# NVlabs/CenterPose

Hardware: AMD Instinct MI355X
Metric: images/sec at 512x512 DLA-34 (backbone + heat-map decode + post-process + PnP) (higher is better)
Workload: dtype f32 via split-f16 (f16x3) MFMA, f32 accumulate

## Files before the change

### centerpose_amd/csrc/cp_common.h

```cpp
#pragma once
#include <hip/hip_runtime.h>
#include <stdint.h>

#include "../../include/centerpose_hip_testing.h"

#if defined(__HIP_DEVICE_COMPILE__) && !defined(__gfx950__)
#error "centerpose_amd device code is written for gfx950 only (raw-buffer range-check semantics, MFMA shapes, LDS-DMA)"
#endif

#define CP_OK 0
#define CP_ERR_INVALID (-1)
#define CP_ERR_LAUNCH (-2)
#define CP_ERR_ALLOC (-3)
#define CP_ERR_STATE (-4)

enum CpAct : int {
    CP_ACT_NONE = 0,
    CP_ACT_RELU = 1,
    CP_ACT_SIGMOID = 2,
    CP_ACT_SIGMOID_FROM = 3,
};

enum CpStore : int {
    CP_STORE_NHWC = 0,
// ... 28 lines not shown
        const int nw = (int)(blockDim.x + 63) >> 6;
        float m = cp_amax_red[0];
        for (int i = 1; i < nw; ++i) m = fmaxf(m, cp_amax_red[i]);
        unsigned* sub = slot + (blockIdx.x & (CP_AMAX_SUB - 1)) * CP_AMAX_STRIDE;
        const unsigned b = __float_as_uint(m);
        if (b > __hip_atomic_load(sub, __ATOMIC_RELAXED, __HIP_MEMORY_SCOPE_AGENT)) atomicMax(sub, b);
    }
}

__device__ __forceinline__ float cp_fast_sigmoid(float x) {
    return __builtin_amdgcn_rcpf(1.f + __builtin_amdgcn_exp2f(-1.4426950408889634f * x));
}
__device__ __forceinline__ float cp_fast_tanh(float x) {
    return 2.f * __builtin_amdgcn_rcpf(1.f + __builtin_amdgcn_exp2f(-2.8853900817779268f * x)) - 1.f;
}
#endif

struct ConvParams {
    const float* src[CP_MAX_SRC];
    int src_c[CP_MAX_SRC];
    int nsrc;
    int Cin;
    int B, H, W, Ho, Wo;
    int KH, KW, stride, pad;
    int K;
    int Kpad;
    const float* wp;
    int Cout, CoutPad;
    const float* scale;
    const float* shift;
    const float* res;
    int res_ld;
    int act;
    int act_from;
    float* out;
    int store;
    int ldo;
    int coff;
    const void* w16_hi;
    const void* w16_lo;
    const void* w16f_hi;
    const void* w16f_lo;
    int Kpad16;
    double* gn_stats;
    int gn_groups, gn_cpg;
    const float* gn_in_mr;
    const float* gn_in_gamma;
    const float* gn_in_beta;
    const float* gn_in_a;
    const float* gn_in_d;
    const float* gru_x3;
    const float* gru_hprev;
    int splitk;
    float* partial;
    int tile_m, tile_n;
    const void* fuse_w2_hi;
    const void* fuse_w2_lo;
    float* fuse_out;
    int fuse_c2;
    int fuse_ngroups, fuse_gtiles;
    int fuse_gc2[CP_MAX_HEAD_GROUP];
    int fuse_gbase[CP_MAX_HEAD_GROUP];
    int fuse_final;
    int fuse_gsig[CP_MAX_HEAD_GROUP];
    const float* fuse_gbias[CP_MAX_HEAD_GROUP];
    float* fuse_gout[CP_MAX_HEAD_GROUP];
    const unsigned* in_amax[CP_MAX_SRC];
    unsigned* out_amax;
    const float* fuse_w2_inv;
    int dbg;
    const float* offmask;
    const int* row_index;
    int rows_per_image, row_index_stride;
    const float* up_t;
    const float* up_wt;
    int up_ld, up_f;
    const float* pj_src;
    int pj_c;
    const unsigned* pj_amax;
    const void* pj_w_hi;
    const void* pj_w_lo;
    const float* pj_scale;
    const float* pj_shift;
};

int cp_launch_conv(const ConvParams& p, hipStream_t stream);
int cp_conv_tile_n(int cout);
int cp_conv_variant(const ConvParams& p);
int cp_launch_splitk_epilogue(const ConvParams& p, hipStream_t stream);
void cp_conv_geometry(const ConvParams& p, bool f16x3, int* tiles, int* nk);
const char* cp_conv_variant_name(int v);
#define CP_NUM_CONV_VARIANTS 46
#define CP_VARIANT_HEAD_ROWS 45
#define CP_VARIANT_DECONV_F32 43
#define CP_VARIANT_DECONV16 44
#define CP_VARIANT_STRM16 41
#define CP_VARIANT_LOWC1S 42
#define CP_VARIANT_GRU 26
bool cp_conv16_supported(const ConvParams& p);
int cp_launch_conv16(const ConvParams& p, hipStream_t stream);
int cp_conv16_variant(const ConvParams& p);
bool cp_conv16_project_supported(const ConvParams& p);
bool cp_halo16_supported(const ConvParams& p);
bool cp_halo16_fused_head_supported(const ConvParams& p);
int cp_launch_halo16_fused_head(const ConvParams& p, hipStream_t stream);
bool cp_halo16_gru_supported(const ConvParams& p);
int cp_launch_halo16_gru(const ConvParams& p, hipStream_t stream);
int cp_launch_halo16(const ConvParams& p, int bn, hipStream_t stream);
bool cp_halo16_project_supported(const ConvParams& p, int bn);
bool cp_strm16_supported(const ConvParams& p);
int cp_strm16_jobs(const ConvParams& p);
int cp_launch_strm16(const ConvParams& p, hipStream_t stream);
int cp_launch_dcn16(const ConvParams& p, int bn, hipStream_t stream);
bool cp_pw16_supported(const ConvParams& p);
int cp_launch_pw16(const ConvParams& p, hipStream_t stream);
bool cp_dcn16p_supported(const ConvParams& p);
int cp_dcn16p_blocks(const ConvParams& p);
int cp_launch_dcn16p(const ConvParams& p, hipStream_t stream);
bool cp_dcn16p_wide(const ConvParams& p);
#define CP_VARIANT_DCN16S 36
#define CP_VARIANT_M64N64 37
#define CP_VARIANT_DCN16PW 38
bool cp_dcn16s_supported(const ConvParams& p);
int cp_dcn16s_items(const ConvParams& p);
int cp_launch_dcn16s(const ConvParams& p, hipStream_t stream);
int cp_launch_frag16_repack(const void* w16, void* w16f, int CoutPad, int Kpad16, hipStream_t s);
#define CP_VARIANT_DCN16T 39
bool cp_dcn16t_supported(const ConvParams& p);
bool cp_dcn16t_upadd_supported(const ConvParams& p);
int cp_launch_dcn16t(const ConvParams& p, hipStream_t stream);
#define CP_VARIANT_DCN16P 30
#define CP_VARIANT_GN_FINAL 31
#define CP_VARIANT_HALO_HEAD 32
#define CP_VARIANT_HALO_GRU 33
#define CP_VARIANT_PW16 34
int cp_launch_pack_weight16(const float* w, void* hi, void* lo, int Cout, int Cin, int taps, int Kpad16, int coff,
                            const float* fwd, hipStream_t s);
int cp_launch_weight_scale(const float* w, int Cout, int per, float* fwd, float* inv, hipStream_t s);
int cp_launch_scale16(const float* scale, const float* inv, float* out, int n, hipStream_t s);
int cp_launch_absmax(const float* x, size_t n, unsigned* slot, hipStream_t s);
bool cp_head_fuse_supported(const ConvParams& p, int c2);
int cp_launch_conv16_fused_head(const ConvParams& p, hipStream_t stream);
int cp_launch_conv16_fused_head_rows(const ConvParams& p, hipStream_t stream);
int cp_launch_pack_head_w2(const float* w1, void* hi, void* lo, float* w2_inv, int C2, int Chid, hipStream_t s);
int cp_launch_head_reduce(const float* slabs, const float* bias, float* out_nchw, int slices, int C2, int B, int HW,
                          int sigmoid, hipStream_t s);
struct HeadReduceGroup {
    int n, slices;
    int c2[CP_MAX_HEAD_GROUP], base[CP_MAX_HEAD_GROUP], sigmoid[CP_MAX_HEAD_GROUP];
    const float* bias[CP_MAX_HEAD_GROUP];
    float* out[CP_MAX_HEAD_GROUP];
};
int cp_launch_head_reduce_grouped(const float* slabs, const HeadReduceGroup& g, int B, int HW, hipStream_t s);
int cp_launch_conv16_gru(const ConvParams& p, hipStream_t stream);
#define CP_VARIANT_FUSED_HEAD 22
size_t cp_lowc_weight_halfs(int kind);
int cp_launch_pack_lowc(int kind, const float* w, void* hi, void* lo, const float* fwd, int cin, hipStream_t s);
int cp_launch_lowc(int kind, const float* in, float* out, const void* w_hi, const void* w_lo, const float* scale,
                   const float* shift, const unsigned* in_amax, unsigned* out_amax, int B, int H, int W, int planes,
                   hipStream_t s);
#define CP_VARIANT_LOWC0 23
#define CP_VARIANT_LOWC01 40
int cp_launch_lowc_fused(const float* in, float* out, const void* w0_hi, const void* w0_lo, const float* scale0, const float* shift0,
                         const void* w1_hi, const void* w1_lo, const float* scale1, const float* shift1, float bound_l, float bound_s,
                         const unsigned* in_amax, unsigned* out_amax, int B, int H, int W, int planes, hipStream_t s);
struct DeconvLaunch {
    const float* x;
    const float* wf;
    const void* w_hi;
    const void* w_lo;
    const float* scale;
    const float* shift;
    float* out;
    const unsigned* in_amax;
    unsigned* out_amax;
    int B, H, W, Cin, Cout, relu, f16x3;
};
int cp_deconv_cout_pad(int Cout);
int cp_launch_pack_deconv(const float* w, float* wf, void* hi, void* lo, float* inv, int Cin, int Cout, hipStream_t s);
int cp_launch_deconv(const DeconvLaunch& l, hipStream_t s);
#define CP_PREC_F32 0
#define CP_PREC_F16X3 1

int cp_launch_nchw_to_nhwc(const float* in, float* out, int B, int C, int H, int W, int Cpad, hipStream_t s);
int cp_launch_nhwc_to_nchw(const float* in, float* out, int B, int C, int H, int W, int ldi, hipStream_t s);
int cp_launch_maxpool2(const float* in, float* out, int B, int H, int W, int C, hipStream_t s);
int cp_launch_maxpool3s2(const float* in, float* out, int B, int H, int W, int C, unsigned* out_amax, hipStream_t s);
int cp_launch_upsample_add(const float* in, const float* w, const float* add, float* out, int B, int H, int W,
                           int C, int f, unsigned* out_amax, hipStream_t s);
int cp_launch_add_relu_sum(const float* a, const float* b, const float* c, const float* d, float* out, size_t n,
                           unsigned* out_amax, hipStream_t s);
int cp_launch_upsample2_nearest_add(const float* up1, const float* low, float* out, int B, int H, int W, int C,
                                    unsigned* out_amax, hipStream_t s);
int cp_launch_gru_gate(const float* x3, const float* h3, const float* hprev, float* hout, size_t M, unsigned* out_amax,
                       hipStream_t s);
int cp_launch_groupnorm_relu(float* x, const float* gamma, const float* beta, double* stats_ws, int B, int HW, int C,
                             int groups, float eps, unsigned* out_amax, hipStream_t s);
int cp_launch_gn_final(const float* x, const float* ga, const float* gd, const float* wp, const float* bias, float* out,
                       int B, int HW, int C, int N, int wld, int sigmoid, hipStream_t s);
int cp_launch_gn_affine(const double* stats, const float* gamma, const float* beta, float* a, float* d, int B, int C,
                        int groups, double count, float eps, const unsigned* x_amax, unsigned* y_amax, hipStream_t s);
int cp_launch_gn_finalize(const double* stats, float* mr, int n, double count, float eps, hipStream_t s);
int cp_launch_pack_weight(const float* w, float* wp, int Cout, int Cin, int taps, int CinP, int CoutPad, int coff,
                          hipStream_t s);

#define CP_DET_BBOX 0
#define CP_DET_SCORE 4
#define CP_DET_KPS 5
#define CP_DET_CLS 21
#define CP_DET_SCALE 22
#define CP_DET_SCALE_UNC 25
#define CP_DET_TRACKING 28
#define CP_DET_TRACKING_HP 30
#define CP_DET_KPS_DISP_MEAN 46
#define CP_DET_KPS_DISP_STD 62
#define CP_DET_KPS_HM_MEAN 78
#define CP_DET_KPS_HM_STD 94
#define CP_DET_KPS_HM_HEIGHT 110
#define CP_DET_STRIDE 118
size_t cp_decode_ws_bytes(int B, int J, int K);
int cp_launch_decode(hipStream_t s, int B, int J, int H, int W, float* hm, const float* hps, const float* wh,
                     const float* hps_unc, const float* scale, const float* scale_unc, const float* reg, float* hm_hp,
                     const float* hp_offset, const float* tracking, const float* tracking_hp, int K, int rep_mode,
                     int fit_gaussian, float balance, int legacy_bool_mask, int apply_sigmoid, float* det, void* ws);
int cp_launch_decode_peaks(hipStream_t s, int B, int J, int H, int W, float* hm, float* hm_hp, int K, int apply_sigmoid,
                           float* pk_score, int* pk_ind, void* cand);
int cp_launch_decode_assoc(hipStream_t s, int B, int J, int H, int W, const float* hps, const float* wh, const float* hps_unc,
                           const float* scale, const float* scale_unc, const float* reg, const float* hm_hp,
                           const float* hp_offset, const float* tracking, const float* tracking_hp, const float* pk_score,
                           const int* pk_ind, int K, int rep_mode, int fit_gaussian, float balance, int legacy_bool_mask,
                           int compact, float* det);
size_t cp_decode_cand_bytes(int B, int J, int H, int W, int K);
size_t cp_decode_tiled_ws_bytes(int B, int J, int H, int W, int K);
int cp_launch_decode_tiled(hipStream_t s, int B, int J, int H, int W, float* hm, const float* hps, const float* wh,
                           const float* hps_unc, const float* scale, const float* scale_unc, const float* reg, float* hm_hp,
                           const float* hp_offset, const float* tracking, const float* tracking_hp, int K, int rep_mode,
                           int fit_gaussian, float balance, int legacy_bool_mask, int apply_sigmoid, float* det, void* ws);

int cp_launch_dcn_generic(hipStream_t s, const float* x, const float* w, const float* bias, const float* offset,
                          const float* mask, float* out, int B, int C, int H, int W, int Co, int Ho, int Wo, int kh, int kw,
                          int sh, int sw, int ph, int pw, int dh, int dw, int dg);

struct DcnBwdArgs {
// ... 152 lines not shown
```

### centerpose_amd/csrc/engine.hip

```cpp
#include "engine_model.h"
#include "track_common.h"

namespace {
thread_local std::string g_err;
}

namespace cp_engine {
int fail(int code, const std::string& msg) {
    g_err = msg;
    return code;
}
int g_default_precision = CP_PREC_F32;
int g_dbg = 0;
}

using namespace cp_engine;

static void drop_kept_in(cp_model* m, const void* ws, size_t bytes) {
    const char* k = (const char*)m->kept.ptr;
    if (k && k >= (const char*)ws && k < (const char*)ws + bytes) m->kept = cp_model::KeptFeat();
}

template <class F>
static int replay_or_capture(cp_model* m, hipStream_t s, const std::vector<uint64_t>& key, F&& enqueue) {
// ... 29 lines not shown
extern "C" {

const char* cp_version(void) { return "centerpose_hip 0.3.0 (gfx950; f32 and split-f16 MFMA)"; }
int cp_abi_version(void) { return CP_ABI_VERSION; }
static_assert(CP_NUM_KERNEL_VARIANTS == CP_NUM_CONV_VARIANTS, "public and internal kernel-variant counts");
int cp_num_kernel_variants(void) { return CP_NUM_KERNEL_VARIANTS; }
int cp_num_roles(void) { return CP_NUM_ROLES; }
const char* cp_last_error(void) { return g_err.c_str(); }

int cp_set_debug(int flags) {
    if (flags & ~CP_SEL_ALL)
        return fail(CP_ERR_INVALID, "cp_set_debug: unknown switch bits " + std::to_string(flags & ~CP_SEL_ALL));
    g_dbg = flags;
    return CP_OK;
}

int cp_set_default_precision(int precision) {
    if (precision != CP_PREC_F32 && precision != CP_PREC_F16X3) return fail(CP_ERR_INVALID, "precision must be 0 or 1");
    g_default_precision = precision;
    return CP_OK;
}

int cp_model_set_precision(cp_model* m, int precision) {
    if (!m || (precision != CP_PREC_F32 && precision != CP_PREC_F16X3)) return fail(CP_ERR_INVALID, "bad argument");
    m->precision = precision;
    m->ws_cached = 0;
    return CP_OK;
}

int cp_model_profile(cp_model* m, int enable) {
    if (!m) return fail(CP_ERR_INVALID, "null model");
    m->profile = enable != 0;
    return CP_OK;
}

int cp_model_profile_read(cp_model* m, double* out, int num_variants) {
    if (!m || !out || num_variants < CP_NUM_CONV_VARIANTS) return fail(CP_ERR_INVALID, "bad argument");
    for (int i = 0; i < num_variants * 4; ++i) out[i] = 0.0;
    for (int i = 0; i < CP_NUM_ROLES * 4; ++i) m->roles[i] = 0.0;
    const char* dump = getenv("CP_PROFILE_DUMP");
    FILE* df = dump ? fopen(dump, "a") : nullptr;
    for (auto& r : m->prof) {
        float ms = 0.f;
        if (hipEventSynchronize(r.e1) != hipSuccess || hipEventElapsedTime(&ms, r.e0, r.e1) != hipSuccess)
            return fail(CP_ERR_LAUNCH, "event timing failed");
        if (df)
            fprintf(df, "%s,%d,%d,%d,%d,%d,%.4f,%.2f,%s\n", r.variant >= 0 ? cp_conv_variant_name(r.variant) : "decode", r.M,
                    r.N, r.K, r.kh, r.stride, ms, r.flops / (ms * 1e-3) / 1e12, cp_role_name(r.role));
        if (r.variant >= 0) {
            out[r.variant * 4 + 0] += 1.0;
            out[r.variant * 4 + 1] += ms;
            out[r.variant * 4 + 2] += r.flops;
            out[r.variant * 4 + 3] += r.bytes;
        }
        if (r.role >= 0 && r.role < CP_NUM_ROLES) {
            m->roles[r.role * 4 + 0] += 1.0;
            m->roles[r.role * 4 + 1] += ms;
            m->roles[r.role * 4 + 2] += r.flops;
            m->roles[r.role * 4 + 3] += r.bytes;
        }
        m->event_pool.push_back(r.e0);
        m->event_pool.push_back(r.e1);
    }
    m->prof.clear();
    if (df) fclose(df);
    return CP_OK;
}

const char* cp_kernel_variant_name(int v) { return cp_conv_variant_name(v); }

const char* cp_role_name(int role) {
    static const char* names[CP_NUM_ROLES] = {"conv", "conv1x1", "dcn", "dcn_offset", "head", "head_final", "gru", "lowc",
                                              "decode", "deconv"};
    return (role >= 0 && role < CP_NUM_ROLES) ? names[role] : "?";
}

int cp_model_profile_roles(cp_model* m, double* out, int num_roles) {
    if (!m || !out || num_roles < CP_NUM_ROLES) return fail(CP_ERR_INVALID, "bad argument");
    for (int i = 0; i < CP_NUM_ROLES * 4; ++i) out[i] = m->roles[i];
    return CP_OK;
}

size_t cp_model_workspace_used(const cp_model* m) { return m ? m->arena.peak : 0; }

size_t cp_model_workspace_bytes(cp_model* m, int B, int H, int W) {
    if (!m) {
        fail(CP_ERR_STATE, "cp_model_workspace_bytes: null model");
        return 0;
    }
    if (m->ws_cached && m->ws_key[0] == B && m->ws_key[1] == H && m->ws_key[2] == W && m->ws_key[3] == g_dbg && m->finalized)
        return m->ws_cached;
    size_t peak = 0;
    const char* const tap_before = m->tap_name;
    const int nu = m->ups_t.empty() ? 1 : 3;
    const int np = m->convs.count("base.level2.project") ? 2 : 1;
    for (int v = 0; v < 4 * nu * np; ++v) {
        const int up = (v >> 2) % nu;
        m->dry_variant = v & 1;
        m->tap_name = (v & 2) ? "" : nullptr;
        m->dry_no_upadd = up != 0;
        m->dry_boundary_upadd = up == 2;
        m->dry_no_project = v >= 4 * nu;
        const int rc = forward_impl(m, nullptr, B, H, W, nullptr, (const float*)1, (const float*)1, (const float*)1, nullptr, 0,
                                    nullptr, 0, true);
        m->dry_variant = 0;
        m->dry_no_upadd = false;
        m->dry_boundary_upadd = false;
        m->dry_no_project = false;
        m->tap_name = tap_before;
        if (rc != CP_OK) return 0;
        if (m->arena.peak > peak) peak = m->arena.peak;
    }
    m->ws_key[0] = B; m->ws_key[1] = H; m->ws_key[2] = W; m->ws_key[3] = g_dbg;
    m->ws_cached = peak;
    return peak;
}

int cp_model_forward(cp_model* m, cp_stream_t stream, int B, int H, int W, const float* images, const float* pre_img,
                     const float* pre_hm, const float* pre_hm_hp, float* const* head_out, int sigmoid_hm,
                     void* workspace, size_t workspace_bytes) {
    if (!images || !head_out || !workspace) return fail(CP_ERR_INVALID, "null argument");
    m->tap_name = nullptr;
    drop_kept_in(m, workspace, workspace_bytes);
    return forward_impl(m, (hipStream_t)stream, B, H, W, images, pre_img, pre_hm, pre_hm_hp, head_out, sigmoid_hm,
                        workspace, workspace_bytes, false);
}

int cp_model_features(cp_model* m, cp_stream_t stream, int B, int H, int W, const float* images, const float* pre_img,
                      const float* pre_hm, const float* pre_hm_hp, float* feat_out, void* workspace, size_t workspace_bytes) {
    if (!m || !images || !feat_out || !workspace) return fail(CP_ERR_INVALID, "null argument");
    if (m->gru) return fail(CP_ERR_STATE, "cp_model_features: dlav1 heads read the ConvGRU steps through GroupNorm, not one feature map");
    if (m->hourglass) return fail(CP_ERR_STATE, "cp_model_features: hourglass has two stacks of heads, not one feature map");
    m->tap_name = nullptr;
    drop_kept_in(m, workspace, workspace_bytes);
    m->feat_out = feat_out;
    const int rc = forward_impl(m, (hipStream_t)stream, B, H, W, images, pre_img, pre_hm, pre_hm_hp, nullptr, 0, workspace,
                                workspace_bytes, false);
    m->feat_out = nullptr;
    return rc;
}

static size_t detect_decode_ws_bytes(int B, int H, int W, int K) {
    const int ho = H / 4, wo = W / 4;
    return ho * wo <= 32768 ? cp_decode_ws_bytes(B, 8, K) : cp_decode_tiled_ws_bytes(B, 8, ho, wo, K);
}

size_t cp_model_detect_workspace_bytes(cp_model* m, int B, int H, int W, int K) {
    const size_t a = cp_model_workspace_bytes(m, B, H, W);
    const size_t d = detect_decode_ws_bytes(B, H, W, K);
    return a && d ? align_up(a, 256) + d : 0;
}

int cp_model_detect(cp_model* m, cp_stream_t stream, int B, int H, int W, const float* images, const float* pre_img,
                    const float* pre_hm, const float* pre_hm_hp, float* const* head_out, int K, int rep_mode,
                    int fit_gaussian, float balance, int legacy_bool_mask, float* det, void* workspace,
                    size_t workspace_bytes, int use_graph) {
    if (!m || !images || !head_out || !det || !workspace) return fail(CP_ERR_INVALID, "null argument");
    if (!m->finalized) return fail(CP_ERR_STATE, "model not finalized");
    const size_t model_ws = align_up(cp_model_workspace_bytes(m, B, H, W), 256);
    if (model_ws == 0) return CP_ERR_INVALID;
    const bool tiled = (H / 4) * (W / 4) > 32768;
    const size_t dec_ws = detect_decode_ws_bytes(B, H, W, K);
    if (dec_ws == 0) return fail(CP_ERR_INVALID, "detect: unsupported decode shape (need K <= 128, K <= H*W/16 <= 2^20, W/4 <= 4096)");
    if (workspace_bytes < model_ws + dec_ws) return fail(CP_ERR_INVALID, "workspace too small");
    float* hp[11] = {nullptr, nullptr, nullptr, nullptr, nullptr, nullptr, nullptr, nullptr, nullptr, nullptr, nullptr};
    const char* names[11] = {"hm", "hps", "wh", "hps_uncertainty", "scale", "scale_uncertainty", "reg", "hm_hp",
                             "hp_offset", "tracking", "tracking_hp"};
    for (size_t i = 0; i < m->headw.size(); ++i)
        for (int j = 0; j < 11; ++j)
            if (m->headw[i].name == names[j]) hp[j] = head_out[i];
    if (!hp[0] || !hp[1] || !hp[2] || !hp[7]) return fail(CP_ERR_INVALID, "detect needs the hm, hps, wh and hm_hp heads");
    hipStream_t s = (hipStream_t)stream;
    auto enqueue = [&]() -> int {
        m->tap_name = nullptr;
        int rc = forward_impl(m, s, B, H, W, images, pre_img, pre_hm, pre_hm_hp, head_out, 1, workspace, model_ws, false);
        if (rc != CP_OK) return rc;
        rc = timed(m, s, [&](cp_model::ProfRec& r) {
            const double hw = (double)(H / 4) * (W / 4);
            r.variant = -1;
            r.role = CP_ROLE_DECODE;
            r.flops = 0.0;
            r.bytes = (double)B * (9.0 * hw * 4 + K * 60.0 * 4 + 8.0 * K * 2 * 4 + (double)K * CP_DET_STRIDE * 4);
            r.M = B; r.N = K; r.K = (int)hw; r.kh = 0; r.stride = 0;
        }, [&]() {
            return (tiled ? cp_launch_decode_tiled : cp_launch_decode)(
                s, B, 8, H / 4, W / 4, hp[0], hp[1], hp[2], hp[3], hp[4], hp[5], hp[6], hp[7], hp[8], hp[9], hp[10], K, rep_mode,
                fit_gaussian, balance, legacy_bool_mask, 0, det, (char*)workspace + model_ws);
        });
        if (rc != CP_OK) return fail(rc, "detect: decode failed (need K <= 128, K <= H*W/16 <= 2^20, W/4 <= 4096)");
        return rc;
    };
// ... 423 lines not shown
```

### centerpose_amd/csrc/engine_forward.hip

```cpp
#include "engine_model.h"

using namespace cp_engine;

namespace {

constexpr int kSplitTiles = 128, kSplitTarget = 384;
constexpr long kLeanMinPixels = 32768;

struct Fwd {
    cp_model* m;
    int B;
    hipStream_t s;
    double* gn_stats_out = nullptr;
    const float* gn_in_mr = nullptr;
    const float* gn_in_a = nullptr;
    const float* gn_in_d = nullptr;
    const float* gn_in_gamma = nullptr;
    const float* gn_in_beta = nullptr;
    int role = -1;
    const unsigned* gn_in_amax = nullptr;
    static constexpr int kMaxSlots = CP_AMAX_STRIDE;
    static constexpr size_t kSlotBytes = (size_t)CP_AMAX_SUB * CP_AMAX_STRIDE * sizeof(unsigned);
    Tensor slots_t;
    unsigned* slots = nullptr;
// ... 269 lines not shown
        timed([&](cp_model::ProfRec& r) { decode_rec(r, (double)B * (K * 60.0 * 4 + 8.0 * K * 2 * 4 + (double)K * CP_DET_STRIDE * 4)); },
              [&]() {
                  return cp_launch_decode_assoc(s, B, J, x.H, x.W, tb[1], tb[2], tb[3], tb[4], tb[5], tb[6], hm_hp, tb[8], tb[9], tb[10],
                                                lc.pk_score, lc.pk_ind, K, lc.rep_mode, lc.fit_gaussian, lc.balance,
                                                lc.legacy_bool_mask, 1, lc.det);
              });
        return true;
    }

    struct UpFuse {
        const Tensor* t;
        const float* wt;
        int f;
    };
    int plan_split(ConvParams& p, bool use16, const ConvW& w) {
        int tiles = 0, nk = 0;
        cp_conv_geometry(p, use16, &tiles, &nk);
        if (use16 && tiles > 0 && (tiles <= 32 || (tiles <= 64 && nk <= 36)) && nk >= 8 && !p.gn_stats && !p.gn_in_a &&
            p.CoutPad % 64 == 0 && w.Cout >= 64 && !(g_dbg & CP_SEL_TILE128_SMALL)) {
            p.tile_m = p.tile_n = 64;
            cp_conv_geometry(p, use16, &tiles, &nk);
        }
        const bool force_strm = use16 && (g_dbg & CP_SEL_STRM16_ALWAYS) && cp_strm16_supported(p);
        if (tiles > 0 && tiles < (p.tile_m == 64 ? 256 : kSplitTiles) && nk >= 8 && !p.gn_stats && !force_strm) {
            int want = (kSplitTarget + tiles - 1) / tiles;
            if (want > nk / 2) want = nk / 2;
            if (want > 32) want = 32;
            if (want > 1) {
                const int per = (nk + want - 1) / want;
                const int sk = (nk + per - 1) / per;
                if (sk > 1) return sk;
            }
        }
        return 1;
    }
    bool upadd_fusable(const DeformW& d, int C, int H, int W, int t_c, int f, bool boundary = false) {
        if (m->precision != CP_PREC_F16X3 || (m->dry_no_upadd && !(boundary && m->dry_boundary_upadd))) return false;
        const float* const some = (const float*)0x1000;
        ConvParams p = conv_params(B, H, W, &some, &C, 1, d.main, 1, 1, CP_ACT_RELU);
        if (p.Cin != d.main.CinP) return false;
        p.offmask = some;
        const unsigned* no_amax = nullptr;
        if (!conv_params_f16(p, d.main, &no_amax, true)) return false;
        p.store = CP_STORE_NHWC;
        p.ldo = d.main.Cout;
        p.up_t = p.up_wt = some;
        p.up_ld = t_c;
        p.up_f = f;
        p.splitk = plan_split(p, true, d.main);
        return p.splitk == 1 && cp_conv16_variant(p) == CP_VARIANT_DCN16T && cp_dcn16t_upadd_supported(p);
    }

    struct ProjFuse {
        const Tensor* bottom;
        const ConvW* w;
    };
    bool project_fusable(const std::string& p, const ConvW& wp, const ConvW& w2, int cb, int C, int H, int W) {
        if (m->precision != CP_PREC_F16X3 || m->dry_no_project) return false;
        if (m->tap_name && std::strstr(m->tap_name, ".project") != nullptr) return false;
        if (g_dbg & (CP_SEL_PW16_FRAG_A | CP_SEL_PW16_NEVER)) return false;
        if (wp.CoutPad != w2.CoutPad || wp.Cout != w2.Cout || wp.Kpad16 != cb || !wp.w16f_hi || !wp.w16f_lo) return false;
        const float* const some = (const float*)0x1000;
        const unsigned* no_amax = nullptr;
        ConvParams q = conv_params(B, H, W, &some, &cb, 1, wp, 1, 0, CP_ACT_NONE);
        if (q.Cin != wp.CinP || !conv_params_f16(q, wp, &no_amax, true)) return false;
        q.store = CP_STORE_NHWC;
        q.ldo = wp.Cout;
        q.splitk = plan_split(q, true, wp);
        const int qv = cp_conv16_variant(q);
        if (q.splitk != 1 || (qv != CP_VARIANT_PW16 && qv != CP_VARIANT_PW16 + 1)) return false;
        ConvParams c = conv_params(B, H, W, &some, &C, 1, w2, 1, 1, CP_ACT_RELU);
        if (c.Cin != w2.CinP || !conv_params_f16(c, w2, &no_amax, true)) return false;
        c.store = CP_STORE_NHWC;
        c.ldo = w2.Cout;
        c.pj_src = some;
        c.pj_c = cb;
        c.pj_w_hi = c.pj_w_lo = some;
        c.splitk = plan_split(c, true, w2);
        return c.splitk == 1 && cp_conv16_project_supported(c);
    }

    Tensor conv(const ConvW& w, const std::vector<const Tensor*>& srcs, int stride, int pad, int act,
                const Tensor* res = nullptr, const Tensor* offmask = nullptr, int act_from = 0,
                float* out_nchw = nullptr, int out_ld = 0, const UpFuse* up = nullptr, const ProjFuse* pj = nullptr) {
        const Tensor& x0 = *srcs[0];
        const int nsrc = (int)srcs.size();
        const float* src[CP_MAX_SRC];
        int src_c[CP_MAX_SRC];
        const unsigned* src_amax[CP_MAX_SRC];
        for (int i = 0; i < nsrc; ++i) {
            src[i] = srcs[i]->ptr();
            src_c[i] = srcs[i]->C;
            src_amax[i] = srcs[i]->amax;
        }
        ConvParams p = conv_params(B, x0.H, x0.W, src, src_c, nsrc, w, stride, pad, act);
        if (p.Cin != w.CinP) {
            chk(fail(CP_ERR_INVALID, "conv: channel mismatch"));
            return Tensor();
        }
        p.res = res ? res->ptr() : nullptr;
        p.res_ld = res ? res->C : 0;
        p.act_from = act_from;
        p.offmask = offmask ? offmask->ptr() : nullptr;
        p.gn_stats = gn_stats_out;
        p.gn_groups = 32;
        p.gn_cpg = w.Cout / 32 > 0 ? w.Cout / 32 : 1;
        if (gn_in_a) {
            p.gn_in_a = gn_in_a;
            p.gn_in_d = gn_in_d;
        }
        if (gn_in_mr) {
            p.gn_in_mr = gn_in_mr;
            p.gn_in_gamma = gn_in_gamma;
            p.gn_in_beta = gn_in_beta;
            p.gn_cpg = w.Cin / 32;
        }
        const bool use16 = conv_params_f16(p, w, src_amax, m->precision == CP_PREC_F16X3);
        if (use16 && p.gn_in_a) p.in_amax[0] = gn_in_amax;
        if (p.gn_in_a && !use16) {
            chk(fail(CP_ERR_INVALID, "conv: GroupNorm affine input without an f16x3 kernel"));
            return Tensor();
        }
        Tensor out;
        if (out_nchw) {
            p.out = out_nchw;
            p.store = CP_STORE_NCHW;
            p.ldo = out_ld;
            p.coff = 0;
        } else {
            const int cstore = (act == CP_ACT_SIGMOID_FROM) ? w.CoutPad : w.Cout;
            out = make(cstore, p.Ho, p.Wo);
            p.out = out.ptr();
            p.out_amax = act == CP_ACT_SIGMOID_FROM ? nullptr : out.amax;
            p.store = CP_STORE_NHWC;
            p.ldo = cstore;
            p.coff = 0;
        }
        Tensor partial;
        p.splitk = plan_split(p, use16, w);
        if (p.splitk > 1) {
            partial = make(p.splitk * p.CoutPad, p.Ho, p.Wo);
            p.partial = partial.ptr();
        }
        if (up) {
            p.up_t = up->t->ptr();
            p.up_wt = up->wt;
            p.up_ld = up->t->C;
            p.up_f = up->f;
        }
        if (pj) {
            p.pj_src = pj->bottom->ptr();
            p.pj_c = pj->bottom->C;
            p.pj_amax = pj->bottom->amax;
            p.pj_w_hi = pj->w->w16f_hi;
            p.pj_w_lo = pj->w->w16f_lo;
            p.pj_scale = pj->w->scale16;
            p.pj_shift = pj->w->shift;
        }
        auto launch = [&]() -> int {
            int rc = use16 ? cp_launch_conv16(p, s) : cp_launch_conv(p, s);
            if (rc == CP_OK && p.splitk > 1) rc = cp_launch_splitk_epilogue(p, s);
            return rc;
        };
        if (!m->dry)
            timed([&](cp_model::ProfRec& r) {
                r.variant = use16 ? cp_conv16_variant(p) : cp_conv_variant(p);
                r.role = role >= 0 ? role : offmask ? CP_ROLE_DCN : act == CP_ACT_SIGMOID_FROM ? CP_ROLE_DCN_OFFSET
                         : (w.KH == 1 && w.KW == 1) ? CP_ROLE_CONV1X1 : CP_ROLE_CONV;
                const double M = (double)B * p.Ho * p.Wo;
                const int cin_real = w.Cin;
                r.flops = 2.0 * M * w.Cout * (double)(w.KH * w.KW * cin_real + (pj ? pj->w->Cin : 0));
                r.bytes = 4.0 * ((double)B * x0.H * x0.W * cin_real + M * w.Cout +
                                 (double)w.KH * w.KW * cin_real * w.Cout + (offmask ? M * 27 : 0.0) +
                                 (res ? M * w.Cout : 0.0) + (up ? (double)B * up->t->H * up->t->W * w.Cout : 0.0) +
                                 (pj ? (M + w.Cout) * (double)pj->w->Cin : 0.0));
                r.M = (int)M; r.N = w.Cout; r.K = w.KH * w.KW * cin_real; r.kh = w.KH; r.stride = stride;
            }, launch);
        gn_stats_out = nullptr;
        gn_in_mr = nullptr;
        gn_in_a = nullptr;
        gn_in_d = nullptr;
        gn_in_amax = nullptr;
        role = -1;
        return out;
    }
    const ConvW& cw(const std::string& k) { return m->convs.at(k); }

    Tensor maxpool(const Tensor& x) {
        Tensor o = make(x.C, x.H / 2, x.W / 2);
        o.amax = x.amax;
        if (!m->dry) chk(cp_launch_maxpool2(x.ptr(), o.ptr(), B, x.H, x.W, x.C, s));
        return o;
    }

    Tensor basic_block(const std::string& p, const Tensor& x, int stride, const Tensor* residual, const ProjFuse* pj = nullptr) {
        Tensor t = conv(cw(p + ".conv1"), {&x}, stride, 1, CP_ACT_RELU);
        tap(p + ".conv1", t);
        Tensor o = conv(cw(p + ".conv2"), {&t}, 1, 1, CP_ACT_RELU, residual, nullptr, 0, nullptr, 0, nullptr, pj);
        tap(p, o);
        return o;
    }

    Tensor tree1(const std::string& p, const Tensor& x, int cin, int cout, int stride, bool level_root,
                 std::vector<const Tensor*> children, const Tensor* bottom_in = nullptr) {
        Tensor bottom_own;
        const Tensor* bottom = &x;
        if (stride > 1) {
            if (bottom_in) bottom = bottom_in;
            else {
                bottom_own = maxpool(x);
                bottom = &bottom_own;
            }
        }
        Tensor proj;
        const Tensor* residual = bottom;
        ProjFuse pj = {bottom, nullptr};
        if (cin != cout) {
            const ConvW& wp = cw(p + ".project");
            const ConvW& w2 = cw(p + ".tree1.conv2");
            if (project_fusable(p, wp, w2, bottom->C, w2.CinP, bottom->H, bottom->W)) {
                pj.w = &wp;
                residual = nullptr;
            } else {
                proj = conv(wp, {bottom}, 1, 0, CP_ACT_NONE);
                tap(p + ".project", proj);
                residual = &proj;
            }
        }
        if (level_root) children.insert(children.begin(), bottom);
        Tensor x1 = basic_block(p + ".tree1", x, stride, residual, pj.w ? &pj : nullptr);
        proj = Tensor();
        Tensor x2 = basic_block(p + ".tree2", x1, 1, &x1);
        std::vector<const Tensor*> srcs = {&x2, &x1};
        for (auto* c : children) srcs.push_back(c);
        Tensor o = conv(cw(p + ".root"), srcs, 1, 0, CP_ACT_RELU);
        tap(p + ".root", o);
        return o;
    }
    Tensor tree2(const std::string& p, const Tensor& x, int cin, int cout) {
        Tensor bottom = maxpool(x);
        Tensor x1 = tree1(p + ".tree1", x, cin, cout, 2, false, {}, &bottom);
        return tree1(p + ".tree2", x1, cout, cout, 1, false, {&bottom, &x1});
    }

    Tensor deform(const std::string& p, const Tensor& x, const UpFuse* up = nullptr) {
        const DeformW& d = m->deforms.at(p);
        Tensor om = conv(d.offset, {&x}, 1, 1, CP_ACT_SIGMOID_FROM, nullptr, nullptr, 18);
        tap(p + ".offmask", om, 27);
        Tensor o = conv(d.main, {&x}, 1, 1, CP_ACT_RELU, nullptr, &om, 0, nullptr, 0, up);
        if (!up) tap(p, o);
        return o;
    }
    Tensor upsample_add(const std::string& p, const Tensor& x, int f, const Tensor& add) {
        Tensor o = make(x.C, x.H * f, x.W * f);
        if (!m->dry)
            chk(cp_launch_upsample_add(x.ptr(), m->ups.at(p), add.ptr(), o.ptr(), B, x.H, x.W, x.C, f, o.amax, s));
        return o;
    }
    struct IdaNext {
        std::string p;
        const Tensor* layer;
        int f;
    };
    Tensor ida(const std::string& p, std::vector<Tensor>& layers, int startp, int endp, const std::vector<int>& up_f,
               bool node_dead = false, const IdaNext* next = nullptr, Tensor u_first = Tensor()) {
        const bool tap_on_node = m->tap_name && std::strstr(m->tap_name, ".node_") != nullptr;
        Tensor u_next = u_first;
        u_first = Tensor();
        for (int i = startp + 1; i < endp; ++i) {
            const std::string k = std::to_string(i - startp);
            Tensor u = u_next;
            u_next = Tensor();
            if (!u.valid()) {
                Tensor t = deform(p + ".proj_" + k, layers[i]);
                u = upsample_add(p + ".up_" + k, t, up_f[i - startp], layers[i - 1]);
            }
            tap(p + ".up_" + k, u);
            const std::string kn = std::to_string(i + 1 - startp);
            const int fn = i + 1 < endp ? up_f[i + 1 - startp] : 0;
            const DeformW& node = m->deforms.at(p + ".node_" + k);
            if (node_dead && !tap_on_node && i + 1 < endp && m->ups_t.count(p + ".up_" + kn) &&
                upadd_fusable(node, u.C, u.H, u.W, m->deforms.at(p + ".proj_" + kn).main.Cout, fn)) {
                Tensor t = deform(p + ".proj_" + kn, layers[i + 1]);
                const UpFuse up = {&t, m->ups_t.at(p + ".up_" + kn), fn};
                u_next = deform(p + ".node_" + k, u, &up);
                layers[i] = Tensor();
            } else if (next && i + 1 == endp && m->ups_t.count(next->p + ".up_1") &&
                       !(m->tap_name && std::strncmp(m->tap_name, (p + ".node_" + k).c_str(), (p + ".node_" + k).size()) == 0) &&
                       upadd_fusable(node, u.C, u.H, u.W, m->deforms.at(next->p + ".proj_1").main.Cout, next->f, true)) {
                Tensor t = deform(next->p + ".proj_1", *next->layer);
                const UpFuse up = {&t, m->ups_t.at(next->p + ".up_1"), next->f};
                u_next = deform(p + ".node_" + k, u, &up);
                layers[i] = Tensor();
            } else {
                layers[i] = deform(p + ".node_" + k, u);
            }
        }
        return u_next;
    }

    Tensor lowc(const std::string& name, int kind, const float* in, int H, int W, int planes, const unsigned* in_amax) {
        if (m->precision != CP_PREC_F16X3 || (g_dbg & CP_SEL_NO_LOWC)) return Tensor();
        const int Ho = kind == 2 ? (H - 1) / 2 + 1 : H, Wo = kind == 2 ? (W - 1) / 2 + 1 : W;
        if (kind == 2 && m->lowc.count(name + ".rows") && !(g_dbg & CP_SEL_LEVEL1_ROWS_NEVER) &&
            ((g_dbg & CP_SEL_LEVEL1_ROWS_ALWAYS) || (long)B * ((Wo + 31) / 32) * ((Ho + 7) / 8) >= 2048))
            kind = 5;
        auto it = m->lowc.find(kind == 5 ? name + ".rows" : name);
        if (it == m->lowc.end()) return Tensor();
        const ConvW& w = cw(name);
        const bool stem = kind == 0 || kind == 3;
        const bool l1 = kind == 2 || kind == 5;
        const int cout = l1 ? 32 : 16, cin = stem ? planes : 16, k = stem ? 7 : 3;
        Tensor out = make(cout, Ho, Wo);
        if (m->dry) return out;
        auto launch = [&]() {
            return cp_launch_lowc(kind, in, out.ptr(), it->second.hi, it->second.lo, it->second.scale16, w.shift, in_amax,
                                  out.amax, B, H, W, planes, s);
        };
        timed([&](cp_model::ProfRec& r) {
            r.variant = kind == 5 ? CP_VARIANT_LOWC1S : CP_VARIANT_LOWC0 + (kind == 3 ? 0 : kind);
            r.role = CP_ROLE_LOWC;
            const double M = (double)B * Ho * Wo;
            r.flops = 2.0 * M * cout * (double)(k * k * cin);
            r.bytes = 4.0 * ((double)B * H * W * cin + M * cout + (double)k * k * cin * cout);
            r.M = (int)M; r.N = cout; r.K = k * k * cin; r.kh = k; r.stride = l1 ? 2 : 1;
        }, launch);
        return out;
    }

    Tensor to_nhwc(const float* nchw, int C, int Cpad, int H, int W) {
        Tensor t = make(Cpad, H, W);
        t.amax = nullptr;
        if (!m->dry) chk(cp_launch_nchw_to_nhwc(nchw, t.ptr(), B, C, H, W, Cpad, s));
        return t;
    }
    Tensor stem(const char* name, int kind, const float* nchw, int H, int W, int C, int Cpad, bool use_lowc) {
        Tensor t = lowc(name, kind, nchw, H, W, C, use_lowc && !m->dry ? input_slot(nchw, (size_t)B * C * H * W) : nullptr);
        if (!t.valid()) {
            Tensor in = to_nhwc(nchw, C, Cpad, H, W);
            t = conv(cw(name), {&in}, 1, 3, CP_ACT_RELU);
        }
        return t;
    }

    Tensor hg_residual(const std::string& p, const Tensor& x, int stride) {
        Tensor t = conv(cw(p + ".conv1"), {&x}, stride, 1, CP_ACT_RELU);
        if (m->convs.count(p + ".skip")) {
            Tensor sk = conv(cw(p + ".skip"), {&x}, stride, 0, CP_ACT_NONE);
            return conv(cw(p + ".conv2"), {&t}, 1, 1, CP_ACT_RELU, &sk);
        }
        return conv(cw(p + ".conv2"), {&t}, 1, 1, CP_ACT_RELU, &x);
    }
    Tensor hg_seq(const std::string& p, Tensor x, int n, int first_stride) {
        for (int i = 0; i < n; ++i) x = hg_residual(p + "." + std::to_string(i), x, i == 0 ? first_stride : 1);
        return x;
    }
    Tensor hg_kp(const std::string& p, const Tensor& x, int n, const int* mods) {
        const int cm = mods[0], nm = mods[1];
        Tensor up1 = hg_seq(p + ".up1", x, cm, 1);
        Tensor low = hg_seq(p + ".low1", x, cm, 2);
        low = n > 1 ? hg_kp(p + ".low2", low, n - 1, mods + 1) : hg_seq(p + ".low2", low, nm, 1);
        low = hg_seq(p + ".low3", low, cm, 1);
        Tensor out = make(up1.C, up1.H, up1.W);
        if (!m->dry)
            chk(cp_launch_upsample2_nearest_add(up1.ptr(), low.ptr(), out.ptr(), B, low.H, low.W, low.C, out.amax, s));
        tap(p, out);
        return out;
    }
    void run_hourglass(int H, int W, const float* images, float* const* head_out, int sigmoid_hm) {
        static const int mods[6] = {2, 2, 2, 2, 2, 4};
        init_slots();
        Tensor inter;
        {
            Tensor in = to_nhwc(images, 3, 4, H, W);
            Tensor p0 = conv(cw("pre.0"), {&in}, 2, 3, CP_ACT_RELU);
            inter = hg_residual("pre.1", p0, 2);
        }
        tap("pre", inter);
        Tensor cnv;
        for (int k = 0; k < 2; ++k) {
            const std::string ks = std::to_string(k);
            Tensor kp = hg_kp("kps." + ks, inter, 5, mods);
            cnv = conv(cw("cnvs." + ks), {&kp}, 1, 1, CP_ACT_RELU);
            tap("cnvs." + ks, cnv);
            if (k == 0) {
                Tensor a = conv(cw("inters_.0"), {&inter}, 1, 0, CP_ACT_NONE);
                Tensor b = conv(cw("cnvs_.0"), {&cnv}, 1, 0, CP_ACT_RELU, &a);
                inter = hg_residual("inters.0", b, 1);
            }
        }
        if (fused_heads_grouped(cnv, head_out, sigmoid_hm)) return;
        for (size_t i = 0; i < m->headw.size(); ++i) {
            const HeadW& hw = m->headw[i];
            const bool sg = sigmoid_hm && (hw.name == "hm" || hw.name == "hm_hp");
            if (hw.w2_hi && m->precision == CP_PREC_F16X3 && !m->tap_name && !(g_dbg & CP_SEL_NO_HEAD_FUSION) &&
                fused_head(hw, cnv, sg, m->dry ? (float*)0x1000 : head_out[i]))
                continue;
            role = CP_ROLE_HEAD;
            Tensor hid = conv(hw.c0, {&cnv}, 1, 1, CP_ACT_RELU);
            role = CP_ROLE_HEAD_FINAL;
            conv(hw.c1, {&hid}, 1, 0, sg ? CP_ACT_SIGMOID : CP_ACT_NONE, nullptr, nullptr, 0,
                 m->dry ? (float*)0x1000 : head_out[i], hw.classes);
        }
    }

    Tensor deconv(const std::string& p, const Tensor& x) {
        const DeconvW& d = m->deconvs.at(p);
// ... 53 lines not shown
            for (int b = 0; b < blocks[l]; ++b) x = res_block(ln + "." + std::to_string(b), x, b == 0 && l ? 2 : 1, bott);
            tap(ln, x);
        }
        for (int i = 0; i < 3; ++i) {
            const std::string fc = "deconv_layers." + std::to_string(6 * i);
            x = deform(fc, x);
            tap("deconv_layers." + std::to_string(6 * i + 2), x);
            x = deconv("deconv_layers." + std::to_string(6 * i + 3), x);
            tap("deconv_layers." + std::to_string(6 * i + 5), x);
        }
        if (features_only(x)) return;
        for (size_t i = 0; i < m->headw.size(); ++i) {
            const HeadW& hw = m->headw[i];
            const bool sg = sigmoid_hm && (hw.name == "hm" || hw.name == "hm_hp");
            role = CP_ROLE_HEAD;
            Tensor hid = conv(hw.c0, {&x}, 1, 1, CP_ACT_RELU);
            role = CP_ROLE_HEAD_FINAL;
            conv(hw.c1, {&hid}, 1, 0, sg ? CP_ACT_SIGMOID : CP_ACT_NONE, nullptr, nullptr, 0,
                 m->dry ? (float*)0x1000 : head_out[i], hw.classes);
        }
    }

    void run(int H, int W, const float* images, const float* pre_img, const float* pre_hm, const float* pre_hm_hp,
             float* const* head_out, int sigmoid_hm) {
        init_slots();
        const bool use_lowc = m->precision == CP_PREC_F16X3 && !(g_dbg & CP_SEL_NO_LOWC) && m->lowc.count("base.base_layer");
        const bool no_pre = m->dry ? m->dry_variant == 1 : (!pre_img && !pre_hm && !pre_hm_hp);
        const bool fuse01 = use_lowc && no_pre && m->lowc.count("base.level0.rows") && m->stem_bound_l > 0.f &&
                            !(g_dbg & CP_SEL_STEM_LEVEL0_UNFUSED) && !(m->tap_name && std::strcmp(m->tap_name, "base.base_layer") == 0) &&
                            !m->convs.count("base.pre_img_layer") && !m->convs.count("base.pre_hm_layer") && !m->convs.count("base.pre_hm_hp_layer");
        Tensor l0f;
        if (fuse01) {
            const unsigned* in_slot = !m->dry ? input_slot(images, (size_t)B * 3 * H * W) : nullptr;
            l0f = make(16, H, W);
            if (!m->dry) {
                const LowcW& a = m->lowc["base.base_layer"];
                const LowcW& c = m->lowc["base.level0.rows"];
                auto launch = [&]() {
                    return cp_launch_lowc_fused(images, l0f.ptr(), a.hi, a.lo, a.scale16, cw("base.base_layer").shift, c.hi, c.lo, c.scale16,
                                                cw("base.level0").shift, m->stem_bound_l, m->stem_bound_s, in_slot, l0f.amax, B, H, W, 3, s);
                };
                timed([&](cp_model::ProfRec& r) {
                    r.variant = CP_VARIANT_LOWC01;
                    r.role = CP_ROLE_LOWC;
                    const double M = (double)B * H * W;
                    r.flops = 2.0 * M * 16 * (147.0 + 144.0);
                    r.bytes = 4.0 * (M * 3 + M * 16);
                    r.M = (int)M; r.N = 16; r.K = 147 + 144; r.kh = 7; r.stride = 1;
                }, launch);
            }
        }
        Tensor x0 = fuse01 ? Tensor() : stem("base.base_layer", 0, images, H, W, 3, 4, use_lowc);
        if (m->dry) {
            if (!m->convs.count("base.pre_img_layer")) pre_img = nullptr;
            if (!m->convs.count("base.pre_hm_layer")) pre_hm = nullptr;
            if (!m->convs.count("base.pre_hm_hp_layer")) pre_hm_hp = nullptr;
        }
        if ((pre_img && !m->convs.count("base.pre_img_layer")) || (pre_hm && !m->convs.count("base.pre_hm_layer")) ||
            (pre_hm_hp && !m->convs.count("base.pre_hm_hp_layer"))) {
            chk(fail(CP_ERR_INVALID, "a previous-frame input was given to a model built without that pre_* layer"));
            return;
        }
        if (pre_img || pre_hm || pre_hm_hp) {
            Tensor a, b, c;
            if (pre_img) a = stem("base.pre_img_layer", 0, pre_img, H, W, 3, 4, use_lowc);
            if (pre_hm) b = stem("base.pre_hm_layer", 0, pre_hm, H, W, 1, 4, use_lowc);
            if (pre_hm_hp) c = stem("base.pre_hm_hp_layer", 3, pre_hm_hp, H, W, 8, 8, use_lowc);
            std::vector<const Tensor*> adds;
            for (Tensor* t : {&a, &b, &c})
                if (t->valid()) adds.push_back(t);
            Tensor sum = make(16, H, W);
            if (!m->dry)
                chk(cp_launch_add_relu_sum(x0.ptr(), adds[0]->ptr(), adds.size() > 1 ? adds[1]->ptr() : nullptr,
                                           adds.size() > 2 ? adds[2]->ptr() : nullptr, sum.ptr(),
                                           (size_t)B * H * W * 16, sum.amax, s));
            x0 = sum;
        }
        if (!fuse01) tap("base.base_layer", x0);
        Tensor l0 = fuse01 ? l0f : lowc("base.level0", 1, x0.ptr(), H, W, 16, x0.amax);
        l0f = Tensor();
        if (!l0.valid()) l0 = conv(cw("base.level0"), {&x0}, 1, 1, CP_ACT_RELU);
        tap("base.level0", l0);
        x0 = Tensor();
        Tensor l1 = lowc("base.level1", 2, l0.ptr(), H, W, 16, l0.amax);
        if (!l1.valid()) l1 = conv(cw("base.level1"), {&l0}, 2, 1, CP_ACT_RELU);
        tap("base.level1", l1);
        l0 = Tensor();
        std::vector<Tensor> L(6);
        L[2] = tree1("base.level2", l1, 32, 64, 2, false, {});
        l1 = Tensor();
        L[3] = tree2("base.level3", L[2], 64, 128);
        L[4] = tree2("base.level4", L[3], 128, 256);
        L[5] = tree1("base.level5", L[4], 256, 512, 2, true, {});
        tap("base.level2", L[2]);
        tap("base.level3", L[3]);
        tap("base.level4", L[4]);
        tap("base.level5", L[5]);

        ida("dla_up.ida_0", L, 4, 6, {1, 2});
        Tensor o2 = L[5];
        ida("dla_up.ida_1", L, 3, 6, {1, 2, 2});
        Tensor o1 = L[5];
        const IdaNext to_ida_up = {"ida_up", &o1, 2};
        Tensor u1 = ida("dla_up.ida_2", L, 2, 6, {1, 2, 2, 2}, true, &to_ida_up);
        Tensor o0 = L[5];
        for (auto& t : L) t = Tensor();
        std::vector<Tensor> y = {o0, o1, o2};
        o0 = o1 = o2 = Tensor();
        ida("ida_up", y, 0, 3, {1, 2, 4}, true, nullptr, u1);
        u1 = Tensor();
        Tensor feat = y[2];
        y.clear();
        tap("feat", feat);
        if (features_only(feat)) return;

        std::vector<Tensor> gru_out;
        if (m->gru) {
            const int steps = m->tracking ? 4 : 3;
            role = CP_ROLE_GRU;
            Tensor x3 = conv(m->gru_x, {&feat}, 1, 1, CP_ACT_NONE);
            Tensor h;
            for (int st = 0; st < steps; ++st) {
                Tensor hn = make(64, feat.H, feat.W);
                const size_t M = (size_t)B * feat.H * feat.W;
                if (st == 0) {
                    if (!m->dry) chk(cp_launch_gru_gate(x3.ptr(), nullptr, nullptr, hn.ptr(), M, hn.amax, s));
                } else if (m->precision == CP_PREC_F16X3 && m->gru_h16_hi && !(g_dbg & CP_SEL_GRU_UNFUSED) &&
                           (size_t)M * 192 * 4 < (size_t)0xf0000000u) {
                    if (!m->dry) {
                        ConvW w;
                        w.KH = w.KW = 3;
                        w.K = w.Kpad = w.Kpad16 = 576;
                        w.Cout = w.CoutPad = 192;
                        w.w16_hi = m->gru_h16_hi;
                        w.w16_lo = m->gru_h16_lo;
                        w.w16f_hi = m->gru_h16f_hi;
                        w.w16f_lo = m->gru_h16f_lo;
                        w.scale16 = m->gru_h16_inv;
                        const float* src = h.ptr();
                        ConvParams p = conv_params(B, feat.H, feat.W, &src, &h.C, 1, w, 1, 1, CP_ACT_NONE);
                        conv_params_f16(p, w, &h.amax, true, true);
                        p.out_amax = hn.amax;
                        p.out = hn.ptr();
                        p.gru_x3 = x3.ptr();
                        p.gru_hprev = h.ptr();
                        p.splitk = 1;
                        timed([&](cp_model::ProfRec& r) {
                            r.variant = cp_halo16_gru_supported(p) ? CP_VARIANT_HALO_GRU : CP_VARIANT_GRU;
                            r.role = CP_ROLE_GRU;
                            r.flops = 2.0 * (double)M * 192 * 576;
                            r.bytes = 4.0 * ((double)M * (64 + 192 + 64 + 64) + 576.0 * 192);
                            r.M = (int)M; r.N = 192; r.K = 576; r.kh = 3; r.stride = 1;
                        }, [&]() { return cp_launch_conv16_gru(p, s); });
                    }
                } else {
                    role = CP_ROLE_GRU;
                    Tensor h3 = conv(m->gru_h, {&h}, 1, 1, CP_ACT_NONE);
                    if (!m->dry) chk(cp_launch_gru_gate(x3.ptr(), h3.ptr(), h.ptr(), hn.ptr(), M, hn.amax, s));
                }
                h = hn;
                gru_out.push_back(h);
                tap(("convGRU.step" + std::to_string(st)).c_str(), h);
            }
        }

        if (!m->gru && fused_heads_grouped(feat, head_out, sigmoid_hm)) return;
        Tensor stats_all;
        if (m->gru) {
            stats_all = make(128 * (int)m->headw.size(), 1, 1);
            if (!m->dry && hipMemsetAsync(stats_all.ptr(), 0, sizeof(double) * 64 * B * m->headw.size(), s) != hipSuccess)
                chk(CP_ERR_LAUNCH);
        }
        for (size_t i = 0; i < m->headw.size(); ++i) {
            const HeadW& hw = m->headw[i];
            const Tensor* src = &feat;
            if (m->gru) {
// ... 14 lines not shown
                    continue;
                }
                src = &gru_out[r];
            }
            Tensor mr, ad;
            double* stats = m->gru && !m->dry ? (double*)stats_all.ptr() + (size_t)i * 64 * B : nullptr;
            const bool fuse_gn = m->gru && ((src->H * src->W) % 32 == 0) && hw.c0.Cout % 32 == 0 && (hw.c0.Cout / 32) % 4 == 0;
            if (m->gru) {
                mr = make(64, 1, 1);
                if (fuse_gn && !m->dry) gn_stats_out = stats;
            }
            const bool sg = sigmoid_hm && (hw.name == "hm" || hw.name == "hm_hp");
            if (!m->gru && hw.w2_hi && m->precision == CP_PREC_F16X3 && !m->tap_name && !(g_dbg & CP_SEL_NO_HEAD_FUSION) &&
                fused_head(hw, *src, sg, m->dry ? (float*)0x1000 : head_out[i]))
                continue;
            role = CP_ROLE_HEAD;
            Tensor hid = conv(hw.c0, {src}, 1, 1, m->gru ? CP_ACT_NONE : CP_ACT_RELU);
            if (m->gru) {
                if (fuse_gn) {
                    const bool affine16 = m->precision == CP_PREC_F16X3 && hw.c1.w16_hi && (hid.H * hid.W) % 128 == 0 &&
                                          !(g_dbg & CP_SEL_GN_HEAD_F32);
                    if (affine16) {
                        ad = make(2 * hid.C, 1, 1);
                        if (!m->dry) {
                            float* ap = ad.ptr();
                            float* dp = ap + (size_t)B * hid.C;
                            unsigned* bound = new_slot();
                            chk(cp_launch_gn_affine((const double*)stats, hw.gn_gamma, hw.gn_beta, ap, dp, B, hid.C, 32,
                                                    (double)hid.H * hid.W * (hid.C / 32), 1e-5f, hid.amax, bound, s));
                            gn_in_a = ap;
                            gn_in_d = dp;
                            gn_in_amax = bound;
                        }
                    } else if (!m->dry) {
                        chk(cp_launch_gn_finalize((const double*)stats, mr.ptr(), B * 32,
                                                  (double)hid.H * hid.W * (hid.C / 32), 1e-5f, s));
                        gn_in_mr = mr.ptr();
                        gn_in_gamma = hw.gn_gamma;
                        gn_in_beta = hw.gn_beta;
                    }
                } else if (!m->dry) {
                    chk(cp_launch_groupnorm_relu(hid.ptr(), hw.gn_gamma, hw.gn_beta, stats, B,
                                                 hid.H * hid.W, hid.C, 32, 1e-5f, hid.amax, s));
                }
            }
            role = CP_ROLE_HEAD_FINAL;
            if (gn_in_a && !(g_dbg & CP_SEL_GN_HEAD_MFMA) && hid.C % 64 == 0 && hid.C <= 256 && (hid.H * hid.W) % 64 == 0 &&
                ((size_t)B * hid.H * hid.W) % 256 == 0 && hw.classes <= 16 && !m->tap_name) {
                auto launch = [&]() -> int {
                    return cp_launch_gn_final(hid.ptr(), gn_in_a, gn_in_d, hw.c1.wp, hw.c1.shift, head_out[i], B, hid.H * hid.W,
                                              hid.C, hw.classes, hw.c1.CoutPad, sg ? 1 : 0, s);
                };
                timed([&](cp_model::ProfRec& r) {
                    r.variant = CP_VARIANT_GN_FINAL;
                    r.role = CP_ROLE_HEAD_FINAL;
                    const double M = (double)B * hid.H * hid.W;
                    r.flops = 2.0 * M * hw.classes * (double)hid.C;
                    r.bytes = 4.0 * (M * hid.C + M * hw.classes + (double)hid.C * hw.classes);
                    r.M = (int)M; r.N = hw.classes; r.K = hid.C; r.kh = 1; r.stride = 1;
                }, launch);
                gn_in_a = gn_in_d = nullptr;
                gn_in_amax = nullptr;
                role = -1;
                continue;
            }
            conv(hw.c1, {&hid}, 1, 0, sg ? CP_ACT_SIGMOID : CP_ACT_NONE, nullptr, nullptr, 0,
                 m->dry ? (float*)0x1000 : head_out[i], hw.classes);
        }
    }
};

}

int cp_engine::forward_impl(cp_model* m, hipStream_t stream, int B, int H, int W, const float* images, const float* pre_img,
                 const float* pre_hm, const float* pre_hm_hp, float* const* head_out, int sigmoid_hm, void* ws,
                 size_t ws_bytes, bool dry) {
    if (!m || !m->finalized) return fail(CP_ERR_STATE, "model not finalized");
    if (B < 1 || H % 32 || W % 32 || H < 32 || W < 32) return fail(CP_ERR_INVALID, "H and W must be multiples of 32");
    if (m->hourglass && (H % 128 || W % 128))
        return fail(CP_ERR_INVALID, "hourglass: H and W must be multiples of 128 (stride 4, then five stride-2 levels)");
    m->arena.reset(dry ? nullptr : ws, ws_bytes);
    m->dry = dry;
    m->status = CP_OK;
    Fwd f{m, B, stream};
    if (m->hourglass) f.run_hourglass(H, W, images, head_out, sigmoid_hm);
    else if (m->resnet) f.run_resnet(H, W, images, head_out, sigmoid_hm);
    else f.run(H, W, images, pre_img, pre_hm, pre_hm_hp, head_out, sigmoid_hm);
    if (!dry && m->arena.overflow)
        return fail(CP_ERR_INVALID, "workspace too small: " + std::to_string(ws_bytes) + " bytes given, this launch sequence peaks at " +
                                        std::to_string(m->arena.peak));
    return m->status;
}

int cp_engine::kept_dense_heads(cp_model* m, hipStream_t stream, float* const* head_out) {
    const auto& k = m->kept;
    m->dry = false;
    m->status = CP_OK;
    Fwd f{m, k.B, stream};
    if (!lean_finished_maps(m) && !k.slabs)
        return fail(CP_ERR_STATE, "dense heads: the lean detect's workspace was sized without room for the slabs this switch setting needs");
    if (!f.grouped_launch(m->reg_group, k.ptr, k.amax, k.C, k.H, k.W, head_out, 0, k.slabs))
        return fail(CP_ERR_STATE, "dense heads: the grouped head launch does not apply under the current switches");
    return m->status;
}

int cp_engine::kept_heads_at(cp_model* m, hipStream_t stream, const int* index, int n, float* const* table_out, float* slabs) {
    const auto& k = m->kept;
    m->dry = false;
    m->status = CP_OK;
    Fwd f{m, k.B, stream};
    f.heads_at_rows(0, (int)m->reg_group.idx.size(), k.ptr, k.amax, k.C, k.H, k.W, index, n, n, k.B, n, table_out, slabs);
    return m->status;
}
```

### centerpose_amd/csrc/engine_model.h

```cpp
#pragma once
#include "../../include/centerpose_hip.h"
#include "../../include/centerpose_hip_testing.h"
#undef CP_OK
#undef CP_ERR_INVALID
#undef CP_ERR_LAUNCH
#undef CP_ERR_ALLOC
#undef CP_ERR_STATE
#undef CP_DET_STRIDE
#undef CP_PNP_STRIDE
#undef CP_TRACK_STRIDE
#include "cp_common.h"

#include <cmath>
#include <cstdio>
#include <cstdlib>
#include <cstring>
#include <map>
#include <memory>
#include <string>
#include <vector>

namespace cp_engine {

int fail(int code, const std::string& msg);
// ... 101 lines not shown
};

struct HeadW {
    std::string name;
    int classes = 0;
    ConvW c0, c1;
    void* w2_hi = nullptr;
    void* w2_lo = nullptr;
    float* w2_inv = nullptr;
    float* gn_gamma = nullptr;
    float* gn_beta = nullptr;
};

inline bool resnet_spec(int depth, bool* bottleneck, int* blocks) {
    static const int spec[5][5] = {{18, 2, 2, 2, 2}, {34, 3, 4, 6, 3}, {50, 3, 4, 6, 3}, {101, 3, 4, 23, 3}, {152, 3, 8, 36, 3}};
    for (const auto& r : spec)
        if (r[0] == depth) {
            *bottleneck = depth >= 50;
            for (int i = 0; i < 4; ++i) blocks[i] = r[i + 1];
            return true;
        }
    return false;
}

}

struct cp_model {
    std::string arch;
    bool gru = false, tracking = false, finalized = false, hourglass = false;
    int resnet = 0;
    int precision = cp_engine::g_default_precision;
    int head_conv = 256;
    std::vector<std::pair<std::string, int>> heads;
    std::map<std::string, std::vector<float>> params;
    std::map<std::string, cp_engine::ConvW> convs;
    std::map<std::string, cp_engine::DeformW> deforms;
    std::map<std::string, float*> ups;
    std::map<std::string, float*> ups_t;
    std::map<std::string, cp_engine::DeconvW> deconvs;
    std::vector<cp_engine::HeadW> headw;
    struct HeadGroup {
        bool ok = false;
        void* w16f_hi = nullptr;
        void* w16f_lo = nullptr;
        void* w2_hi = nullptr;
        void* w2_lo = nullptr;
        float* scale16 = nullptr;
        float* shift = nullptr;
        float* w2_inv = nullptr;
        int Cin = 0, hid = 0, Kpad16 = 0;
        void* w16_hi = nullptr;
        void* w16_lo = nullptr;
        std::vector<int> idx;
    } head_group;
    HeadGroup hm_group, reg_group;
    int lean_ncentre = 0;
    struct LeanCall {
        float* const* table_out;
        float* pk_score;
        int* pk_ind;
        void* scratch;
        float* dense_slabs;
        int K, rep_mode, fit_gaussian, legacy_bool_mask;
        float balance;
        float* det;
    };
    const LeanCall* lean = nullptr;
    bool lean_taken = false;
    int lean_key[5] = {0, 0, 0, -1, -1};
    bool lean_ok = false;
    struct KeptFeat {
        const float* ptr = nullptr;
        unsigned* amax = nullptr;
        int B = 0, H = 0, W = 0, C = 0;
        float* slabs = nullptr;
    } kept;
    std::map<std::vector<uint64_t>, KeptFeat> graph_kept;
    std::map<std::string, cp_engine::LowcW> lowc;
    int ws_key[4] = {0, 0, 0, -1};
    size_t ws_cached = 0;
    bool dry_no_upadd = false;
    bool dry_boundary_upadd = false;
    bool dry_no_project = false;
    int dry_variant = 0;
    float stem_bound_l = 0.f, stem_bound_s = 0.f;
    cp_engine::ConvW gru_x, gru_h;
    void* gru_h16_hi = nullptr;
    void* gru_h16_lo = nullptr;
    void* gru_h16f_hi = nullptr;
    void* gru_h16f_lo = nullptr;
    float* gru_h16_fwd = nullptr;
    float* gru_h16_inv = nullptr;
    std::vector<void*> device_allocs;
    cp_engine::Arena arena;
    hipStream_t stream = nullptr;
    int B = 0;
    bool dry = false;
    int status = CP_OK;
    const char* tap_name = nullptr;
    float* tap_out = nullptr;
    int* tap_dims = nullptr;
    float* feat_out = nullptr;
    struct ProfRec {
        int variant;
        int role = 0;
        double flops, bytes;
        int M, N, K, kh, stride;
        hipEvent_t e0, e1;
    };
    std::map<std::vector<uint64_t>, hipGraphExec_t> graphs;
    bool profile = false;
    std::vector<ProfRec> prof;
    double roles[CP_NUM_ROLES * 4] = {0};
    std::vector<hipEvent_t> event_pool;
    hipEvent_t get_event() {
        if (!event_pool.empty()) {
            hipEvent_t e = event_pool.back();
            event_pool.pop_back();
            return e;
        }
        hipEvent_t e = nullptr;
        (void)hipEventCreate(&e);
        return e;
    }
};

namespace cp_engine {

int forward_impl(cp_model* m, hipStream_t stream, int B, int H, int W, const float* images, const float* pre_img,
                 const float* pre_hm, const float* pre_hm_hp, float* const* head_out, int sigmoid_hm, void* ws,
                 size_t ws_bytes, bool dry);

int kept_dense_heads(cp_model* m, hipStream_t stream, float* const* head_out);
int kept_heads_at(cp_model* m, hipStream_t stream, const int* index, int n, float* const* table_out, float* slabs);

inline size_t lean_slab_bytes(const cp_model* m, size_t rows) {
    size_t planes = 0;
    for (int i : m->reg_group.idx) planes += (size_t)(m->reg_group.hid / 128) * m->headw[i].classes;
    return align_up(planes * rows * sizeof(float), 256);
}

inline bool lean_finished_maps(const cp_model* m) {
    return m->head_group.Cin == 64 && m->head_group.hid == 256 && !(g_dbg & CP_SEL_HEADS_SLABS);
}

template <class D, class F>
inline int timed(cp_model* m, hipStream_t s, D&& describe, F&& launch) {
    if (!m->profile) return launch();
    cp_model::ProfRec r;
    describe(r);
    r.e0 = m->get_event();
    r.e1 = m->get_event();
    (void)hipEventRecord(r.e0, s);
    const int rc = launch();
    (void)hipEventRecord(r.e1, s);
    m->prof.push_back(r);
    return rc;
}

inline ConvW conv_w_f32(float* wp, const float* scale, const float* shift, int Cin, int Cout, int KH, int KW) {
    ConvW w;
    w.wp = wp;
    w.scale = scale;
    w.shift = shift;
    w.Cin = w.CinP = Cin;
    w.Cout = Cout;
    w.CoutPad = (int)align_up((size_t)Cout, cp_conv_tile_n(Cout));
    w.KH = KH;
    w.KW = KW;
    w.K = KH * KW * Cin;
    w.Kpad = (int)align_up((size_t)w.K, 16);
    return w;
}

inline ConvParams conv_params(int B, int H, int W, const float* const* src, const int* src_c, int nsrc, const ConvW& w,
                              int stride, int pad, int act) {
    ConvParams p;
    std::memset(&p, 0, sizeof(p));
    p.nsrc = nsrc;
    for (int i = 0; i < nsrc; ++i) {
        p.src[i] = src[i];
// ... 60 lines not shown
```

### centerpose_amd/csrc/igemm16.hip

```cpp
#include "igemm16_common.h"

namespace {

template <int MT, int NT, int WM, int WN, bool MULTISRC, bool FUSE = false, bool GNIN = false, bool GRU = false, bool ROWS = false>
__global__ __launch_bounds__(WM * WN * 64, 2) void igemm16p_kernel(const ConvParams p, const int tiles_m, const int tiles_n) {
    static_assert(!FUSE || (MT == 2 && NT == 2 && WM == 2 && WN == 2 && !MULTISRC), "fused head: 128x128 tiles");
    static_assert(!GRU || (MT == 1 && NT == 3 && WM == 4 && WN == 1 && !MULTISRC && !FUSE), "GRU: 128x96 tiles");
    static_assert(!ROWS || FUSE, "pixel lists: fused heads only");
    typedef Frag<32> F;
    typedef F::acc_t acc_t;
    constexpr int BM = 32 * MT * WM, BN = 32 * NT * WN;
    constexpr int NTH = WM * WN * 64;
    constexpr int RPP = NTH / 8;
    constexpr int A_SLOTS = BM * BK16 / 4 / NTH;
    constexpr int B_CHUNKS = BN * BK16 * 2 / 16;
    constexpr int B_SLOTS = (B_CHUNKS + NTH - 1) / NTH;
    constexpr bool B_PART = B_CHUNKS % NTH != 0;
    constexpr int A_SZ = BM * LDH, B_SZ = BN * LDH;
    constexpr int BUF = 2 * A_SZ + 2 * B_SZ;
    constexpr int NM = 3 * MT * NT;
    constexpr int NR = 2 * MT + 2 * NT;
    __shared__ __attribute__((aligned(16))) _Float16 lds[2 * BUF];

    const int tid = threadIdx.x;
// ... 507 lines not shown
    hipLaunchKernelGGL(weight_scale_kernel, dim3(Cout), dim3(64), 0, s, w, per, fwd, inv);
    return hipGetLastError() == hipSuccess ? CP_OK : CP_ERR_LAUNCH;
}

int cp_launch_scale16(const float* scale, const float* inv, float* out, int n, hipStream_t s) {
    hipLaunchKernelGGL(scale16_kernel, dim3((n + 255) / 256), dim3(256), 0, s, scale, inv, out, n);
    return hipGetLastError() == hipSuccess ? CP_OK : CP_ERR_LAUNCH;
}

int cp_launch_absmax(const float* x, size_t n, unsigned* slot, hipStream_t s) {
    if (n % 4 || ((uintptr_t)x & 15)) return CP_ERR_INVALID;
    size_t g = (n / 4 + 255) / 256;
    if (g > 2048) g = 2048;
    if (g < 1) g = 1;
    hipLaunchKernelGGL(absmax_kernel, dim3((unsigned)g), dim3(256), 0, s, (const float4*)x, n / 4, slot);
    return hipGetLastError() == hipSuccess ? CP_OK : CP_ERR_LAUNCH;
}

static int conv16_tile_n(const ConvParams& p) {
    const int bn = cp_conv_tile_n(p.Cout);
    if (p.tile_n && p.tile_n < bn && p.CoutPad % p.tile_n == 0 && (!p.offmask || p.tile_n == 64)) return p.tile_n;
    return (bn < 32 && p.CoutPad >= 32 && p.CoutPad % 32 == 0) ? 32 : bn;
}

static bool dcn16p_wanted(const ConvParams& p) {
    if ((p.dbg & CP_SEL_DCN16P_NEVER) || !cp_dcn16p_supported(p)) return false;
    return (p.dbg & CP_SEL_DCN16P_ALWAYS) || cp_dcn16p_blocks(p) >= 64;
}

static bool dcn16s_wanted(const ConvParams& p) {
    if ((p.dbg & CP_SEL_DCN16S_NEVER) || !dcn16p_wanted(p) || !cp_dcn16s_supported(p)) return false;
    if (cp_dcn16p_wide(p) && !(p.dbg & CP_SEL_DCN16S_ALWAYS)) return false;
    return (p.dbg & CP_SEL_DCN16S_ALWAYS) || cp_dcn16s_items(p) >= 4096;
}

static bool dcn16t_wanted(const ConvParams& p) {
    if ((p.dbg & CP_SEL_DCN16T_NEVER) || !dcn16p_wanted(p) || !cp_dcn16t_supported(p)) return false;
    if (p.dbg & CP_SEL_DCN16T_ALWAYS) return true;
    if (p.dbg & CP_SEL_DCN16S_ALWAYS) return false;
    return !cp_dcn16p_wide(p) && cp_dcn16p_blocks(p) >= 1024;
}

static bool strm16_wanted(const ConvParams& p) {
    if ((p.dbg & CP_SEL_STRM16_NEVER) || (p.dbg & CP_SEL_HALO_NEVER) || !cp_strm16_supported(p)) return false;
    return (p.dbg & CP_SEL_STRM16_ALWAYS) || cp_strm16_jobs(p) >= 1024;
}

static bool halo16_wanted(const ConvParams& p, int bn) {
    if ((p.dbg & CP_SEL_HALO_NEVER) || p.gn_in_a || !cp_halo16_supported(p)) return false;
    return bn == 32 || (p.w16f_hi && p.w16f_lo && !(p.dbg & CP_SEL_HALO_LDS_WEIGHTS)) || (p.dbg & CP_SEL_HALO_ALWAYS);
}

static bool pw16_wanted(const ConvParams& p) { return !(p.dbg & CP_SEL_PW16_NEVER) && cp_pw16_supported(p); }

bool cp_conv16_supported(const ConvParams& p) {
    if (!p.w16_hi || !p.w16_lo || p.Cin % BK16 != 0 || p.KH * p.KW > 32) return false;
    for (int s = 0; s < p.nsrc; ++s)
        if (p.src_c[s] % BK16 != 0) return false;
    const int bn = conv16_tile_n(p);
    if (bn < 32) return false;
    if (p.gn_in_mr) return false;
    if (p.gn_in_a || p.gn_in_d) {
        if (!p.gn_in_a || !p.gn_in_d || bn != 32 || p.KH != 1 || p.KW != 1 || p.pad != 0 || p.stride != 1 || p.nsrc != 1 ||
            p.offmask || (p.Ho * p.Wo) % 128 != 0)
            return false;
    }
    if (p.offmask && bn < 64) return false;
    for (int s = 0; s < p.nsrc; ++s)
        if ((size_t)p.B * p.H * p.W * p.src_c[s] * 4 >= (size_t)0xf0000000u) return false;
    if ((size_t)p.CoutPad * p.Kpad16 * 2 >= ((size_t)1 << 32)) return false;
    return true;
}

bool cp_conv16_project_supported(const ConvParams& p) {
    if (!cp_conv16_supported(p) || p.offmask || p.gn_in_a || p.up_t) return false;
    const int bn = conv16_tile_n(p);
    return !(bn == 64 && p.tile_m == 64) && halo16_wanted(p, bn) && cp_halo16_project_supported(p, bn);
}

int cp_launch_conv16(const ConvParams& p, hipStream_t stream) {
    if (!cp_conv16_supported(p)) return CP_ERR_INVALID;
    if (p.up_t && !(p.offmask && dcn16t_wanted(p) && cp_dcn16t_upadd_supported(p))) return CP_ERR_INVALID;
    const int bn = conv16_tile_n(p);
    if (p.pj_src) return cp_conv16_project_supported(p) ? cp_launch_halo16(p, bn, stream) : CP_ERR_INVALID;
    const bool cat = p.nsrc > 1;
    if (p.gn_in_a) {
        const int M = p.B * p.Ho * p.Wo;
        const int tiles_m = (M + 127) / 128, tiles_n = p.CoutPad / 32;
        hipLaunchKernelGGL((igemm16p_kernel<1, 1, 4, 1, false, false, true>),
                           dim3(tiles_m * tiles_n, p.splitk > 1 ? p.splitk : 1), dim3(NT16), 0, stream, p, tiles_m, tiles_n);
        return hipGetLastError() == hipSuccess ? CP_OK : CP_ERR_LAUNCH;
    }
    if (p.offmask) {
        if (p.KH != 3 || p.KW != 3 || p.stride != 1 || p.pad != 1 || p.nsrc != 1 || p.H != p.Ho || p.W != p.Wo)
            return CP_ERR_INVALID;
        if (dcn16t_wanted(p)) return cp_launch_dcn16t(p, stream);
        if (dcn16s_wanted(p)) return cp_launch_dcn16s(p, stream);
        if (dcn16p_wanted(p)) return cp_launch_dcn16p(p, stream);
        return cp_launch_dcn16(p, bn, stream);
    }
    if (bn == 64 && p.tile_m == 64) return cat ? launch16<1, 1, 2, 2, true>(p, stream) : launch16<1, 1, 2, 2, false>(p, stream);
    if (bn == 32 && strm16_wanted(p)) return cp_launch_strm16(p, stream);
    if (halo16_wanted(p, bn)) return cp_launch_halo16(p, bn, stream);
    if (pw16_wanted(p)) return cp_launch_pw16(p, stream);
    if (bn == 128) return cat ? launch16<2, 2, 2, 2, true>(p, stream) : launch16<2, 2, 2, 2, false>(p, stream);
    if (bn == 64) return cat ? launch16<2, 1, 2, 2, true>(p, stream) : launch16<2, 1, 2, 2, false>(p, stream);
    return cat ? launch16<1, 1, 4, 1, true>(p, stream) : launch16<1, 1, 4, 1, false>(p, stream);
}

int cp_conv16_variant(const ConvParams& p) {
    const int bn = conv16_tile_n(p);
    if (p.offmask) return dcn16t_wanted(p) ? CP_VARIANT_DCN16T : dcn16s_wanted(p) ? CP_VARIANT_DCN16S : dcn16p_wanted(p) ? (cp_dcn16p_wide(p) ? CP_VARIANT_DCN16PW : CP_VARIANT_DCN16P) : bn == 128 ? 18 : 17;
    const int t = bn == 32 ? 0 : bn == 64 ? 1 : 2;
    if (bn == 64 && p.tile_m == 64) return CP_VARIANT_M64N64;
    if (bn == 32 && strm16_wanted(p)) return CP_VARIANT_STRM16;
    if (halo16_wanted(p, bn)) return 27 + t;
    if (pw16_wanted(p)) return CP_VARIANT_PW16 + (p.CoutPad % 128 == 0 ? 1 : 0);
    return (p.nsrc > 1 ? 19 : 14) + t;
}

int cp_launch_pack_weight16(const float* w, void* hi, void* lo, int Cout, int Cin, int taps, int Kpad16, int coff,
                            const float* fwd, hipStream_t s) {
    const size_t n = (size_t)Cout * Cin * taps;
    int g = (int)((n + 255) / 256);
    if (g > 4096) g = 4096;
    hipLaunchKernelGGL(pack_weight16_kernel, dim3(g), dim3(256), 0, s, w, (_Float16*)hi, (_Float16*)lo, Cout, Cin, taps,
                       Kpad16, coff, fwd);
    return hipGetLastError() == hipSuccess ? CP_OK : CP_ERR_LAUNCH;
}

bool cp_head_fuse_supported(const ConvParams& p, int c2) {
    return cp_conv16_supported(p) && !p.offmask && p.nsrc == 1 && p.CoutPad % 128 == 0 && p.Cout == p.CoutPad &&
           c2 >= 1 && c2 <= 32 && !p.res && !p.gn_stats && !p.gn_in_mr &&
           (p.act == CP_ACT_RELU || p.act == CP_ACT_NONE);
}

int cp_launch_conv16_fused_head(const ConvParams& p, hipStream_t stream) {
    if (!cp_head_fuse_supported(p, p.fuse_c2) || !p.fuse_w2_hi || !p.fuse_w2_lo || !p.fuse_out || p.splitk > 1)
        return CP_ERR_INVALID;
    if (cp_halo16_fused_head_supported(p)) return cp_launch_halo16_fused_head(p, stream);
    const int M = p.B * p.Ho * p.Wo;
    const int tiles_m = (M + 127) / 128, tiles_n = p.CoutPad / 128;
    hipLaunchKernelGGL((igemm16p_kernel<2, 2, 2, 2, false, true>), dim3(tiles_m * tiles_n), dim3(NT16), 0, stream, p,
                       tiles_m, tiles_n);
    return hipGetLastError() == hipSuccess ? CP_OK : CP_ERR_LAUNCH;
}

int cp_launch_conv16_fused_head_rows(const ConvParams& p, hipStream_t stream) {
    const int c2 = p.fuse_ngroups > 0 ? 1 : p.fuse_c2;
    if (!cp_head_fuse_supported(p, c2) || !p.fuse_w2_hi || !p.fuse_w2_lo || !p.fuse_out || p.splitk > 1 || !p.row_index ||
        p.rows_per_image < 1 || p.row_index_stride < p.rows_per_image || p.KH != 3 || p.KW != 3 || p.stride != 1 || p.pad != 1 ||
        p.fuse_ngroups < 0 || p.fuse_ngroups > CP_MAX_HEAD_GROUP)
        return CP_ERR_INVALID;
    if (p.fuse_ngroups > 0) {
        if (p.fuse_gtiles < 1 || p.fuse_ngroups * p.fuse_gtiles * 128 != p.CoutPad) return CP_ERR_INVALID;
        for (int g = 0; g < p.fuse_ngroups; ++g)
            if (p.fuse_gc2[g] < 1 || p.fuse_gc2[g] > 32 || p.fuse_gbase[g] < 0) return CP_ERR_INVALID;
    }
    const long long M = (long long)p.B * p.rows_per_image;
    if (M >= (1ll << 24)) return CP_ERR_INVALID;
    const int tiles_m = (int)((M + 127) / 128), tiles_n = p.CoutPad / 128;
    hipLaunchKernelGGL((igemm16p_kernel<2, 2, 2, 2, false, true, false, false, true>), dim3(tiles_m * tiles_n), dim3(NT16), 0,
                       stream, p, tiles_m, tiles_n);
    return hipGetLastError() == hipSuccess ? CP_OK : CP_ERR_LAUNCH;
}

// ... 44 lines not shown
```

### centerpose_amd/csrc/lowc.hip

```cpp
#include "cp_common.h"

typedef _Float16 h8 __attribute__((ext_vector_type(8)));
typedef __fp16 fp16x2 __attribute__((ext_vector_type(2)));
typedef float f32x4 __attribute__((ext_vector_type(4)));
typedef float f32x16 __attribute__((ext_vector_type(16)));
typedef uint32_t u32x4 __attribute__((ext_vector_type(4)));
typedef uint32_t u32x2 __attribute__((ext_vector_type(2)));

#ifdef CP_LOWC_STAMP
__device__ unsigned long long g_lowc_clk[4][16];
#define LOWC_STAMP(i) do { if (blockIdx.x == gridDim.x / 2 + 1 && threadIdx.x == 0) { asm volatile("s_waitcnt vmcnt(0) lgkmcnt(0)"); \
                                g_lowc_clk[(CIN == 4 ? 0 : S) + (NG - 1) * 3][i] = clock64(); } } while (0)
extern "C" int cp_debug_read_lowc_clk(unsigned long long* out) {
    return hipMemcpyFromSymbol(out, HIP_SYMBOL(g_lowc_clk), sizeof(unsigned long long) * 64) == hipSuccess ? 0 : -1;
}
#else
#define LOWC_STAMP(i) do { } while (0)
#endif

namespace {

struct LowcParams {
    const float* in;
    float* out;
// ... 362 lines not shown
            for (int g = 0; g < 2; ++g) {
                h8 wh[3], wl[3];
#pragma unroll
                for (int k = 0; k < 3; ++k) {
                    const u32x4 a = w1_s[0][2 * (2 - k) + g][lane], c = w1_s[1][2 * (2 - k) + g][lane];
                    wh[k] = *reinterpret_cast<const h8*>(&a);
                    wl[k] = *reinterpret_cast<const h8*>(&c);
                }
#pragma unroll
                for (int k = 0; k < 3; ++k) lacc[k] = __builtin_amdgcn_mfma_f32_16x16x32_f16(wh[k], bl[g], lacc[k], 0, 0, 0);
#pragma unroll
                for (int k = 0; k < 3; ++k) lacc[k] = __builtin_amdgcn_mfma_f32_16x16x32_f16(wl[k], bh[g], lacc[k], 0, 0, 0);
#pragma unroll
                for (int k = 0; k < 3; ++k) lacc[k] = __builtin_amdgcn_mfma_f32_16x16x32_f16(wh[k], bh[g], lacc[k], 0, 0, 0);
            }
            const int o = i - 1;
            const f32x4 ldone = lacc[0];
            lacc[0] = lacc[1];
            lacc[1] = lacc[2];
            lacc[2] = f32x4{0.f, 0.f, 0.f, 0.f};
            {
                const bool st_ok = o >= y0 && o < y_end && ocol_ok;
                float4 y;
                y.x = fmaxf(ldone[0] * sc1.x + sh1.x, 0.f);
                y.y = fmaxf(ldone[1] * sc1.y + sh1.y, 0.f);
                y.z = fmaxf(ldone[2] * sc1.z + sh1.z, 0.f);
                y.w = fmaxf(ldone[3] * sc1.w + sh1.w, 0.f);
                const float m4 = fmaxf(fmaxf(y.x, y.y), fmaxf(y.z, y.w));
                amax = fmaxf(amax, st_ok ? m4 : 0.f);
                const u32x4 pk = {__float_as_uint(y.x), __float_as_uint(y.y), __float_as_uint(y.z), __float_as_uint(y.w)};
                __builtin_amdgcn_raw_buffer_store_b128(pk, r_out, (int)(st_ok ? (unsigned)((o * p.W + x0 + pl) * 64 + 16 * q) : 0x80000000u), 0, 0);
            }
        }
    }
    if (p.out_amax) cp_amax_commit(p.out_amax, amax);
}

template <int CIN, int KS>
__global__ void pack_lowc_weights(const float* __restrict__ w, uint16_t* __restrict__ hi, uint16_t* __restrict__ lo,
                                  const float* __restrict__ fwd, int cout, int cin, int ci0) {
    constexpr int KSTEPS = CIN == 4 ? KS : (KS * KS * CIN + 31) / 32;
    const int nf = cout / 16, total = KSTEPS * nf * 64 * 8;
    for (int idx = blockIdx.x * blockDim.x + threadIdx.x; idx < total; idx += gridDim.x * blockDim.x) {
        const int j = idx & 7, lane = (idx >> 3) & 63, sf = idx >> 9;
        const int f = sf % nf, s = sf / nf;
        const int co = f * 16 + (lane & 15), q = lane >> 4;
        float v = 0.f;
        if (CIN == 4) {
            const int kh = s, kw = 2 * q + (j >> 2), ci = ci0 + (j & 3);
            if (kw < KS && ci < cin) v = w[(((size_t)co * cin + ci) * KS + kh) * KS + kw];
        } else {
            const int tap = 2 * s + (q >> 1), ci = (q & 1) * 8 + j;
            if (tap < KS * KS && ci < cin) v = w[(((size_t)co * cin + ci) * KS + tap / KS) * KS + tap % KS];
        }
        uint32_t h, l;
        split2(fwd ? v * fwd[co] : v, 0.f, &h, &l);
        hi[idx] = (uint16_t)(h & 0xffffu);
        lo[idx] = (uint16_t)(l & 0xffffu);
    }
}

constexpr int L1_W = 32;
constexpr int L1_PIECES = (2 * L1_W + 1) * 4;
constexpr int L1_NLD = (L1_PIECES + 63) / 64;
constexpr int L1_PITCH = 48;
constexpr int L1_PLANE = 40 * L1_PITCH;
constexpr int L1_ROWB = 4 * L1_PLANE;
constexpr int L1_WAVES = 8;
constexpr int L1_WB = 9 * 2 * 1024;
constexpr int L1_TPITCH = 144;
constexpr int L1_TRB = 32 * L1_TPITCH;
constexpr int L1_LDS = L1_WB + L1_WAVES * (L1_ROWB + L1_TRB);
constexpr int L1_PF = 4;
static_assert(L1_LDS > 80 * 1024 && L1_LDS <= 160 * 1024, "one workgroup per CU");

struct Lowc1Params {
    const float* in;
    float* out;
    const void *w_hi, *w_lo;
    const float *scale, *shift;
    const unsigned* in_amax;
    unsigned* out_amax;
    int B, H, W, Ho, Wo, rows, strips, bands, njobs;
};

__global__ __launch_bounds__(64 * L1_WAVES, 1) void lowc1s_kernel(const Lowc1Params p) {
    extern __shared__ __attribute__((aligned(16))) unsigned char l1_smem[];
    const int tid = threadIdx.x, lane = tid & 63;
    const int wid = __builtin_amdgcn_readfirstlane(tid >> 6);
    {
        const u32x4* gh = reinterpret_cast<const u32x4*>(p.w_hi);
        const u32x4* gl = reinterpret_cast<const u32x4*>(p.w_lo);
        u32x4* ws = reinterpret_cast<u32x4*>(l1_smem);
        for (int i = tid; i < 9 * 64; i += 64 * L1_WAVES) {
            const int t = i >> 6, l = i & 63;
            ws[(2 * t) * 64 + l] = gh[i];
            ws[(2 * t + 1) * 64 + l] = gl[i];
        }
    }
    __syncthreads();
    float afwd = 1.f, ainv = 1.f;
    if (p.in_amax) cp_amax_to_scale(cp_amax_read(p.in_amax), &afwd, &ainv);
    afwd = __uint_as_float(__builtin_amdgcn_readfirstlane(__float_as_uint(afwd)));
    ainv = __uint_as_float(__builtin_amdgcn_readfirstlane(__float_as_uint(ainv)));
    unsigned char* row_b = l1_smem + L1_WB + wid * (L1_ROWB + L1_TRB);
    unsigned char* tr_b = row_b + L1_ROWB;
    const unsigned char* w_b = l1_smem + lane * 16;
    const int px = lane & 31, kg = lane >> 5;
    float4 sc[4], sh[4];
#pragma unroll
    for (int g4 = 0; g4 < 4; ++g4) {
        const int n0 = 8 * g4 + 4 * kg;
        sc[g4] = p.scale ? *reinterpret_cast<const float4*>(p.scale + n0) : make_float4(1.f, 1.f, 1.f, 1.f);
        sh[g4] = p.shift ? *reinterpret_cast<const float4*>(p.shift + n0) : make_float4(0.f, 0.f, 0.f, 0.f);
        sc[g4].x *= ainv; sc[g4].y *= ainv; sc[g4].z *= ainv; sc[g4].w *= ainv;
    }
    float amax = 0.f;
    int wo[L1_NLD];
#pragma unroll
    for (int k = 0; k < L1_NLD; ++k) {
        const int i = lane + 64 * k, pp = i >> 2;
        wo[k] = (pp & 1) * L1_PLANE + (pp >> 1) * L1_PITCH + (i & 3) * 8;
    }

    for (int job = (int)blockIdx.x * L1_WAVES + wid; job < p.njobs; job += (int)gridDim.x * L1_WAVES) {
        int t = job;
        const int sx = t % p.strips;
        t /= p.strips;
        const int band = t % p.bands, b = t / p.bands;
        const int x0 = sx * L1_W;
        const int y0 = band * p.rows, y1 = min(y0 + p.rows, p.Ho);
        const int jlast = 2 * y1 - 1;
        const __amdgpu_buffer_rsrc_t r_in = __builtin_amdgcn_make_buffer_rsrc(const_cast<float*>(p.in + (size_t)b * p.H * p.W * 16), 0,
                                                                            (int)((unsigned)p.H * (unsigned)p.W * 64u), 0x00020000);
        const __amdgpu_buffer_rsrc_t r_out = __builtin_amdgcn_make_buffer_rsrc(p.out + (size_t)b * p.Ho * p.Wo * 32, 0,
                                                                             (int)((unsigned)p.Ho * (unsigned)p.Wo * 128u), 0x00020000);
        unsigned cvo[L1_NLD];
#pragma unroll
        for (int k = 0; k < L1_NLD; ++k) {
            const int i = lane + 64 * k, c = 2 * x0 - 1 + (i >> 2);
            cvo[k] = (i < L1_PIECES && (unsigned)c < (unsigned)p.W) ? (unsigned)(c * 64 + (i & 3) * 16) : 0xffffffffu;
        }
        const float col_okf = x0 + px < p.Wo ? 1.f : 0.f;
        float4 pf[L1_PF][L1_NLD];
        auto request = [&](int j, float4 (&v)[L1_NLD]) {
            const bool row_ok = (unsigned)j < (unsigned)p.H && j <= jlast;
            const int so = row_ok ? j * p.W * 64 : 0;
#pragma unroll
            for (int k = 0; k < L1_NLD; ++k) {
                const u32x4 x = __builtin_amdgcn_raw_buffer_load_b128(r_in, (int)(row_ok ? cvo[k] : 0xffffffffu), so, 0);
                v[k] = make_float4(__uint_as_float(x.x), __uint_as_float(x.y), __uint_as_float(x.z), __uint_as_float(x.w));
            }
        };
#pragma unroll
        for (int d = 0; d < L1_PF; ++d) {
            request(2 * y0 - 1 + d, pf[d]);
            __builtin_amdgcn_sched_barrier(0);
        }
        f32x16 acc;
#pragma unroll
        for (int r = 0; r < 16; ++r) acc[r] = 0.f;

        auto stage = [&](const int j, float4 (&buf)[L1_NLD]) {
#pragma unroll
            for (int k = 0; k < L1_NLD; ++k) {
                const float4 v = buf[k];
                uint32_t h0, l0, h1, l1;
                split2(v.x * afwd, v.y * afwd, &h0, &l0);
                split2(v.z * afwd, v.w * afwd, &h1, &l1);
                *reinterpret_cast<u32x2*>(row_b + wo[k]) = u32x2{h0, h1};
                *reinterpret_cast<u32x2*>(row_b + 2 * L1_PLANE + wo[k]) = u32x2{l0, l1};
            }
            request(j + L1_PF, buf);
            __builtin_amdgcn_wave_barrier();
        };
        auto mac = [&](const int kh, f32x16& a) {
#pragma unroll
            for (int kw = 0; kw < 3; ++kw) {
                const int ao = (kw == 1 ? L1_PLANE : 0) + (px + (kw == 2 ? 1 : 0)) * L1_PITCH + kg * 16;
                const h8 xh = *reinterpret_cast<const h8*>(row_b + ao), xl = *reinterpret_cast<const h8*>(row_b + 2 * L1_PLANE + ao);
                const int tp = kh * 3 + kw;
                const h8 wh = *reinterpret_cast<const h8*>(w_b + (2 * tp) * 1024), wl = *reinterpret_cast<const h8*>(w_b + (2 * tp + 1) * 1024);
                a = __builtin_amdgcn_mfma_f32_32x32x16_f16(wh, xl, a, 0, 0, 0);
                a = __builtin_amdgcn_mfma_f32_32x32x16_f16(wl, xh, a, 0, 0, 0);
                a = __builtin_amdgcn_mfma_f32_32x32x16_f16(wh, xh, a, 0, 0, 0);
            }
        };
        auto odd_row = [&](const int j, float4 (&buf)[L1_NLD]) {
            stage(j, buf);
            mac(2, acc);
            f32x16 nxt;
#pragma unroll
            for (int r = 0; r < 16; ++r) nxt[r] = 0.f;
            mac(0, nxt);
            __builtin_amdgcn_wave_barrier();
            const int o = (j - 1) >> 1;
            const unsigned okm = ~(unsigned)((o - y0) >> 31) & (unsigned)((o - y1) >> 31);
            const float okf = __uint_as_float(okm & __float_as_uint(col_okf));
#pragma unroll
            for (int g4 = 0; g4 < 4; ++g4) {
                float4 y;
                y.x = fmaxf(acc[4 * g4] * sc[g4].x + sh[g4].x, 0.f);
                y.y = fmaxf(acc[4 * g4 + 1] * sc[g4].y + sh[g4].y, 0.f);
                y.z = fmaxf(acc[4 * g4 + 2] * sc[g4].z + sh[g4].z, 0.f);
                y.w = fmaxf(acc[4 * g4 + 3] * sc[g4].w + sh[g4].w, 0.f);
                amax = fmaxf(amax, fmaxf(fmaxf(y.x, y.y), fmaxf(y.z, y.w)) * okf);
                *reinterpret_cast<float4*>(tr_b + px * L1_TPITCH + (2 * g4 + kg) * 16) = y;
            }
            __builtin_amdgcn_wave_barrier();
            const unsigned row_out = (unsigned)(o * p.Wo) * 128u, row_no = ~okm & 0x80000000u;
#pragma unroll
            for (int i = 0; i < 4; ++i) {
                const int pxo = (lane >> 3) + 8 * i;
                const u32x4 pk = *reinterpret_cast<const u32x4*>(tr_b + pxo * L1_TPITCH + (lane & 7) * 16);
                const unsigned col_no = x0 + pxo < p.Wo ? 0u : 0x80000000u;
                __builtin_amdgcn_raw_buffer_store_b128(pk, r_out, (int)((row_out + (unsigned)((x0 + pxo) * 128 + (lane & 7) * 16)) | row_no | col_no), 0, 0);
            }
            __builtin_amdgcn_wave_barrier();
            acc = nxt;
        };
        auto even_row = [&](const int j, float4 (&buf)[L1_NLD]) {
            stage(j, buf);
            mac(1, acc);
            __builtin_amdgcn_wave_barrier();
        };
        for (int j = 2 * y0 - 1; j <= jlast; j += 4) {
            odd_row(j, pf[0]);
            even_row(j + 1, pf[1]);
            odd_row(j + 2, pf[2]);
            even_row(j + 3, pf[3]);
        }
    }
    if (p.out_amax) cp_amax_commit(p.out_amax, amax);
}

__global__ void pack_lowc1s_weights(const float* __restrict__ w, uint16_t* __restrict__ hi, uint16_t* __restrict__ lo,
                                    const float* __restrict__ fwd, int cin) {
    const int total = 9 * 64 * 8;
    for (int idx = blockIdx.x * blockDim.x + threadIdx.x; idx < total; idx += gridDim.x * blockDim.x) {
        const int j = idx & 7, lane = (idx >> 3) & 63, tp = idx >> 9;
        const int co = lane & 31, ci = (lane >> 5) * 8 + j;
        float v = 0.f;
        if (ci < cin) v = w[(((size_t)co * cin + ci) * 3 + tp / 3) * 3 + tp % 3];
        uint32_t h, l;
        split2(fwd ? v * fwd[co] : v, 0.f, &h, &l);
        hi[idx] = (uint16_t)(h & 0xffffu);
        lo[idx] = (uint16_t)(l & 0xffffu);
    }
}

template <int CIN, int KS, int S, int COUT, int TW, int TH, bool NCHW_IN, int NG = 1>
int launch_lowc(const LowcParams& p, hipStream_t s) {
    const int tiles = ((p.Wo + TW - 1) / TW) * ((p.Ho + TH - 1) / TH) * p.B;
    hipLaunchKernelGGL((lowc_kernel<CIN, KS, S, COUT, TW, TH, NCHW_IN, NG>), dim3(tiles), dim3(256), 0, s, p);
    return hipGetLastError() == hipSuccess ? CP_OK : CP_ERR_LAUNCH;
}

}

size_t cp_lowc_weight_halfs(int kind) {
    return kind == 0 ? (size_t)7 * 1 * 512 : kind == 1 ? (size_t)5 * 1 * 512 : kind == 2 ? (size_t)5 * 2 * 512 : kind == 4 ? (size_t)6 * 512 : kind == 5 ? (size_t)9 * 512 : (size_t)14 * 512;
}

int cp_launch_pack_lowc(int kind, const float* w, void* hi, void* lo, const float* fwd, int cin, hipStream_t s) {
    if (kind == 0) hipLaunchKernelGGL((pack_lowc_weights<4, 7>), dim3(16), dim3(256), 0, s, w, (uint16_t*)hi, (uint16_t*)lo, fwd, 16, cin, 0);
    else if (kind == 1) hipLaunchKernelGGL((pack_lowc_weights<16, 3>), dim3(16), dim3(256), 0, s, w, (uint16_t*)hi, (uint16_t*)lo, fwd, 16, cin, 0);
    else if (kind == 2) hipLaunchKernelGGL((pack_lowc_weights<16, 3>), dim3(16), dim3(256), 0, s, w, (uint16_t*)hi, (uint16_t*)lo, fwd, 32, cin, 0);
    else if (kind == 3) {
        hipLaunchKernelGGL((pack_lowc_weights<4, 7>), dim3(16), dim3(256), 0, s, w, (uint16_t*)hi, (uint16_t*)lo, fwd, 16, cin, 0);
        hipLaunchKernelGGL((pack_lowc_weights<4, 7>), dim3(16), dim3(256), 0, s, w, (uint16_t*)hi + 7 * 512, (uint16_t*)lo + 7 * 512,
                           fwd, 16, cin, 4);
    } else if (kind == 4) {
        hipLaunchKernelGGL(pack_lowc_rows_weights, dim3(16), dim3(256), 0, s, w, (uint16_t*)hi, (uint16_t*)lo, fwd, 16, cin);
    } else if (kind == 5) {
        hipLaunchKernelGGL(pack_lowc1s_weights, dim3(16), dim3(256), 0, s, w, (uint16_t*)hi, (uint16_t*)lo, fwd, cin);
    } else return CP_ERR_INVALID;
    return hipGetLastError() == hipSuccess ? CP_OK : CP_ERR_LAUNCH;
}

int cp_launch_lowc_fused(const float* in, float* out, const void* w0_hi, const void* w0_lo, const float* scale0, const float* shift0,
                         const void* w1_hi, const void* w1_lo, const float* scale1, const float* shift1, float bound_l, float bound_s,
                         const unsigned* in_amax, unsigned* out_amax, int B, int H, int W, int planes, hipStream_t s) {
    if (planes < 1 || planes > 3 || B < 1 || H < 1 || W < 1) return CP_ERR_INVALID;
    Lowc2Params p;
    p.in = in; p.out = out;
    p.w0_hi = w0_hi; p.w0_lo = w0_lo; p.w1_hi = w1_hi; p.w1_lo = w1_lo;
    p.scale0 = scale0; p.shift0 = shift0; p.scale1 = scale1; p.shift1 = shift1;
    p.in_amax = in_amax; p.out_amax = out_amax;
    p.bound_l = bound_l; p.bound_s = bound_s;
    p.B = B; p.H = H; p.W = W; p.planes = planes;
    p.strips = (W + L2_SW - 1) / L2_SW;
    int bands = 8192 / (B * p.strips);
    if (bands < 1) bands = 1;
    int rows = (H + bands - 1) / bands;
    if (rows < 8) rows = 8;
    p.rows = rows;
    p.bands = (H + rows - 1) / rows;
    const int groups = (p.strips + 3) / 4;
    hipLaunchKernelGGL(lowc2_kernel, dim3(groups * p.bands * B), dim3(256), 0, s, p);
    return hipGetLastError() == hipSuccess ? CP_OK : CP_ERR_LAUNCH;
}

int cp_launch_lowc(int kind, const float* in, float* out, const void* w_hi, const void* w_lo, const float* scale,
                   const float* shift, const unsigned* in_amax, unsigned* out_amax, int B, int H, int W, int planes,
                   hipStream_t s) {
    LowcParams p;
    p.in_amax = in_amax;
    p.out_amax = out_amax;
    p.in = in;
    p.out = out;
    p.w_hi = w_hi;
    p.w_lo = w_lo;
    p.scale = scale;
    p.shift = shift;
    p.B = B;
    p.H = H;
    p.W = W;
    p.planes = planes;
    if (kind == 0) {
        if (planes < 1 || planes > 4) return CP_ERR_INVALID;
        p.Ho = H; p.Wo = W; p.pad = 3;
        return launch_lowc<4, 7, 1, 16, 64, 8, true>(p, s);
    }
    if (kind == 1) {
        p.Ho = H; p.Wo = W; p.pad = 1;
        return launch_lowc<16, 3, 1, 16, 32, 8, false>(p, s);
    }
    if (kind == 2) {
        p.Ho = (H + 2 - 3) / 2 + 1; p.Wo = (W + 2 - 3) / 2 + 1; p.pad = 1;
        return launch_lowc<16, 3, 2, 32, 32, 8, false>(p, s);
    }
    if (kind == 3) {
        if (planes < 5 || planes > 8) return CP_ERR_INVALID;
        p.Ho = H; p.Wo = W; p.pad = 3;
        return launch_lowc<4, 7, 1, 16, 64, 8, true, 2>(p, s);
    }
    if (kind == 5) {
        Lowc1Params q;
        q.in = in; q.out = out; q.w_hi = w_hi; q.w_lo = w_lo; q.scale = scale; q.shift = shift; q.in_amax = in_amax; q.out_amax = out_amax;
        q.B = B; q.H = H; q.W = W;
        q.Ho = (H + 2 - 3) / 2 + 1; q.Wo = (W + 2 - 3) / 2 + 1;
        if ((size_t)H * W * 64 >= (size_t)0x70000000u || (size_t)q.Ho * q.Wo * 128 >= (size_t)0x70000000u) return CP_ERR_INVALID;
        static int cus_of[16] = {0};
        int dev = 0;
        if (hipGetDevice(&dev) != hipSuccess || dev < 0 || dev >= 16) return CP_ERR_LAUNCH;
        if (!cus_of[dev]) {
            hipDeviceProp_t prop;
            if (hipFuncSetAttribute(reinterpret_cast<const void*>(&lowc1s_kernel), hipFuncAttributeMaxDynamicSharedMemorySize, L1_LDS) != hipSuccess)
                return CP_ERR_LAUNCH;
            cus_of[dev] = (hipGetDeviceProperties(&prop, dev) == hipSuccess && prop.multiProcessorCount > 0) ? prop.multiProcessorCount : 256;
        }
        const int cus = cus_of[dev];
        q.strips = (q.Wo + L1_W - 1) / L1_W;
        int rows = 64;
        while (rows > 8 && B * q.strips * ((q.Ho + rows - 1) / rows) < cus * L1_WAVES) rows >>= 1;
        int use_cus = cus;
        if (B * q.strips * ((q.Ho + 31) / 32) >= 2 * cus * L1_WAVES) {
            rows = 32;
            use_cus = cus * 3 / 4;
        }
        q.rows = rows;
        q.bands = (q.Ho + rows - 1) / rows;
        q.njobs = B * q.strips * q.bands;
        const int blocks = (q.njobs + L1_WAVES - 1) / L1_WAVES < use_cus ? (q.njobs + L1_WAVES - 1) / L1_WAVES : use_cus;
        hipLaunchKernelGGL(lowc1s_kernel, dim3(blocks), dim3(64 * L1_WAVES), L1_LDS, s, q);
        return hipGetLastError() == hipSuccess ? CP_OK : CP_ERR_LAUNCH;
    }
    return CP_ERR_INVALID;
}
```

### centerpose_amd/csrc/pw16.hip

```cpp
#include "igemm16_common.h"

namespace {

constexpr int DA = 6;
constexpr int DB = 3;

template <int NT>
__global__ __launch_bounds__(256, 2) void pw16_kernel(const ConvParams p, const int tiles_m, const int tiles_n) {
    typedef Frag<32> F;
    typedef F::acc_t acc_t;
    const int lane = threadIdx.x & 63;
    const int wid = __builtin_amdgcn_readfirstlane(threadIdx.x >> 6);
    const int tile = tile_of_block(tiles_m, tiles_n);
    const int tn = tile % tiles_n, tm = tile / tiles_n;
    const int M = p.B * p.Ho * p.Wo;
    float afwd, ainv;
    conv_in_scale(p, &afwd, &ainv);

    const int row = tm * 128 + wid * 32 + (lane & 31), half = lane >> 5;
    const int n0 = p.src_c[0] >> 4, n1 = p.nsrc > 1 ? p.src_c[1] >> 4 : 0, n2 = p.nsrc > 2 ? p.src_c[2] >> 4 : 0;
    const __amdgpu_buffer_rsrc_t r0 = make_rsrc(p.src[0], (unsigned)M * (unsigned)p.src_c[0] * 4u);
    const __amdgpu_buffer_rsrc_t r1 = make_rsrc(p.nsrc > 1 ? p.src[1] : p.src[0], p.nsrc > 1 ? (unsigned)M * (unsigned)p.src_c[1] * 4u : 0u);
    const __amdgpu_buffer_rsrc_t r2 = make_rsrc(p.nsrc > 2 ? p.src[2] : p.src[0], p.nsrc > 2 ? (unsigned)M * (unsigned)p.src_c[2] * 4u : 0u);
    const __amdgpu_buffer_rsrc_t r3 = make_rsrc(p.nsrc > 3 ? p.src[3] : p.src[0], p.nsrc > 3 ? (unsigned)M * (unsigned)p.src_c[3] * 4u : 0u);
// ... 15 lines not shown
    auto issue_a = [&](int set, int g) {
        if (g >= G) return;
        int kk = g;
        if (kk < n0) {
            ra[set][0] = __builtin_amdgcn_raw_buffer_load_b128(r0, (int)v0, kk * 64, 0);
            ra[set][1] = __builtin_amdgcn_raw_buffer_load_b128(r0, (int)v0, kk * 64 + 16, 0);
            return;
        }
        kk -= n0;
        if (kk < n1) {
            ra[set][0] = __builtin_amdgcn_raw_buffer_load_b128(r1, (int)v1, kk * 64, 0);
            ra[set][1] = __builtin_amdgcn_raw_buffer_load_b128(r1, (int)v1, kk * 64 + 16, 0);
            return;
        }
        kk -= n1;
        if (kk < n2) {
            ra[set][0] = __builtin_amdgcn_raw_buffer_load_b128(r2, (int)v2, kk * 64, 0);
            ra[set][1] = __builtin_amdgcn_raw_buffer_load_b128(r2, (int)v2, kk * 64 + 16, 0);
            return;
        }
        kk -= n2;
        ra[set][0] = __builtin_amdgcn_raw_buffer_load_b128(r3, (int)v3, kk * 64, 0);
        ra[set][1] = __builtin_amdgcn_raw_buffer_load_b128(r3, (int)v3, kk * 64 + 16, 0);
    };
    auto issue_b = [&](int set, int g) {
        if (g >= G) return;
#pragma unroll
        for (int j = 0; j < NT; ++j) {
            rbh[set][j] = __builtin_amdgcn_raw_buffer_load_b128(r_wh, (int)bd_off[j], g * 1024, 0);
            rbl[set][j] = __builtin_amdgcn_raw_buffer_load_b128(r_wl, (int)bd_off[j], g * 1024, 0);
        }
    };

    acc_t acc[1][NT];
#pragma unroll
    for (int j = 0; j < NT; ++j)
#pragma unroll
        for (int r = 0; r < F::NACC; ++r) acc[0][j][r] = 0.f;

#pragma unroll
    for (int u = 0; u < DB; ++u) issue_b(u, u);
#pragma unroll
    for (int u = 0; u < DA; ++u) issue_a(u, u);

    for (int g0 = 0; g0 < G; g0 += DA) {
#pragma unroll
        for (int u = 0; u < DA; ++u) {
            const int g = g0 + u;
            if (g < G) {
                const u32x4 x0 = ra[u][0], x1 = ra[u][1];
                const Split2 s0 = split2(__uint_as_float(x0.x) * afwd, __uint_as_float(x0.y) * afwd);
                const Split2 s1 = split2(__uint_as_float(x0.z) * afwd, __uint_as_float(x0.w) * afwd);
                const Split2 s2 = split2(__uint_as_float(x1.x) * afwd, __uint_as_float(x1.y) * afwd);
                const Split2 s3 = split2(__uint_as_float(x1.z) * afwd, __uint_as_float(x1.w) * afwd);
                const u32x4 hv = {s0.hi, s1.hi, s2.hi, s3.hi}, lv = {s0.lo, s1.lo, s2.lo, s3.lo};
                const h8 ah = *reinterpret_cast<const h8*>(&hv), al = *reinterpret_cast<const h8*>(&lv);
                issue_a(u, g + DA);
                __builtin_amdgcn_sched_barrier(0);
                constexpr int DBm = DB;
                const int sb = u % DBm;
#pragma unroll
                for (int j = 0; j < NT; ++j)
                    acc[0][j] = __builtin_amdgcn_mfma_f32_32x32x16_f16(al, *reinterpret_cast<const h8*>(&rbh[sb][j]), acc[0][j], 0, 0, 0);
#pragma unroll
                for (int j = 0; j < NT; ++j)
                    acc[0][j] = __builtin_amdgcn_mfma_f32_32x32x16_f16(ah, *reinterpret_cast<const h8*>(&rbl[sb][j]), acc[0][j], 0, 0, 0);
#pragma unroll
                for (int j = 0; j < NT; ++j)
                    acc[0][j] = __builtin_amdgcn_mfma_f32_32x32x16_f16(ah, *reinterpret_cast<const h8*>(&rbh[sb][j]), acc[0][j], 0, 0, 0);
                __builtin_amdgcn_sched_barrier(0);
                issue_b(sb, g + DB);
                __builtin_amdgcn_sched_barrier(0);
            }
        }
    }
    igemm_epilogue<32, 1, NT, 4, 1>(p, acc, tm, tn, wid, 0, lane, ainv);
}

constexpr int PA = 3;
constexpr int PW_PITCH = 80;
constexpr int PW_PLANE = 32 * PW_PITCH;

template <int NT>
__global__ __launch_bounds__(256, NT == 2 ? 3 : 2) void pw16s_kernel(const ConvParams p, const int tiles_m, const int tiles_n) {
    typedef Frag<32> F;
    typedef F::acc_t acc_t;
    __shared__ __attribute__((aligned(16))) unsigned char stage_s[4][2 * PW_PLANE];
    const int lane = threadIdx.x & 63;
    const int wid = __builtin_amdgcn_readfirstlane(threadIdx.x >> 6);
    const int tile = tile_of_block(tiles_m, tiles_n);
    const int tn = tile % tiles_n, tm = tile / tiles_n;
    const int M = p.B * p.Ho * p.Wo;
    float afwd, ainv;
    conv_in_scale(p, &afwd, &ainv);
    unsigned char* st_hi = stage_s[wid];
    unsigned char* st_lo = st_hi + PW_PLANE;

    const int c4 = lane & 7, row0 = tm * 128 + wid * 32 + (lane >> 3);
    const int n0 = p.src_c[0] >> 5, n1 = p.nsrc > 1 ? p.src_c[1] >> 5 : 0, n2 = p.nsrc > 2 ? p.src_c[2] >> 5 : 0;
    const __amdgpu_buffer_rsrc_t r0 = make_rsrc(p.src[0], (unsigned)M * (unsigned)p.src_c[0] * 4u);
    const __amdgpu_buffer_rsrc_t r1 = make_rsrc(p.nsrc > 1 ? p.src[1] : p.src[0], p.nsrc > 1 ? (unsigned)M * (unsigned)p.src_c[1] * 4u : 0u);
    const __amdgpu_buffer_rsrc_t r2 = make_rsrc(p.nsrc > 2 ? p.src[2] : p.src[0], p.nsrc > 2 ? (unsigned)M * (unsigned)p.src_c[2] * 4u : 0u);
    const __amdgpu_buffer_rsrc_t r3 = make_rsrc(p.nsrc > 3 ? p.src[3] : p.src[0], p.nsrc > 3 ? (unsigned)M * (unsigned)p.src_c[3] * 4u : 0u);
    const int GC = p.Kpad16 >> 5;

    const unsigned w_bytes = (unsigned)((size_t)p.CoutPad * p.Kpad16 * 2);
    const __amdgpu_buffer_rsrc_t r_wh = make_rsrc(p.w16f_hi, w_bytes), r_wl = make_rsrc(p.w16f_lo, w_bytes);
    const int G = p.Kpad16 >> 4;
    unsigned bd_off[NT];
#pragma unroll
    for (int j = 0; j < NT; ++j) bd_off[j] = (unsigned)((((tn * NT + j) * G) * 64 + lane) * 16);

    u32x4 ra[PA][4];
    u32x4 rbh[DB][NT], rbl[DB][NT];
    auto load4 = [&](u32x4 (&dst)[4], const __amdgpu_buffer_rsrc_t r, const int cs, const int kk) {
        const unsigned v = (unsigned)row0 * (unsigned)(cs * 4) + (unsigned)(c4 * 16);
#pragma unroll
        for (int i = 0; i < 4; ++i) dst[i] = __builtin_amdgcn_raw_buffer_load_b128(r, (int)v, kk * 128 + i * 8 * cs * 4, 0);
    };
    auto issue_a = [&](int set, int c) {
        if (c >= GC) return;
        int kk = c;
        if (kk < n0) { load4(ra[set], r0, p.src_c[0], kk); return; }
        kk -= n0;
        if (kk < n1) { load4(ra[set], r1, p.src_c[1], kk); return; }
        kk -= n1;
        if (kk < n2) { load4(ra[set], r2, p.src_c[2], kk); return; }
        kk -= n2;
        load4(ra[set], r3, p.src_c[3], kk);
    };
    auto issue_b = [&](int set, int g) {
        if (g >= G) return;
#pragma unroll
        for (int j = 0; j < NT; ++j) {
            rbh[set][j] = __builtin_amdgcn_raw_buffer_load_b128(r_wh, (int)bd_off[j], g * 1024, 0);
            rbl[set][j] = __builtin_amdgcn_raw_buffer_load_b128(r_wl, (int)bd_off[j], g * 1024, 0);
        }
    };

    acc_t acc[1][NT];
#pragma unroll
    for (int j = 0; j < NT; ++j)
#pragma unroll
        for (int r = 0; r < F::NACC; ++r) acc[0][j][r] = 0.f;

#pragma unroll
    for (int u = 0; u < DB; ++u) issue_b(u, u);
#pragma unroll
    for (int u = 0; u < PA; ++u) issue_a(u, u);

    const int wr_off = (lane >> 3) * PW_PITCH + c4 * 8;
    const int rd_off = (lane & 31) * PW_PITCH + (lane >> 5) * 16;
    static_assert((2 * PA) % DB == 0, "the B register set of a K step must be a compile-time index");
    for (int c0 = 0; c0 < GC; c0 += PA) {
#pragma unroll
        for (int u = 0; u < PA; ++u) {
            const int c = c0 + u;
            if (c < GC) {
#pragma unroll
                for (int i = 0; i < 4; ++i) {
                    const u32x4 x = ra[u][i];
                    const Split2 s0 = split2(__uint_as_float(x.x) * afwd, __uint_as_float(x.y) * afwd);
                    const Split2 s1 = split2(__uint_as_float(x.z) * afwd, __uint_as_float(x.w) * afwd);
                    *reinterpret_cast<u32x2*>(st_hi + wr_off + 8 * i * PW_PITCH) = u32x2{s0.hi, s1.hi};
                    *reinterpret_cast<u32x2*>(st_lo + wr_off + 8 * i * PW_PITCH) = u32x2{s0.lo, s1.lo};
                }
                issue_a(u, c + PA);
                __builtin_amdgcn_wave_barrier();
                h8 ah[2], al[2];
#pragma unroll
                for (int h = 0; h < 2; ++h) {
                    ah[h] = *reinterpret_cast<const h8*>(st_hi + rd_off + 32 * h);
                    al[h] = *reinterpret_cast<const h8*>(st_lo + rd_off + 32 * h);
                }
                __builtin_amdgcn_wave_barrier();
#pragma unroll
                for (int h = 0; h < 2; ++h) {
                    const int g = 2 * c + h;
                    const int sb = (2 * u + h) % DB;
                    __builtin_amdgcn_sched_barrier(0);
#pragma unroll
                    for (int j = 0; j < NT; ++j)
                        acc[0][j] = __builtin_amdgcn_mfma_f32_32x32x16_f16(al[h], *reinterpret_cast<const h8*>(&rbh[sb][j]), acc[0][j], 0, 0, 0);
#pragma unroll
                    for (int j = 0; j < NT; ++j)
                        acc[0][j] = __builtin_amdgcn_mfma_f32_32x32x16_f16(ah[h], *reinterpret_cast<const h8*>(&rbl[sb][j]), acc[0][j], 0, 0, 0);
#pragma unroll
                    for (int j = 0; j < NT; ++j)
                        acc[0][j] = __builtin_amdgcn_mfma_f32_32x32x16_f16(ah[h], *reinterpret_cast<const h8*>(&rbh[sb][j]), acc[0][j], 0, 0, 0);
                    __builtin_amdgcn_sched_barrier(0);
                    issue_b(sb, g + DB);
                    __builtin_amdgcn_sched_barrier(0);
                }
            }
        }
    }
    igemm_epilogue<32, 1, NT, 4, 1>(p, acc, tm, tn, wid, 0, lane, ainv);
}

template <int NT>
int launch_pw16s(const ConvParams& p, hipStream_t stream) {
    const int M = p.B * p.Ho * p.Wo;
    const int tiles_m = (M + 127) / 128, tiles_n = p.CoutPad / (32 * NT);
    hipLaunchKernelGGL((pw16s_kernel<NT>), dim3(tiles_m * tiles_n), dim3(256), 0, stream, p, tiles_m, tiles_n);
    return hipGetLastError() == hipSuccess ? CP_OK : CP_ERR_LAUNCH;
}

template <int NT>
int launch_pw16(const ConvParams& p, hipStream_t stream) {
    const int M = p.B * p.Ho * p.Wo;
    const int tiles_m = (M + 127) / 128, tiles_n = p.CoutPad / (32 * NT);
    hipLaunchKernelGGL((pw16_kernel<NT>), dim3(tiles_m * tiles_n), dim3(256), 0, stream, p, tiles_m, tiles_n);
    return hipGetLastError() == hipSuccess ? CP_OK : CP_ERR_LAUNCH;
}

}

static_assert(DA % DB == 0, "the B register set of a K step must be a compile-time index");

bool cp_pw16_supported(const ConvParams& p) {
    if (!p.w16f_hi || !p.w16f_lo || p.KH != 1 || p.KW != 1 || p.stride != 1 || p.pad != 0 || p.H != p.Ho || p.W != p.Wo)
        return false;
    if (p.offmask || p.gn_in_a || p.gn_in_d || p.gn_in_mr || p.gn_stats || p.splitk > 1 || p.nsrc < 1 || p.nsrc > 4)
        return false;
    if (p.CoutPad % 64 != 0 || p.Kpad16 != p.Cin || p.Cin % 32 != 0) return false;
    int c = 0;
    const size_t M = (size_t)p.B * p.Ho * p.Wo;
    for (int s = 0; s < p.nsrc; ++s) {
        if (p.src_c[s] % 32 != 0 || M * p.src_c[s] * 4 >= (size_t)0xf0000000u) return false;
        c += p.src_c[s];
    }
    return c == p.Cin && (size_t)p.CoutPad * p.Kpad16 * 2 < (size_t)0x7fffffff && M * p.ldo * 4 < (size_t)0xf0000000u;
}

int cp_launch_pw16(const ConvParams& p, hipStream_t stream) {
    if (!cp_pw16_supported(p)) return CP_ERR_INVALID;
    if (!(p.dbg & CP_SEL_PW16_FRAG_A)) return p.CoutPad % 128 == 0 ? launch_pw16s<4>(p, stream) : launch_pw16s<2>(p, stream);
    return p.CoutPad % 128 == 0 ? launch_pw16<4>(p, stream) : launch_pw16<2>(p, stream);
}
```

### centerpose_amd/hip.py

```python
import contextlib
import ctypes
import enum
import os
from collections import OrderedDict
from collections.abc import Mapping

import torch

_HERE = os.path.dirname(os.path.abspath(__file__))
LIB_PATH = os.environ.get("CENTERPOSE_HIP_LIB") or os.path.join(_HERE, "libcenterpose_hip.so")

_lib = None
ABI_VERSION = 7

c_void_p = ctypes.c_void_p
c_int = ctypes.c_int
c_size_t = ctypes.c_size_t
c_char_p = ctypes.c_char_p


class TrackParams(ctypes.Structure):
    _fields_ = [(n, ctypes.c_double) for n in ("new_thresh", "pre_thresh", "R", "conf_lo", "conf_hi")] + \
               [(n, ctypes.c_int) for n in ("max_age", "kalman", "scale_pool", "use_pnp", "hps_uncertainty", "show_axes",
                                            "cat_rule", "render_hm_mode", "render_hmhp_mode", "pre_hm", "pre_hm_hp", "K",
# ... 19 lines not shown
                ("clamped", (c_void_p * 2) * POSE_LOSS_MAX_STACKS)]


CP_ERR_INVALID = -1
PT_MAX_OBJS = 64
PT_IMG_STRIDE, PT_OBJ_STRIDE = 32, 64
PT_IMG = dict(trans=0, width=6, height=7, flipped=8, rot=9, num_objs=10, proj=11)
PT_OBJ = dict(nsym=0, cuboid=1, quat=19, loc=23, kps3d=26, scale=53)
PT_FLAGS = ("center_3D", "use_absolute_scale", "obj_scale", "hps_uncertainty", "reg_hp_offset", "hm_hp")
PT_OUTPUTS = ("hm", "hm_hp", "reg_mask", "ind", "hps", "hps_mask", "hps_uncertainty", "wh", "reg", "scale",
              "scale_uncertainty", "hp_offset", "hp_ind", "hp_mask")


class PoseTargetsDesc(ctypes.Structure):
    _fields_ = [(n, c_int) for n in ("B", "S", "R", "max_objs", "num_joints") + PT_FLAGS] + \
               [("images", c_void_p), ("objects", c_void_p)] + [("out_" + n, c_void_p) for n in PT_OUTPUTS]


PTK_IMG_STRIDE, PTK_PRE_STRIDE, PTK_CUR_STRIDE = 32, 128, 2
PTK_IMG = dict(trans=0, num_pre=6, proj=7)
PTK_PRE = dict(skip=56, idsym=57, id=58, draws=64)
PTK_DRAW = dict(ct_noise=0, ct_lost=2, ct_heat=3, ct_fp=4, ct_fp_noise=5, ct_fp_peak=7, joints=8, joint_stride=7,
                j_noise=0, j_lost=2, j_fp=3, j_fp_noise=4, j_fp_peak=6)
PTK_NUM_DRAWS = 64
PTK_CUR = dict(id=0, skip=1)
PTK_GEOMETRY = ("input_w", "input_h", "down_ratio", "max_pre_objs")
PTK_FLAGS = ("hm_heat_random", "hm_hp_heat_random", "tracking_label_mode", "pre_hm", "pre_hm_hp", "tracking", "tracking_hp")
PTK_DISTURB = ("hm_disturb", "lost_disturb", "fp_disturb", "hm_hp_disturb", "hp_lost_disturb", "hp_fp_disturb")
PTK_OUTPUTS = ("pre_hm", "pre_hm_hp", "tracking", "tracking_mask", "tracking_hp", "tracking_hp_mask")


class PoseTargetsTrackDesc(ctypes.Structure):
    _fields_ = [("cur", PoseTargetsDesc)] + [(n, c_int) for n in PTK_GEOMETRY + PTK_FLAGS + ("reserved",)] + \
               [(n, ctypes.c_double) for n in PTK_DISTURB] + \
               [(n, c_void_p) for n in ("track_images", "pre_objects", "cur_objects")] + \
               [("out_" + n, c_void_p) for n in PTK_OUTPUTS]


def _sig(fn, restype, *argtypes):
    fn.restype = restype
    fn.argtypes = list(argtypes)


def lib():
    global _lib
    if _lib is not None:
        return _lib
    if not os.path.exists(LIB_PATH):
        raise RuntimeError(
            "centerpose_amd: %s not found — build it with `python -c 'import __graft_entry__ as g; g.build()'` "
            "(or `make -C centerpose_amd/csrc`).  There is no CPU fallback." % LIB_PATH)
    L = ctypes.CDLL(LIB_PATH)
    if not hasattr(L, "cp_abi_version"):
        raise RuntimeError("centerpose_amd: %s predates the ABI guard (no cp_abi_version): rebuild the library" % LIB_PATH)
    _sig(L.cp_abi_version, c_int)
    if L.cp_abi_version() != ABI_VERSION:
        raise RuntimeError("centerpose_amd: %s has ABI version %d, this binding was written for %d (rebuild the library)"
                           % (LIB_PATH, L.cp_abi_version(), ABI_VERSION))
    _sig(L.cp_version, c_char_p)
    _sig(L.cp_last_error, c_char_p)
    _sig(L.cp_num_kernel_variants, c_int)
    _sig(L.cp_num_roles, c_int)
    _sig(L.cp_dcnv2_workspace_bytes, c_size_t, c_int, c_int, c_int, c_int, c_int)
    _sig(L.cp_dcnv2_forward, c_int, c_void_p, c_void_p, c_void_p, c_void_p, c_void_p, c_void_p, c_void_p,
         *([c_int] * 14), c_void_p, c_size_t)
    _sig(L.cp_dcnv2_backward_workspace_bytes, c_size_t, *([c_int] * 14))
    _sig(L.cp_dcnv2_backward, c_int, *([c_void_p] * 11), *([c_int] * 14), c_void_p, c_size_t)
    _sig(L.cp_pose_heads_chunk_images, c_int, c_int, c_int, c_int, c_int)
    _sig(L.cp_pose_heads_forward_workspace_bytes, c_size_t, *([c_int] * 6), ctypes.POINTER(c_int))
    _sig(L.cp_pose_heads_backward_workspace_bytes, c_size_t, *([c_int] * 6), ctypes.POINTER(c_int))
    _sig(L.cp_pose_heads_forward, c_int, c_void_p, c_void_p, c_int, *([ctypes.POINTER(c_void_p)] * 4), ctypes.POINTER(c_int),
         ctypes.POINTER(c_void_p), *([c_int] * 5), c_void_p, c_size_t)
    _sig(L.cp_pose_heads_backward, c_int, c_void_p, c_void_p, c_int, *([ctypes.POINTER(c_void_p)] * 4), ctypes.POINTER(c_int),
         *([ctypes.POINTER(c_void_p)] * 5), c_void_p, *([c_int] * 5), c_void_p, c_size_t)
    _sig(L.cp_model_features, c_int, c_void_p, c_void_p, c_int, c_int, c_int, c_void_p, c_void_p, c_void_p, c_void_p,
         c_void_p, c_void_p, c_size_t)
    _sig(L.cp_model_create, c_int, c_char_p, c_int, c_int, ctypes.POINTER(c_char_p), ctypes.POINTER(c_int), c_int,
         ctypes.POINTER(c_void_p))
    _sig(L.cp_model_set_param, c_int, c_void_p, c_char_p, c_void_p, ctypes.c_int64)
    _sig(L.cp_model_finalize, c_int, c_void_p)
    _sig(L.cp_model_destroy, None, c_void_p)
    _sig(L.cp_model_workspace_bytes, c_size_t, c_void_p, c_int, c_int, c_int)
    _sig(L.cp_model_workspace_used, c_size_t, c_void_p)
    _sig(L.cp_model_forward, c_int, c_void_p, c_void_p, c_int, c_int, c_int, c_void_p, c_void_p, c_void_p, c_void_p,
         ctypes.POINTER(c_void_p), c_int, c_void_p, c_size_t)
    _sig(L.cp_model_forward_tap, c_int, c_void_p, c_void_p, c_int, c_int, c_int, c_void_p, c_void_p, c_void_p,
         c_void_p, ctypes.POINTER(c_void_p), c_int, c_void_p, c_size_t, c_char_p, c_void_p, ctypes.POINTER(c_int))
    _sig(L.cp_conv2d_workspace_bytes, c_size_t, c_int, c_int, c_int, c_int)
    _sig(L.cp_conv_transpose2d_workspace_bytes, c_size_t, c_int, c_int)
    _sig(L.cp_conv_transpose2d_nhwc, c_int, c_void_p, c_void_p, c_void_p, c_void_p, c_void_p, c_void_p,
         c_int, c_int, c_int, c_int, c_int, c_int, c_void_p, c_size_t)
    _sig(L.cp_conv2d_nhwc, c_int, c_void_p, c_void_p, c_void_p, c_void_p, c_void_p, c_void_p, c_void_p,
         *([c_int] * 10), c_void_p, c_size_t)
    _sig(L.cp_conv2d_backward_workspace_bytes, c_size_t, *([c_int] * 10))
    _sig(L.cp_conv2d_backward_nhwc, c_int, *([c_void_p] * 8), *([c_int] * 9), c_void_p, c_size_t)
    _sig(L.cp_conv_transpose2d_dw_nhwc, c_int, *([c_void_p] * 5), *([c_int] * 5))
    _sig(L.cp_conv_transpose2d_backward_workspace_bytes, c_size_t, *([c_int] * 10))
    _sig(L.cp_conv_transpose2d_backward_nhwc, c_int, *([c_void_p] * 6), *([c_int] * 9), c_void_p, c_size_t)
    _sig(L.cp_batchnorm_workspace_bytes, c_size_t, *([c_int] * 4))
    _sig(L.cp_batchnorm_forward_nhwc, c_int, *([c_void_p] * 10), *([c_int] * 5), ctypes.c_float, ctypes.c_float, c_int, c_void_p,
         c_size_t)
    _sig(L.cp_batchnorm_backward_nhwc, c_int, *([c_void_p] * 11), *([c_int] * 5), c_void_p, c_size_t)
    _sig(L.cp_groupnorm_workspace_bytes, c_size_t, *([c_int] * 5))
    _sig(L.cp_groupnorm_forward_nhwc, c_int, *([c_void_p] * 7), *([c_int] * 5), ctypes.c_float, c_int, c_void_p, c_size_t)
    _sig(L.cp_groupnorm_backward_nhwc, c_int, *([c_void_p] * 10), *([c_int] * 5), c_void_p, c_size_t)
    _sig(L.cp_gru_gate_forward, c_int, *([c_void_p] * 5), c_int, c_int)
    _sig(L.cp_gru_gate_backward, c_int, *([c_void_p] * 8), c_int, c_int)
    _sig(L.cp_maxpool2d_forward_nhwc, c_int, c_void_p, c_void_p, c_void_p, *([c_int] * 7))
    _sig(L.cp_maxpool2d_backward_nhwc, c_int, c_void_p, c_void_p, c_void_p, c_void_p, *([c_int] * 7))
    _sig(L.cp_conv2d_stem_backward_workspace_bytes, c_size_t, *([c_int] * 6))
    _sig(L.cp_conv2d_stem_backward, c_int, *([c_void_p] * 7), c_size_t, *([c_int] * 6))
    _sig(L.cp_decode_workspace_bytes, c_size_t, c_int, c_int)
    _sig(L.cp_decode, c_int, c_void_p, c_int, c_int, c_int, *([c_void_p] * 11), c_int, c_int, c_int, ctypes.c_float,
         c_int, c_int, c_void_p, c_void_p, c_size_t)
    _sig(L.cp_decode_tiled_workspace_bytes, c_size_t, c_int, c_int, c_int, c_int)
    _sig(L.cp_decode_tiled, c_int, c_void_p, c_int, c_int, c_int, *([c_void_p] * 11), c_int, c_int, c_int, ctypes.c_float,
         c_int, c_int, c_void_p, c_void_p, c_size_t)
    _sig(L.cp_model_detect_workspace_bytes, c_size_t, c_void_p, c_int, c_int, c_int, c_int)
    _sig(L.cp_model_detect, c_int, c_void_p, c_void_p, c_int, c_int, c_int, c_void_p, c_void_p, c_void_p, c_void_p,
         ctypes.POINTER(c_void_p), c_int, c_int, c_int, ctypes.c_float, c_int, c_void_p, c_void_p, c_size_t, c_int)
    _sig(L.cp_model_lean_supported, c_int, c_void_p, c_int, c_int, c_int)
    _sig(L.cp_model_detect_lean_workspace_bytes, c_size_t, c_void_p, c_int, c_int, c_int, c_int)
    _sig(L.cp_model_detect_lean, c_int, c_void_p, c_void_p, c_int, c_int, c_int, c_void_p, c_void_p, c_void_p, c_void_p,
         ctypes.POINTER(c_void_p), ctypes.POINTER(c_void_p), c_void_p, c_void_p, c_int, c_int, c_int, ctypes.c_float, c_int,
         c_void_p, c_void_p, c_size_t, c_int)
    _sig(L.cp_model_dense_heads, c_int, c_void_p, c_void_p, ctypes.POINTER(c_void_p))
    _sig(L.cp_model_heads_at_workspace_bytes, c_size_t, c_void_p, c_int, c_int)
    _sig(L.cp_model_heads_at, c_int, c_void_p, c_void_p, c_void_p, c_int, ctypes.POINTER(c_void_p), c_void_p, c_size_t)
    _sig(L.cp_decode_peaks_workspace_bytes, c_size_t, c_int, c_int, c_int, c_int)
    _sig(L.cp_decode_peaks, c_int, c_void_p, c_int, c_int, c_int, c_void_p, c_void_p, c_int, c_int, c_void_p, c_void_p,
         c_void_p, c_size_t)
    _sig(L.cp_decode_gathered, c_int, c_void_p, c_int, c_int, c_int, *([c_void_p] * 12), c_int, c_int, c_int, ctypes.c_float,
         c_int, c_void_p)
    _sig(L.cp_set_default_precision, c_int, c_int)
    _sig(L.cp_set_debug, c_int, c_int)
    _sig(L.cp_render_gaussians, c_int, c_void_p, c_void_p, c_int, c_void_p, c_int, c_int, c_int, c_int)
    _sig(L.cp_postprocess_workspace_bytes, c_size_t, c_int, c_int)
    _sig(L.cp_postprocess, c_int, c_void_p, c_void_p, c_int, c_int, c_void_p, ctypes.c_double, c_int, ctypes.c_float,
         c_void_p, c_void_p, c_void_p, c_size_t)
    _sig(L.cp_preprocess, c_int, c_void_p, c_void_p, c_int, c_int, ctypes.POINTER(ctypes.c_double),
         ctypes.POINTER(ctypes.c_float), ctypes.POINTER(ctypes.c_float), c_void_p, c_int, c_int)
    _sig(L.cp_preprocess_batch, c_int, c_void_p, c_void_p, c_int, c_int, c_int, ctypes.POINTER(ctypes.c_double),
         ctypes.POINTER(ctypes.c_float), ctypes.POINTER(ctypes.c_float), c_void_p, c_int, c_int)
    _sig(L.cp_resize_u8, c_int, c_void_p, c_void_p, c_int, c_int, c_int, c_void_p, c_int, c_int)
    _sig(L.cp_model_set_precision, c_int, c_void_p, c_int)
    _sig(L.cp_model_profile, c_int, c_void_p, c_int)
    _sig(L.cp_model_profile_read, c_int, c_void_p, ctypes.POINTER(ctypes.c_double), c_int)
    _sig(L.cp_kernel_variant_name, c_char_p, c_int)
    _sig(L.cp_model_profile_roles, c_int, c_void_p, ctypes.POINTER(ctypes.c_double), c_int)
    _sig(L.cp_role_name, c_char_p, c_int)
    _sig(L.cp_pnp_workspace_bytes, c_size_t, c_int)
    _sig(L.cp_pnp_from_post_workspace_bytes, c_size_t, c_int, c_int)
    _sig(L.cp_pnp_from_post, c_int, c_void_p, c_void_p, c_void_p, c_int, c_int, c_int, c_void_p, c_void_p, c_void_p, c_size_t)
    _sig(L.cp_pnp_solve, c_int, c_void_p, c_void_p, c_void_p, c_void_p, c_int, c_int, c_void_p, c_void_p, c_size_t)
    _sig(L.cp_track_state_bytes, c_size_t, c_int, c_int)
    _sig(L.cp_track_workspace_bytes, c_size_t, c_int, c_int, c_int)
    _sig(L.cp_track_reset, c_int, c_void_p, c_void_p, c_int, c_int)
    _sig(L.cp_track_status, c_int, c_void_p, c_void_p, c_int, ctypes.POINTER(c_int))
    _sig(L.cp_track_step, c_int, c_void_p, ctypes.POINTER(TrackParams), c_void_p, c_void_p, c_void_p, c_void_p, c_int, c_void_p,
         c_void_p, c_void_p, c_size_t)
    _sig(L.cp_linear_assignment, c_int, c_void_p, c_int, c_int, c_int, ctypes.POINTER(c_int))
    _sig(L.cp_box_iou, c_int, c_void_p, c_void_p, c_void_p, c_int, c_void_p)
    _sig(L.cp_box_eval, c_int, c_void_p, *([c_void_p] * 6), c_int, c_int, c_void_p)
    _sig(L.cp_pose_loss_workspace_bytes, c_size_t, ctypes.POINTER(PoseLossDesc))
    _sig(L.cp_pose_loss_forward, c_int, c_void_p, ctypes.POINTER(PoseLossDesc), c_void_p, c_void_p, c_void_p, c_void_p,
         c_void_p, c_size_t)
    _sig(L.cp_pose_loss_backward, c_int, c_void_p, ctypes.POINTER(PoseLossDesc), c_void_p, ctypes.POINTER(c_void_p),
         ctypes.POINTER(c_void_p), c_void_p, c_size_t)
    _sig(L.cp_pose_targets_workspace_bytes, c_size_t, ctypes.POINTER(PoseTargetsDesc))
    _sig(L.cp_pose_targets, c_int, c_void_p, ctypes.POINTER(PoseTargetsDesc), c_void_p, c_size_t)
    _sig(L.cp_pose_targets_track_workspace_bytes, c_size_t, ctypes.POINTER(PoseTargetsTrackDesc))
    _sig(L.cp_pose_targets_track, c_int, c_void_p, ctypes.POINTER(PoseTargetsTrackDesc), c_void_p, c_size_t)
    _lib = L
    return L


def linear_assignment(cost, solver=1):
    import numpy as np

    cost = np.ascontiguousarray(cost, dtype=np.float64)
    if cost.ndim != 2:
        raise ValueError("linear_assignment: a 2-D cost matrix is expected")
    n, m = cost.shape
    match = (c_int * max(n, 1))()
    _check(lib().cp_linear_assignment(cost.ctypes.data_as(c_void_p), n, m, int(solver), match), "cp_linear_assignment")
    return np.array([(i, match[i]) for i in range(n) if match[i] >= 0], dtype=np.int64).reshape(-1, 2)


def exported_symbols():
    return ["cp_version", "cp_last_error", "cp_dcnv2_workspace_bytes", "cp_dcnv2_forward", "cp_model_create",
            "cp_model_set_param", "cp_model_finalize", "cp_model_destroy", "cp_model_workspace_bytes", "cp_model_workspace_used",
            "cp_model_forward", "cp_model_forward_tap", "cp_conv2d_workspace_bytes", "cp_conv2d_nhwc",
            "cp_decode_workspace_bytes", "cp_decode", "cp_pnp_workspace_bytes", "cp_pnp_solve", "cp_model_profile", "cp_model_profile_read",
            "cp_kernel_variant_name", "cp_set_default_precision", "cp_model_set_precision", "cp_model_detect_workspace_bytes", "cp_model_detect", "cp_set_debug", "cp_preprocess", "cp_preprocess_batch", "cp_postprocess_workspace_bytes", "cp_postprocess", "cp_render_gaussians",
            "cp_model_profile_roles", "cp_role_name", "cp_pnp_from_post_workspace_bytes", "cp_pnp_from_post", "cp_resize_u8",
            "cp_abi_version", "cp_num_kernel_variants", "cp_num_roles", "cp_track_state_bytes", "cp_track_workspace_bytes",
            "cp_track_reset", "cp_track_step", "cp_track_status", "cp_linear_assignment", "cp_decode_tiled_workspace_bytes",
            "cp_decode_tiled", "cp_box_iou", "cp_box_eval", "cp_conv_transpose2d_workspace_bytes",
            "cp_conv_transpose2d_nhwc", "cp_dcnv2_backward_workspace_bytes", "cp_dcnv2_backward",
            "cp_pose_loss_workspace_bytes", "cp_pose_loss_forward", "cp_pose_loss_backward",
            "cp_pose_targets_workspace_bytes", "cp_pose_targets", "cp_model_lean_supported",
            "cp_model_detect_lean_workspace_bytes", "cp_model_detect_lean", "cp_model_dense_heads",
            "cp_model_heads_at_workspace_bytes", "cp_model_heads_at", "cp_decode_peaks_workspace_bytes", "cp_decode_peaks",
            "cp_decode_gathered", "cp_pose_heads_chunk_images", "cp_pose_heads_forward_workspace_bytes",
            "cp_pose_heads_forward", "cp_pose_heads_backward_workspace_bytes", "cp_pose_heads_backward",
            "cp_model_features", "cp_conv2d_backward_workspace_bytes", "cp_conv2d_backward_nhwc",
            "cp_batchnorm_workspace_bytes", "cp_batchnorm_forward_nhwc", "cp_batchnorm_backward_nhwc",
            "cp_conv_transpose2d_dw_nhwc", "cp_conv_transpose2d_backward_workspace_bytes",
            "cp_conv_transpose2d_backward_nhwc", "cp_maxpool2d_forward_nhwc", "cp_maxpool2d_backward_nhwc",
            "cp_conv2d_stem_backward_workspace_bytes", "cp_conv2d_stem_backward", "cp_groupnorm_workspace_bytes",
            "cp_groupnorm_forward_nhwc", "cp_groupnorm_backward_nhwc", "cp_gru_gate_forward", "cp_gru_gate_backward",
            "cp_pose_targets_track_workspace_bytes", "cp_pose_targets_track"]


def _check(rc, what):
    if rc != 0:
        msg = lib().cp_last_error().decode() if _lib is not None else ""
        raise RuntimeError("centerpose_hip: %s failed with code %d (%s)" % (what, rc, msg))


class KernelSel(enum.IntFlag):
    HEADS_SLABS = 0x00000001
    HEADS_WG_PER_HEAD = 0x00000002
    PW16_FRAG_A = 0x00000004
    SPLITK_ELEMENTWISE = 0x00000008
    TILE128_SMALL = 0x00000010
    NO_HEAD_FUSION = 0x00000020
    NO_LOWC = 0x00000040
    GN_HEAD_F32 = 0x00000080
    GRU_UNFUSED = 0x00000100
    NO_PRESCALE = 0x00000200
    DCN16S_GRID8 = 0x00000400
    HALO_NEVER = 0x00001000
    HALO_ALWAYS = 0x00002000
    HALO_LDS_WEIGHTS = 0x00004000
    DCN16P_NEVER = 0x00008000
    DCN16P_ALWAYS = 0x00010000
    GN_HEAD_MFMA = 0x00020000
    LEVEL1_ROWS_NEVER = 0x00040000
    DCN16P_NOT_WIDE = 0x00080000
    DCN16S_NEVER = 0x00100000
    DCN16S_ALWAYS = 0x00200000
    PW16_NEVER = 0x00400000
    DCN_GENERIC = 0x00800000
    HEADS_PER_HEAD_LAUNCH = 0x01000000
    DCN16T_ALWAYS = 0x02000000
    DCN16T_NEVER = 0x04000000
    STEM_LEVEL0_UNFUSED = 0x08000000
    STRM16_NEVER = 0x10000000
    STRM16_ALWAYS = 0x20000000
    LEVEL1_ROWS_ALWAYS = 0x40000000


@contextlib.contextmanager
def select_kernels(flags):
    _check(lib().cp_set_debug(int(flags)), "cp_set_debug")
    try:
        yield
    finally:
        lib().cp_set_debug(0)


def _stream():
    return c_void_p(torch.cuda.current_stream().cuda_stream)


def _ptr(t):
    return c_void_p(t.data_ptr()) if t is not None else c_void_p(0)


def _dev(t):
    if not t.is_cuda:
        raise RuntimeError("centerpose_hip: tensors must live on the HIP device (no CPU path)")
    return t.contiguous().float()
# ... 1026 lines not shown
        if m._det_gen != self._gen:
            raise RuntimeError("detect: the dense '%s' maps of this call were not read before the next detect() on the model, and "
                               "the feature map they are computed from is gone; read them earlier or call detect(heads=\"dense\")"
                               % "', '".join(k for k in self._shapes if k not in self._ready))
        dev = self.pk_ind.device
        new = OrderedDict((k, torch.empty(*shp, device=dev, dtype=torch.float32)) for k, shp in self._shapes.items()
                          if k not in self._ready)
        ptrs = (c_void_p * len(self._shapes))(*[new[k].data_ptr() if k in new else 0 for k in self._shapes])
        _check(lib().cp_model_dense_heads(m._h, _stream(), ptrs), "cp_model_dense_heads")
        self._ready.update(new)


class HipModel(object):

    def __init__(self, arch, heads, state_dict, tracking_task=False, head_conv=256, precision=None):
        L = lib()
        self.arch = arch
        self.heads = OrderedDict(heads)
        self.tracking_task = bool(tracking_task)
        names = (c_char_p * len(self.heads))(*[k.encode() for k in self.heads])
        classes = (c_int * len(self.heads))(*[int(v) for v in self.heads.values()])
        h = c_void_p()
        _check(L.cp_model_create(arch.encode(), int(self.tracking_task), len(self.heads), names, classes,
                                 int(head_conv), ctypes.byref(h)), "cp_model_create")
        self._h = h
        for k, v in state_dict.items():
            if k.startswith("module.") and not k.startswith("module_list"):
                k = k[7:]
            if not torch.is_floating_point(v):
                continue
            t = v.detach().cpu().contiguous().float()
            _check(L.cp_model_set_param(h, k.encode(), c_void_p(t.data_ptr()), t.numel()), "cp_model_set_param")
        _check(L.cp_model_finalize(h), "cp_model_finalize")
        if precision is not None:
            self.set_precision(precision)
        self._ws = None
        self._ws_key = None

    def __del__(self):
        try:
            if getattr(self, "_h", None) is not None and _lib is not None:
                _lib.cp_model_destroy(self._h)
                self._h = None
        except Exception:
            pass

    def set_precision(self, name):
        _check(lib().cp_model_set_precision(self._h, PRECISIONS[name]), "cp_model_set_precision")
        self.precision = name

    def profile(self, enable=True):
        _check(lib().cp_model_profile(self._h, int(bool(enable))), "cp_model_profile")

    def profile_read(self):
        nv = lib().cp_num_kernel_variants()
        buf = (ctypes.c_double * (nv * 4))()
        _check(lib().cp_model_profile_read(self._h, buf, nv), "cp_model_profile_read")
        out = OrderedDict()
        for v in range(nv):
            if buf[v * 4] > 0:
                out[lib().cp_kernel_variant_name(v).decode()] = dict(
                    launches=int(buf[v * 4]), ms=buf[v * 4 + 1], flops=buf[v * 4 + 2], bytes=buf[v * 4 + 3])
        return out

    def profile_roles(self):
        nr = lib().cp_num_roles()
        buf = (ctypes.c_double * (nr * 4))()
        _check(lib().cp_model_profile_roles(self._h, buf, nr), "cp_model_profile_roles")
        out = OrderedDict()
        for r in range(nr):
            if buf[r * 4] > 0:
                out[lib().cp_role_name(r).decode()] = dict(
                    launches=int(buf[r * 4]), ms=buf[r * 4 + 1], flops=buf[r * 4 + 2], bytes=buf[r * 4 + 3])
        return out

    def workspace_bytes(self, B, H, W):
        n = lib().cp_model_workspace_bytes(self._h, B, H, W)
        if n == 0:
            raise RuntimeError("cp_model_workspace_bytes failed: " + lib().cp_last_error().decode())
        return n

    def workspace_used(self):
        return int(lib().cp_model_workspace_used(self._h))

    def _workspace(self, B, H, W, device):
        key = (B, H, W, str(device))
        if self._ws_key != key:
            self._ws = None
            n = self.workspace_bytes(B, H, W)
            self._ws = torch.empty(n, dtype=torch.uint8, device=device)
            self._ws_key = key
        return self._ws

    def forward(self, images, pre_img=None, pre_hm=None, pre_hm_hp=None, sigmoid_hm=False, tap=None):
        L = lib()
        images = _dev(images)
        B, _, H, W = images.shape
        pre_img = _dev(pre_img) if pre_img is not None else None
        pre_hm = _dev(pre_hm) if pre_hm is not None else None
        pre_hm_hp = _dev(pre_hm_hp) if pre_hm_hp is not None else None
        outs = OrderedDict()
        for k, c in self.heads.items():
            outs[k] = torch.empty(B, c, H // 4, W // 4, device=images.device, dtype=torch.float32)
        ptrs = (c_void_p * len(outs))(*[t.data_ptr() for t in outs.values()])
        ws = self._workspace(B, H, W, images.device)
        if tap is None:
            rc = L.cp_model_forward(self._h, _stream(), B, H, W, _ptr(images), _ptr(pre_img), _ptr(pre_hm),
                                    _ptr(pre_hm_hp), ptrs, int(bool(sigmoid_hm)), _ptr(ws), ws.numel())
            _check(rc, "cp_model_forward")
            return outs
        tap_buf = torch.zeros(B * 512 * (H // 4) * (W // 4) if False else B * 16 * H * W, device=images.device,
                              dtype=torch.float32)
        dims = (c_int * 3)(0, 0, 0)
        rc = L.cp_model_forward_tap(self._h, _stream(), B, H, W, _ptr(images), _ptr(pre_img), _ptr(pre_hm),
                                    _ptr(pre_hm_hp), ptrs, int(bool(sigmoid_hm)), _ptr(ws), ws.numel(),
                                    tap.encode(), _ptr(tap_buf), dims)
        _check(rc, "cp_model_forward_tap")
        C, h, w = dims[0], dims[1], dims[2]
        if C == 0:
            raise RuntimeError("unknown tap %r" % tap)
        return outs, tap_buf[: B * C * h * w].view(B, C, h, w)

    def features(self, images, pre_img=None, pre_hm=None, pre_hm_hp=None):
        L = lib()
        if self.arch.startswith("dlav1") or self.arch == "hourglass":
            raise NotImplementedError("features(): %s has no single feature map that plain conv3x3 -> ReLU -> conv1x1 heads read"
                                      % self.arch)
        images = _dev(images)
        B, _, H, W = images.shape
        pre_img = _dev(pre_img) if pre_img is not None else None
        pre_hm = _dev(pre_hm) if pre_hm is not None else None
        pre_hm_hp = _dev(pre_hm_hp) if pre_hm_hp is not None else None
        feat = torch.empty(B, H // 4, W // 4, 64, device=images.device, dtype=torch.float32)
        ws = self._workspace(B, H, W, images.device)
        rc = L.cp_model_features(self._h, _stream(), B, H, W, _ptr(images), _ptr(pre_img), _ptr(pre_hm), _ptr(pre_hm_hp),
                                 _ptr(feat), _ptr(ws), ws.numel())
        _check(rc, "cp_model_features")
        return feat.permute(0, 3, 1, 2)

    def lean_supported(self, B, H, W):
        return bool(lib().cp_model_lean_supported(self._h, int(B), int(H), int(W)))

    def heads_at(self, index):
        L = lib()
        index = index.to(torch.int32).contiguous()
        B, n = index.shape
        out = OrderedDict((k, torch.empty(B, c, n, device=index.device, dtype=torch.float32)) for k, c in self.heads.items()
                          if k not in _MAP_HEADS)
        ptrs = (c_void_p * len(self.heads))(*[out[k].data_ptr() if k in out else 0 for k in self.heads])
        nb = L.cp_model_heads_at_workspace_bytes(self._h, B, n)
        ws = torch.empty(max(nb, 256), dtype=torch.uint8, device=index.device)
        _check(L.cp_model_heads_at(self._h, _stream(), _ptr(index), n, ptrs, _ptr(ws), ws.numel()), "cp_model_heads_at")
        return out

    def _detect_lean(self, images, pre_img, pre_hm, pre_hm_hp, K, rep_mode, fit_gaussian, balance, legacy_bool_mask, graph):
        L = lib()
        B, _, H, W = images.shape
        dev = images.device
        key = ("lean", B, H, W, str(dev), K)
        st = getattr(self, "_lean_state", None)
        if st is None or st[0] != key:
            f32 = dict(device=dev, dtype=torch.float32)
            maps = OrderedDict((k, torch.empty(B, self.heads[k], H // 4, W // 4, **f32)) for k in _MAP_HEADS)
            tables = OrderedDict((k, torch.empty(*((B, 8, 2, K) if k == "hp_offset" else (B, c, K)), **f32))
                                 for k, c in self.heads.items() if k not in _MAP_HEADS)
            pk_score = torch.empty(B, 9, K, **f32)
# ... 283 lines not shown
```

### include/centerpose_hip.h

```cpp
#ifndef CENTERPOSE_HIP_H
#define CENTERPOSE_HIP_H

#include <stddef.h>
#include <stdint.h>

#ifdef __cplusplus
extern "C" {
#endif

typedef void* cp_stream_t;
typedef struct cp_model cp_model;

#define CP_OK 0
#define CP_ERR_INVALID (-1)
#define CP_ERR_LAUNCH (-2)
#define CP_ERR_ALLOC (-3)
#define CP_ERR_STATE (-4)

#define CP_ABI_VERSION 7
const char* cp_version(void);
int cp_abi_version(void);
const char* cp_last_error(void);

size_t cp_dcnv2_workspace_bytes(int B, int C, int H, int W, int Co);
int cp_dcnv2_forward(cp_stream_t stream, const float* input, const float* weight, const float* bias,
                     const float* offset, const float* mask, float* output, int B, int C, int H, int W, int Co,
                     int kh, int kw, int sh, int sw, int ph, int pw, int dh, int dw, int deformable_group,
                     void* workspace, size_t workspace_bytes);

size_t cp_dcnv2_backward_workspace_bytes(int B, int C, int H, int W, int Co, int kh, int kw, int sh, int sw, int ph,
                                         int pw, int dh, int dw, int deformable_group);
int cp_dcnv2_backward(cp_stream_t stream, const float* input, const float* weight, const float* offset,
                      const float* mask, const float* grad_output, float* grad_input, float* grad_offset,
                      float* grad_mask, float* grad_weight, float* grad_bias, int B, int C, int H, int W, int Co,
                      int kh, int kw, int sh, int sw, int ph, int pw, int dh, int dw, int deformable_group,
                      void* workspace, size_t workspace_bytes);

int cp_pose_heads_chunk_images(int B, int H, int W, int hid);
size_t cp_pose_heads_forward_workspace_bytes(int B, int H, int W, int Cin, int hid, int n, const int* classes);
int cp_pose_heads_forward(cp_stream_t stream, const float* feat, int n, const float* const* w0, const float* const* b0,
                          const float* const* w1, const float* const* b1, const int* classes, float* const* out, int B,
                          int H, int W, int Cin, int hid, void* workspace, size_t workspace_bytes);
size_t cp_pose_heads_backward_workspace_bytes(int B, int H, int W, int Cin, int hid, int n, const int* classes);
int cp_pose_heads_backward(cp_stream_t stream, const float* feat, int n, const float* const* w0, const float* const* b0,
                           const float* const* w1, const float* const* b1, const int* classes,
                           const float* const* grad_out, float* const* grad_w0, float* const* grad_b0,
                           float* const* grad_w1, float* const* grad_b1, float* grad_feat, int B, int H, int W, int Cin,
                           int hid, void* workspace, size_t workspace_bytes);

int cp_model_create(const char* arch, int tracking_task, int num_heads, const char* const* head_names,
                    const int* head_classes, int head_conv, cp_model** out);
int cp_model_set_param(cp_model* m, const char* name, const float* host_data, int64_t numel);
int cp_model_finalize(cp_model* m);
void cp_model_destroy(cp_model* m);

size_t cp_model_workspace_bytes(cp_model* m, int B, int H, int W);
size_t cp_model_workspace_used(const cp_model* m);

int cp_model_forward(cp_model* m, cp_stream_t stream, int B, int H, int W, const float* images,
                     const float* pre_img, const float* pre_hm, const float* pre_hm_hp, float* const* head_out,
                     int sigmoid_hm, void* workspace, size_t workspace_bytes);

int cp_model_features(cp_model* m, cp_stream_t stream, int B, int H, int W, const float* images, const float* pre_img,
                      const float* pre_hm, const float* pre_hm_hp, float* feat_out, void* workspace,
                      size_t workspace_bytes);

size_t cp_model_detect_workspace_bytes(cp_model* m, int B, int H, int W, int K);
int cp_model_detect(cp_model* m, cp_stream_t stream, int B, int H, int W, const float* images, const float* pre_img,
                    const float* pre_hm, const float* pre_hm_hp, float* const* head_out, int K, int rep_mode,
                    int fit_gaussian, float balance, int legacy_bool_mask, float* det, void* workspace,
                    size_t workspace_bytes, int use_graph);

int cp_model_lean_supported(cp_model* m, int B, int H, int W);
size_t cp_model_detect_lean_workspace_bytes(cp_model* m, int B, int H, int W, int K);
int cp_model_detect_lean(cp_model* m, cp_stream_t stream, int B, int H, int W, const float* images, const float* pre_img,
                         const float* pre_hm, const float* pre_hm_hp, float* const* head_out, float* const* table_out,
                         float* pk_score, int* pk_ind, int K, int rep_mode, int fit_gaussian, float balance,
                         int legacy_bool_mask, float* det, void* workspace, size_t workspace_bytes, int use_graph);
int cp_model_dense_heads(cp_model* m, cp_stream_t stream, float* const* head_out);
size_t cp_model_heads_at_workspace_bytes(cp_model* m, int B, int n);
int cp_model_heads_at(cp_model* m, cp_stream_t stream, const int* index, int n, float* const* table_out, void* workspace,
                      size_t workspace_bytes);

int cp_model_forward_tap(cp_model* m, cp_stream_t stream, int B, int H, int W, const float* images,
                         const float* pre_img, const float* pre_hm, const float* pre_hm_hp, float* const* head_out,
                         int sigmoid_hm, void* workspace, size_t workspace_bytes, const char* tap_name,
                         float* tap_out, int* tap_dims);

#define CP_PREC_F32 0
#define CP_PREC_F16X3 1
int cp_set_default_precision(int precision);
int cp_model_set_precision(cp_model* m, int precision);

#define CP_NUM_KERNEL_VARIANTS 46
int cp_num_kernel_variants(void);
int cp_model_profile(cp_model* m, int enable);
int cp_model_profile_read(cp_model* m, double* out, int num_variants);
const char* cp_kernel_variant_name(int v);
#define CP_ROLE_CONV 0
#define CP_ROLE_CONV1X1 1
#define CP_ROLE_DCN 2
#define CP_ROLE_DCN_OFFSET 3
#define CP_ROLE_HEAD 4
#define CP_ROLE_HEAD_FINAL 5
#define CP_ROLE_GRU 6
#define CP_ROLE_LOWC 7
#define CP_ROLE_DECODE 8
#define CP_ROLE_DECONV 9
#define CP_NUM_ROLES 10
int cp_num_roles(void);
int cp_model_profile_roles(cp_model* m, double* out, int num_roles);
const char* cp_role_name(int role);

size_t cp_conv2d_workspace_bytes(int Cin, int Cout, int KH, int KW);
int cp_conv2d_nhwc(cp_stream_t stream, const float* x, const float* w, const float* scale, const float* shift,
                   const float* residual, float* out, int B, int H, int W, int Cin, int Cout, int KH, int KW,
                   int stride, int pad, int act, void* workspace, size_t workspace_bytes);

size_t cp_conv2d_backward_workspace_bytes(int B, int H, int W, int Cin, int Cout, int KH, int KW, int stride, int pad,
                                          int need_grad_x);
int cp_conv2d_backward_nhwc(cp_stream_t stream, const float* x, const float* w, const float* y_or_null,
                            const float* grad_out, float* grad_x_or_null, float* grad_w, float* grad_bias_or_null, int B,
                            int H, int W, int Cin, int Cout, int KH, int KW, int stride, int pad, void* workspace,
                            size_t workspace_bytes);

size_t cp_batchnorm_workspace_bytes(int B, int H, int W, int C);
int cp_batchnorm_forward_nhwc(cp_stream_t stream, const float* x, const float* gamma_or_null, const float* beta_or_null,
                              const float* residual_or_null, float* running_mean_or_null, float* running_var_or_null,
                              float* y, float* save_mean, float* save_invstd, int B, int H, int W, int C, int training,
                              float momentum, float eps, int act, void* workspace, size_t workspace_bytes);
int cp_batchnorm_backward_nhwc(cp_stream_t stream, const float* x, const float* y_or_null, const float* grad_out,
                               const float* gamma_or_null, const float* save_mean, const float* save_invstd,
                               float* grad_x_or_null, float* grad_residual_or_null, float* grad_gamma_or_null,
                               float* grad_beta_or_null, int B, int H, int W, int C, int training, void* workspace,
                               size_t workspace_bytes);

size_t cp_groupnorm_workspace_bytes(int B, int H, int W, int C, int G);
int cp_groupnorm_forward_nhwc(cp_stream_t stream, const float* x, const float* gamma_or_null, const float* beta_or_null,
                              float* y, float* save_mean, float* save_invstd, int B, int H, int W, int C, int G, float eps,
                              int act, void* workspace, size_t workspace_bytes);
// ... 232 lines not shown
```

Before: 4577.

## Fuse 2x2 maxpool into level1 lowc and pointwise root conv epilogues

```diff
diff --git a/centerpose_amd/csrc/cp_common.h b/centerpose_amd/csrc/cp_common.h
--- a/centerpose_amd/csrc/cp_common.h
+++ b/centerpose_amd/csrc/cp_common.h
@@ -134,6 +134,7 @@
     const void* pj_w_lo;
     const float* pj_scale;
     const float* pj_shift;
+    float* pool_out;
 };
 
 int cp_launch_conv(const ConvParams& p, hipStream_t stream);
@@ -165,6 +166,7 @@
 int cp_launch_strm16(const ConvParams& p, hipStream_t stream);
 int cp_launch_dcn16(const ConvParams& p, int bn, hipStream_t stream);
 bool cp_pw16_supported(const ConvParams& p);
+bool cp_pw16_pool_supported(const ConvParams& p);
 int cp_launch_pw16(const ConvParams& p, hipStream_t stream);
 bool cp_dcn16p_supported(const ConvParams& p);
 int cp_dcn16p_blocks(const ConvParams& p);
@@ -210,7 +212,8 @@
 int cp_launch_pack_lowc(int kind, const float* w, void* hi, void* lo, const float* fwd, int cin, hipStream_t s);
 int cp_launch_lowc(int kind, const float* in, float* out, const void* w_hi, const void* w_lo, const float* scale,
                    const float* shift, const unsigned* in_amax, unsigned* out_amax, int B, int H, int W, int planes,
-                   hipStream_t s);
+                   hipStream_t s, float* pool_out = nullptr);
+bool cp_lowc_pool_supported(int kind, int H, int W);
 #define CP_VARIANT_LOWC0 23
 #define CP_VARIANT_LOWC01 40
 int cp_launch_lowc_fused(const float* in, float* out, const void* w0_hi, const void* w0_lo, const float* scale0, const float* shift0,
diff --git a/centerpose_amd/csrc/engine.hip b/centerpose_amd/csrc/engine.hip
--- a/centerpose_amd/csrc/engine.hip
+++ b/centerpose_amd/csrc/engine.hip
@@ -135,6 +135,7 @@
 }
 
 size_t cp_model_workspace_used(const cp_model* m) { return m ? m->arena.peak : 0; }
+int cp_model_maxpool_launches(const cp_model* m) { return m ? m->maxpool2_launches : 0; }
 
 size_t cp_model_workspace_bytes(cp_model* m, int B, int H, int W) {
     if (!m) {
@@ -147,19 +148,21 @@
     const char* const tap_before = m->tap_name;
     const int nu = m->ups_t.empty() ? 1 : 3;
     const int np = m->convs.count("base.level2.project") ? 2 : 1;
-    for (int v = 0; v < 4 * nu * np; ++v) {
+    for (int v = 0; v < 4 * nu * np * np; ++v) {
         const int up = (v >> 2) % nu;
         m->dry_variant = v & 1;
         m->tap_name = (v & 2) ? "" : nullptr;
         m->dry_no_upadd = up != 0;
         m->dry_boundary_upadd = up == 2;
-        m->dry_no_project = v >= 4 * nu;
+        m->dry_no_project = (v / (4 * nu)) % np == 1;
+        m->dry_no_pool = v >= 4 * nu * np;
         const int rc = forward_impl(m, nullptr, B, H, W, nullptr, (const float*)1, (const float*)1, (const float*)1, nullptr, 0,
                                     nullptr, 0, true);
         m->dry_variant = 0;
         m->dry_no_upadd = false;
         m->dry_boundary_upadd = false;
         m->dry_no_project = false;
+        m->dry_no_pool = false;
         m->tap_name = tap_before;
         if (rc != CP_OK) return 0;
         if (m->arena.peak > peak) peak = m->arena.peak;
diff --git a/centerpose_amd/csrc/engine_forward.hip b/centerpose_amd/csrc/engine_forward.hip
--- a/centerpose_amd/csrc/engine_forward.hip
+++ b/centerpose_amd/csrc/engine_forward.hip
@@ -375,7 +375,8 @@
 
     Tensor conv(const ConvW& w, const std::vector<const Tensor*>& srcs, int stride, int pad, int act,
                 const Tensor* res = nullptr, const Tensor* offmask = nullptr, int act_from = 0,
-                float* out_nchw = nullptr, int out_ld = 0, const UpFuse* up = nullptr, const ProjFuse* pj = nullptr) {
+                float* out_nchw = nullptr, int out_ld = 0, const UpFuse* up = nullptr, const ProjFuse* pj = nullptr,
+                Tensor* pooled = nullptr) {
         const Tensor& x0 = *srcs[0];
         const int nsrc = (int)srcs.size();
         const float* src[CP_MAX_SRC];
@@ -434,6 +435,14 @@
         if (p.splitk > 1) {
             partial = make(p.splitk * p.CoutPad, p.Ho, p.Wo);
             p.partial = partial.ptr();
+        }
+        if (pooled && use16 && !out_nchw && p.splitk == 1 && !up && !pj && !m->dry_no_pool) {
+            const int v = cp_conv16_variant(p);
+            if ((v == CP_VARIANT_PW16 || v == CP_VARIANT_PW16 + 1) && cp_pw16_pool_supported(p)) {
+                *pooled = make(p.ldo, p.Ho / 2, p.Wo / 2);
+                pooled->amax = out.amax;
+                p.pool_out = m->dry ? (float*)0x1000 : pooled->ptr();
+            }
         }
         if (up) {
             p.up_t = up->t->ptr();
@@ -466,7 +475,7 @@
                 r.bytes = 4.0 * ((double)B * x0.H * x0.W * cin_real + M * w.Cout +
                                  (double)w.KH * w.KW * cin_real * w.Cout + (offmask ? M * 27 : 0.0) +
                                  (res ? M * w.Cout : 0.0) + (up ? (double)B * up->t->H * up->t->W * w.Cout : 0.0) +
-                                 (pj ? (M + w.Cout) * (double)pj->w->Cin : 0.0));
+                                 (pj ? (M + w.Cout) * (double)pj->w->Cin : 0.0) + (p.pool_out ? M / 4 * w.Cout : 0.0));
                 r.M = (int)M; r.N = w.Cout; r.K = w.KH * w.KW * cin_real; r.kh = w.KH; r.stride = stride;
             }, launch);
         gn_stats_out = nullptr;
@@ -482,6 +491,7 @@
     Tensor maxpool(const Tensor& x) {
         Tensor o = make(x.C, x.H / 2, x.W / 2);
         o.amax = x.amax;
+        ++m->maxpool2_launches;
         if (!m->dry) chk(cp_launch_maxpool2(x.ptr(), o.ptr(), B, x.H, x.W, x.C, s));
         return o;
     }
@@ -495,7 +505,7 @@
     }
 
     Tensor tree1(const std::string& p, const Tensor& x, int cin, int cout, int stride, bool level_root,
-                 std::vector<const Tensor*> children, const Tensor* bottom_in = nullptr) {
+                 std::vector<const Tensor*> children, const Tensor* bottom_in = nullptr, Tensor* pool_next = nullptr) {
         Tensor bottom_own;
         const Tensor* bottom = &x;
         if (stride > 1) {
@@ -504,6 +514,7 @@
                 bottom_own = maxpool(x);
                 bottom = &bottom_own;
             }
+            tap(p + ".bottom", *bottom);
         }
         Tensor proj;
         const Tensor* residual = bottom;
@@ -526,14 +537,15 @@
         Tensor x2 = basic_block(p + ".tree2", x1, 1, &x1);
         std::vector<const Tensor*> srcs = {&x2, &x1};
         for (auto* c : children) srcs.push_back(c);
-        Tensor o = conv(cw(p + ".root"), srcs, 1, 0, CP_ACT_RELU);
+        Tensor o = conv(cw(p + ".root"), srcs, 1, 0, CP_ACT_RELU, nullptr, nullptr, 0, nullptr, 0, nullptr, nullptr, pool_next);
         tap(p + ".root", o);
         return o;
     }
-    Tensor tree2(const std::string& p, const Tensor& x, int cin, int cout) {
-        Tensor bottom = maxpool(x);
+    Tensor tree2(const std::string& p, const Tensor& x, int cin, int cout, const Tensor& bottom_in, Tensor* pool_next) {
+        Tensor bottom = bottom_in.valid() ? bottom_in : maxpool(x);
+        tap(p + ".bottom", bottom);
         Tensor x1 = tree1(p + ".tree1", x, cin, cout, 2, false, {}, &bottom);
-        return tree1(p + ".tree2", x1, cout, cout, 1, false, {&bottom, &x1});
+        return tree1(p + ".tree2", x1, cout, cout, 1, false, {&bottom, &x1}, nullptr, pool_next);
     }
 
     Tensor deform(const std::string& p, const Tensor& x, const UpFuse* up = nullptr) {
@@ -592,7 +604,8 @@
         return u_next;
     }
 
-    Tensor lowc(const std::string& name, int kind, const float* in, int H, int W, int planes, const unsigned* in_amax) {
+    Tensor lowc(const std::string& name, int kind, const float* in, int H, int W, int planes, const unsigned* in_amax,
+                Tensor* pooled = nullptr) {
         if (m->precision != CP_PREC_F16X3 || (g_dbg & CP_SEL_NO_LOWC)) return Tensor();
         const int Ho = kind == 2 ? (H - 1) / 2 + 1 : H, Wo = kind == 2 ? (W - 1) / 2 + 1 : W;
         if (kind == 2 && m->lowc.count(name + ".rows") && !(g_dbg & CP_SEL_LEVEL1_ROWS_NEVER) &&
@@ -605,17 +618,22 @@
         const bool l1 = kind == 2 || kind == 5;
         const int cout = l1 ? 32 : 16, cin = stem ? planes : 16, k = stem ? 7 : 3;
         Tensor out = make(cout, Ho, Wo);
+        const bool pool = pooled && !m->dry_no_pool && cp_lowc_pool_supported(kind, H, W);
+        if (pool) {
+            *pooled = make(cout, Ho / 2, Wo / 2);
+            pooled->amax = out.amax;
+        }
         if (m->dry) return out;
         auto launch = [&]() {
             return cp_launch_lowc(kind, in, out.ptr(), it->second.hi, it->second.lo, it->second.scale16, w.shift, in_amax,
-                                  out.amax, B, H, W, planes, s);
+                                  out.amax, B, H, W, planes, s, pool ? pooled->ptr() : nullptr);
         };
         timed([&](cp_model::ProfRec& r) {
             r.variant = kind == 5 ? CP_VARIANT_LOWC1S : CP_VARIANT_LOWC0 + (kind == 3 ? 0 : kind);
             r.role = CP_ROLE_LOWC;
             const double M = (double)B * Ho * Wo;
             r.flops = 2.0 * M * cout * (double)(k * k * cin);
-            r.bytes = 4.0 * ((double)B * H * W * cin + M * cout + (double)k * k * cin * cout);
+            r.bytes = 4.0 * ((double)B * H * W * cin + M * cout + (double)k * k * cin * cout + (pool ? M / 4 * cout : 0.0));
             r.M = (int)M; r.N = cout; r.K = k * k * cin; r.kh = k; r.stride = l1 ? 2 : 1;
         }, launch);
         return out;
@@ -835,16 +853,20 @@
         if (!l0.valid()) l0 = conv(cw("base.level0"), {&x0}, 1, 1, CP_ACT_RELU);
         tap("base.level0", l0);
         x0 = Tensor();
-        Tensor l1 = lowc("base.level1", 2, l0.ptr(), H, W, 16, l0.amax);
+        Tensor pl[4];
+        Tensor l1 = lowc("base.level1", 2, l0.ptr(), H, W, 16, l0.amax, &pl[0]);
         if (!l1.valid()) l1 = conv(cw("base.level1"), {&l0}, 2, 1, CP_ACT_RELU);
         tap("base.level1", l1);
         l0 = Tensor();
         std::vector<Tensor> L(6);
-        L[2] = tree1("base.level2", l1, 32, 64, 2, false, {});
-        l1 = Tensor();
-        L[3] = tree2("base.level3", L[2], 64, 128);
-        L[4] = tree2("base.level4", L[3], 128, 256);
-        L[5] = tree1("base.level5", L[4], 256, 512, 2, true, {});
+        L[2] = tree1("base.level2", l1, 32, 64, 2, false, {}, pl[0].valid() ? &pl[0] : nullptr, &pl[1]);
+        l1 = pl[0] = Tensor();
+        L[3] = tree2("base.level3", L[2], 64, 128, pl[1], &pl[2]);
+        pl[1] = Tensor();
+        L[4] = tree2("base.level4", L[3], 128, 256, pl[2], &pl[3]);
+        pl[2] = Tensor();
+        L[5] = tree1("base.level5", L[4], 256, 512, 2, true, {}, pl[3].valid() ? &pl[3] : nullptr);
+        pl[3] = Tensor();
         tap("base.level2", L[2]);
         tap("base.level3", L[3]);
         tap("base.level4", L[4]);
@@ -1025,6 +1047,7 @@
     m->arena.reset(dry ? nullptr : ws, ws_bytes);
     m->dry = dry;
     m->status = CP_OK;
+    m->maxpool2_launches = 0;
     Fwd f{m, B, stream};
     if (m->hourglass) f.run_hourglass(H, W, images, head_out, sigmoid_hm);
     else if (m->resnet) f.run_resnet(H, W, images, head_out, sigmoid_hm);
diff --git a/centerpose_amd/csrc/engine_model.h b/centerpose_amd/csrc/engine_model.h
--- a/centerpose_amd/csrc/engine_model.h
+++ b/centerpose_amd/csrc/engine_model.h
@@ -207,6 +207,7 @@
     bool dry_no_upadd = false;
     bool dry_boundary_upadd = false;
     bool dry_no_project = false;
+    bool dry_no_pool = false;
     int dry_variant = 0;
     float stem_bound_l = 0.f, stem_bound_s = 0.f;
     cp_engine::ConvW gru_x, gru_h;
@@ -222,6 +223,7 @@
     int B = 0;
     bool dry = false;
     int status = CP_OK;
+    int maxpool2_launches = 0;
     const char* tap_name = nullptr;
     float* tap_out = nullptr;
     int* tap_dims = nullptr;
diff --git a/centerpose_amd/csrc/igemm16.hip b/centerpose_amd/csrc/igemm16.hip
--- a/centerpose_amd/csrc/igemm16.hip
+++ b/centerpose_amd/csrc/igemm16.hip
@@ -613,6 +613,8 @@
     if (!cp_conv16_supported(p)) return CP_ERR_INVALID;
     if (p.up_t && !(p.offmask && dcn16t_wanted(p) && cp_dcn16t_upadd_supported(p))) return CP_ERR_INVALID;
     const int bn = conv16_tile_n(p);
+    if (p.pool_out && !(pw16_wanted(p) && cp_conv16_variant(p) == CP_VARIANT_PW16 + (p.CoutPad % 128 == 0 ? 1 : 0) && cp_pw16_pool_supported(p)))
+        return CP_ERR_INVALID;
     if (p.pj_src) return cp_conv16_project_supported(p) ? cp_launch_halo16(p, bn, stream) : CP_ERR_INVALID;
     const bool cat = p.nsrc > 1;
     if (p.gn_in_a) {
diff --git a/centerpose_amd/csrc/lowc.hip b/centerpose_amd/csrc/lowc.hip
--- a/centerpose_amd/csrc/lowc.hip
+++ b/centerpose_amd/csrc/lowc.hip
@@ -468,8 +468,10 @@
     const unsigned* in_amax;
     unsigned* out_amax;
     int B, H, W, Ho, Wo, rows, strips, bands, njobs;
+    float* pool;
 };
 
+template <bool POOL>
 __global__ __launch_bounds__(64 * L1_WAVES, 1) void lowc1s_kernel(const Lowc1Params p) {
     extern __shared__ __attribute__((aligned(16))) unsigned char l1_smem[];
     const int tid = threadIdx.x, lane = tid & 63;
@@ -521,6 +523,11 @@
                                                                             (int)((unsigned)p.H * (unsigned)p.W * 64u), 0x00020000);
         const __amdgpu_buffer_rsrc_t r_out = __builtin_amdgcn_make_buffer_rsrc(p.out + (size_t)b * p.Ho * p.Wo * 32, 0,
                                                                              (int)((unsigned)p.Ho * (unsigned)p.Wo * 128u), 0x00020000);
+        const __amdgpu_buffer_rsrc_t r_pool = __builtin_amdgcn_make_buffer_rsrc(
+            POOL ? p.pool + (size_t)b * (p.Ho >> 1) * (p.Wo >> 1) * 32 : p.out, 0, POOL ? (int)((unsigned)(p.Ho >> 1) * (unsigned)(p.Wo >> 1) * 128u) : 0, 0x00020000);
+        float4 keep[4];
+#pragma unroll
+        for (int g4 = 0; g4 < 4; ++g4) keep[g4] = make_float4(0.f, 0.f, 0.f, 0.f);
         unsigned cvo[L1_NLD];
 #pragma unroll
         for (int k = 0; k < L1_NLD; ++k) {
@@ -572,7 +579,7 @@
                 a = __builtin_amdgcn_mfma_f32_32x32x16_f16(wh, xh, a, 0, 0, 0);
             }
         };
-        auto odd_row = [&](const int j, float4 (&buf)[L1_NLD]) {
+        auto odd_row = [&](const int j, float4 (&buf)[L1_NLD], const bool fold) {
             stage(j, buf);
             mac(2, acc);
             f32x16 nxt;
@@ -592,6 +599,14 @@
                 y.w = fmaxf(acc[4 * g4 + 3] * sc[g4].w + sh[g4].w, 0.f);
                 amax = fmaxf(amax, fmaxf(fmaxf(y.x, y.y), fmaxf(y.z, y.w)) * okf);
                 *reinterpret_cast<float4*>(tr_b + px * L1_TPITCH + (2 * g4 + kg) * 16) = y;
+                if (POOL) {
+                    if (fold) {
+                        keep[g4].x = fmaxf(keep[g4].x, y.x); keep[g4].y = fmaxf(keep[g4].y, y.y);
+                        keep[g4].z = fmaxf(keep[g4].z, y.z); keep[g4].w = fmaxf(keep[g4].w, y.w);
+                    } else {
+                        keep[g4] = y;
+                    }
+                }
             }
             __builtin_amdgcn_wave_barrier();
             const unsigned row_out = (unsigned)(o * p.Wo) * 128u, row_no = ~okm & 0x80000000u;
@@ -603,6 +618,23 @@
                 __builtin_amdgcn_raw_buffer_store_b128(pk, r_out, (int)((row_out + (unsigned)((x0 + pxo) * 128 + (lane & 7) * 16)) | row_no | col_no), 0, 0);
             }
             __builtin_amdgcn_wave_barrier();
+            if (POOL && fold) {
+#pragma unroll
+                for (int g4 = 0; g4 < 4; ++g4) *reinterpret_cast<float4*>(tr_b + px * L1_TPITCH + (2 * g4 + kg) * 16) = keep[g4];
+                __builtin_amdgcn_wave_barrier();
+                const unsigned prow_out = (unsigned)((o >> 1) * (p.Wo >> 1)) * 128u;
+#pragma unroll
+                for (int i = 0; i < 2; ++i) {
+                    const int q = (lane >> 3) + 8 * i;
+                    const float4 a = *reinterpret_cast<const float4*>(tr_b + (2 * q) * L1_TPITCH + (lane & 7) * 16);
+                    const float4 c = *reinterpret_cast<const float4*>(tr_b + (2 * q + 1) * L1_TPITCH + (lane & 7) * 16);
+                    const u32x4 pk = {__float_as_uint(fmaxf(a.x, c.x)), __float_as_uint(fmaxf(a.y, c.y)), __float_as_uint(fmaxf(a.z, c.z)),
+                                      __float_as_uint(fmaxf(a.w, c.w))};
+                    const unsigned col_no = (x0 >> 1) + q < (p.Wo >> 1) ? 0u : 0x80000000u;
+                    __builtin_amdgcn_raw_buffer_store_b128(pk, r_pool, (int)((prow_out + (unsigned)(((x0 >> 1) + q) * 128 + (lane & 7) * 16)) | row_no | col_no), 0, 0);
+                }
+                __builtin_amdgcn_wave_barrier();
+            }
             acc = nxt;
         };
         auto even_row = [&](const int j, float4 (&buf)[L1_NLD]) {
@@ -611,9 +643,9 @@
             __builtin_amdgcn_wave_barrier();
         };
         for (int j = 2 * y0 - 1; j <= jlast; j += 4) {
-            odd_row(j, pf[0]);
+            odd_row(j, pf[0], true);
             even_row(j + 1, pf[1]);
-            odd_row(j + 2, pf[2]);
+            odd_row(j + 2, pf[2], false);
             even_row(j + 3, pf[3]);
         }
     }
@@ -687,9 +719,14 @@
     return hipGetLastError() == hipSuccess ? CP_OK : CP_ERR_LAUNCH;
 }
 
+bool cp_lowc_pool_supported(int kind, int H, int W) {
+    return kind == 5 && ((H + 2 - 3) / 2 + 1) % 2 == 0 && ((W + 2 - 3) / 2 + 1) % 2 == 0;
+}
+
 int cp_launch_lowc(int kind, const float* in, float* out, const void* w_hi, const void* w_lo, const float* scale,
                    const float* shift, const unsigned* in_amax, unsigned* out_amax, int B, int H, int W, int planes,
-                   hipStream_t s) {
+                   hipStream_t s, float* pool_out) {
+    if (pool_out && !cp_lowc_pool_supported(kind, H, W)) return CP_ERR_INVALID;
     LowcParams p;
     p.in_amax = in_amax;
     p.out_amax = out_amax;
@@ -732,7 +769,8 @@
         if (hipGetDevice(&dev) != hipSuccess || dev < 0 || dev >= 16) return CP_ERR_LAUNCH;
         if (!cus_of[dev]) {
             hipDeviceProp_t prop;
-            if (hipFuncSetAttribute(reinterpret_cast<const void*>(&lowc1s_kernel), hipFuncAttributeMaxDynamicSharedMemorySize, L1_LDS) != hipSuccess)
+            if (hipFuncSetAttribute(reinterpret_cast<const void*>(&lowc1s_kernel<false>), hipFuncAttributeMaxDynamicSharedMemorySize, L1_LDS) != hipSuccess ||
+                hipFuncSetAttribute(reinterpret_cast<const void*>(&lowc1s_kernel<true>), hipFuncAttributeMaxDynamicSharedMemorySize, L1_LDS) != hipSuccess)
                 return CP_ERR_LAUNCH;
             cus_of[dev] = (hipGetDeviceProperties(&prop, dev) == hipSuccess && prop.multiProcessorCount > 0) ? prop.multiProcessorCount : 256;
         }
@@ -749,7 +787,9 @@
         q.bands = (q.Ho + rows - 1) / rows;
         q.njobs = B * q.strips * q.bands;
         const int blocks = (q.njobs + L1_WAVES - 1) / L1_WAVES < use_cus ? (q.njobs + L1_WAVES - 1) / L1_WAVES : use_cus;
-        hipLaunchKernelGGL(lowc1s_kernel, dim3(blocks), dim3(64 * L1_WAVES), L1_LDS, s, q);
+        q.pool = pool_out;
+        if (pool_out) hipLaunchKernelGGL(lowc1s_kernel<true>, dim3(blocks), dim3(64 * L1_WAVES), L1_LDS, s, q);
+        else hipLaunchKernelGGL(lowc1s_kernel<false>, dim3(blocks), dim3(64 * L1_WAVES), L1_LDS, s, q);
         return hipGetLastError() == hipSuccess ? CP_OK : CP_ERR_LAUNCH;
     }
     return CP_ERR_INVALID;
diff --git a/centerpose_amd/csrc/pw16.hip b/centerpose_amd/csrc/pw16.hip
--- a/centerpose_amd/csrc/pw16.hip
+++ b/centerpose_amd/csrc/pw16.hip
@@ -121,6 +121,47 @@
 constexpr int PW_PLANE = 32 * PW_PITCH;
 
 template <int NT>
+__device__ __forceinline__ void pw16s_pool_epilogue(const ConvParams& p, f32x16 (&acc)[1][NT], const int tn, const int lane, const float ainv,
+                                                    const bool live, const int pair_row, const int blk) {
+    const int lcol = lane & 31, h = lane >> 5, W = p.Wo;
+    const bool relu = p.act == CP_ACT_RELU;
+    float amax = 0.f;
+    if (live) {
+        const size_t base = (size_t)(2 * pair_row) * W + 16 * blk;
+        const __amdgpu_buffer_rsrc_t ro = make_rsrc(p.out + base * p.ldo, (unsigned)((W + 16) * p.ldo) * 4u);
+        const __amdgpu_buffer_rsrc_t rp = make_rsrc(p.pool_out + ((size_t)pair_row * (W >> 1) + 8 * blk) * p.ldo, (unsigned)(8 * p.ldo) * 4u);
+#pragma unroll
+        for (int j = 0; j < NT; ++j) {
+            const int n = tn * (32 * NT) + j * 32 + lcol;
+            const float sc = (p.scale ? p.scale[n] : 1.f) * ainv;
+            const float sh = p.shift ? p.shift[n] : 0.f;
+            const bool n_ok = n < p.Cout;
+            float v[16];
+#pragma unroll
+            for (int r = 0; r < 16; ++r) v[r] = acc[0][j][r] * sc + sh;
+            if (relu) {
+#pragma unroll
+                for (int r = 0; r < 16; ++r) v[r] = fmaxf(v[r], 0.f);
+            }
+#pragma unroll
+            for (int r = 0; r < 16; ++r) amax = fmaxf(amax, fabsf(v[r]));
+            const unsigned vo = n_ok ? (unsigned)(4 * h * p.ldo + n) * 4u : 0x80000000u;
+#pragma unroll
+            for (int r = 0; r < 16; ++r)
+                __builtin_amdgcn_raw_buffer_store_b32(__float_as_uint(v[r]), ro, (int)vo, ((r >> 3) * W + (r & 3) + 8 * ((r >> 2) & 1)) * p.ldo * 4, 0);
+            const unsigned vp = n_ok ? (unsigned)(2 * h * p.ldo + n) * 4u : 0x80000000u;
+#pragma unroll
+            for (int q = 0; q < 4; ++q) {
+                const int r = 2 * q;
+                const float mx = fmaxf(fmaxf(v[r], v[r + 1]), fmaxf(v[r + 8], v[r + 9]));
+                __builtin_amdgcn_raw_buffer_store_b32(__float_as_uint(mx), rp, (int)vp, ((q & 1) + 4 * (q >> 1)) * p.ldo * 4, 0);
+            }
+        }
+    }
+    if (p.out_amax) cp_amax_commit(p.out_amax, amax);
+}
+
+template <int NT, bool POOL>
 __global__ __launch_bounds__(256, NT == 2 ? 3 : 2) void pw16s_kernel(const ConvParams p, const int tiles_m, const int tiles_n) {
     typedef Frag<32> F;
     typedef F::acc_t acc_t;
@@ -135,13 +176,16 @@
     unsigned char* st_hi = stage_s[wid];
     unsigned char* st_lo = st_hi + PW_PLANE;
 
-    const int c4 = lane & 7, row0 = tm * 128 + wid * 32 + (lane >> 3);
+    const int grp = 4 * tm + wid, wblk = POOL ? p.Wo >> 4 : 1;
+    const int pair_row = POOL ? grp / wblk : 0, blk = POOL ? grp - pair_row * wblk : 0;
+    const bool live = !POOL || pair_row < p.B * (p.Ho >> 1);
+    const int c4 = lane & 7, row0 = POOL ? 2 * pair_row * p.Wo + 16 * blk + (lane >> 3) : tm * 128 + wid * 32 + (lane >> 3);
     const int n0 = p.src_c[0] >> 5, n1 = p.nsrc > 1 ? p.src_c[1] >> 5 : 0, n2 = p.nsrc > 2 ? p.src_c[2] >> 5 : 0;
     const __amdgpu_buffer_rsrc_t r0 = make_rsrc(p.src[0], (unsigned)M * (unsigned)p.src_c[0] * 4u);
     const __amdgpu_buffer_rsrc_t r1 = make_rsrc(p.nsrc > 1 ? p.src[1] : p.src[0], p.nsrc > 1 ? (unsigned)M * (unsigned)p.src_c[1] * 4u : 0u);
     const __amdgpu_buffer_rsrc_t r2 = make_rsrc(p.nsrc > 2 ? p.src[2] : p.src[0], p.nsrc > 2 ? (unsigned)M * (unsigned)p.src_c[2] * 4u : 0u);
     const __amdgpu_buffer_rsrc_t r3 = make_rsrc(p.nsrc > 3 ? p.src[3] : p.src[0], p.nsrc > 3 ? (unsigned)M * (unsigned)p.src_c[3] * 4u : 0u);
-    const int GC = p.Kpad16 >> 5;
+    const int GC = live ? p.Kpad16 >> 5 : 0;
 
     const unsigned w_bytes = (unsigned)((size_t)p.CoutPad * p.Kpad16 * 2);
     const __amdgpu_buffer_rsrc_t r_wh = make_rsrc(p.w16f_hi, w_bytes), r_wl = make_rsrc(p.w16f_lo, w_bytes);
@@ -155,7 +199,8 @@
     auto load4 = [&](u32x4 (&dst)[4], const __amdgpu_buffer_rsrc_t r, const int cs, const int kk) {
         const unsigned v = (unsigned)row0 * (unsigned)(cs * 4) + (unsigned)(c4 * 16);
 #pragma unroll
-        for (int i = 0; i < 4; ++i) dst[i] = __builtin_amdgcn_raw_buffer_load_b128(r, (int)v, kk * 128 + i * 8 * cs * 4, 0);
+        for (int i = 0; i < 4; ++i)
+            dst[i] = __builtin_amdgcn_raw_buffer_load_b128(r, (int)v, kk * 128 + (POOL ? (i >> 1) * p.Wo + (i & 1) * 8 : i * 8) * cs * 4, 0);
     };
     auto issue_a = [&](int set, int c) {
         if (c >= GC) return;
@@ -234,14 +279,16 @@
             }
         }
     }
-    igemm_epilogue<32, 1, NT, 4, 1>(p, acc, tm, tn, wid, 0, lane, ainv);
+    if (POOL) pw16s_pool_epilogue<NT>(p, acc, tn, lane, ainv, live, pair_row, blk);
+    else igemm_epilogue<32, 1, NT, 4, 1>(p, acc, tm, tn, wid, 0, lane, ainv);
 }
 
 template <int NT>
 int launch_pw16s(const ConvParams& p, hipStream_t stream) {
     const int M = p.B * p.Ho * p.Wo;
     const int tiles_m = (M + 127) / 128, tiles_n = p.CoutPad / (32 * NT);
-    hipLaunchKernelGGL((pw16s_kernel<NT>), dim3(tiles_m * tiles_n), dim3(256), 0, stream, p, tiles_m, tiles_n);
+    if (p.pool_out) hipLaunchKernelGGL((pw16s_kernel<NT, true>), dim3(tiles_m * tiles_n), dim3(256), 0, stream, p, tiles_m, tiles_n);
+    else hipLaunchKernelGGL((pw16s_kernel<NT, false>), dim3(tiles_m * tiles_n), dim3(256), 0, stream, p, tiles_m, tiles_n);
     return hipGetLastError() == hipSuccess ? CP_OK : CP_ERR_LAUNCH;
 }
 
@@ -272,8 +319,14 @@
     return c == p.Cin && (size_t)p.CoutPad * p.Kpad16 * 2 < (size_t)0x7fffffff && M * p.ldo * 4 < (size_t)0xf0000000u;
 }
 
+bool cp_pw16_pool_supported(const ConvParams& p) {
+    if (!cp_pw16_supported(p) || (p.dbg & CP_SEL_PW16_FRAG_A)) return false;
+    if (p.res || p.gn_stats || p.store != CP_STORE_NHWC || p.coff != 0 || (p.act != CP_ACT_NONE && p.act != CP_ACT_RELU)) return false;
+    return p.Ho % 2 == 0 && p.Wo % 16 == 0;
+}
+
 int cp_launch_pw16(const ConvParams& p, hipStream_t stream) {
-    if (!cp_pw16_supported(p)) return CP_ERR_INVALID;
+    if (!cp_pw16_supported(p) || (p.pool_out && !cp_pw16_pool_supported(p))) return CP_ERR_INVALID;
     if (!(p.dbg & CP_SEL_PW16_FRAG_A)) return p.CoutPad % 128 == 0 ? launch_pw16s<4>(p, stream) : launch_pw16s<2>(p, stream);
     return p.CoutPad % 128 == 0 ? launch_pw16<4>(p, stream) : launch_pw16<2>(p, stream);
 }
diff --git a/centerpose_amd/hip.py b/centerpose_amd/hip.py
--- a/centerpose_amd/hip.py
+++ b/centerpose_amd/hip.py
@@ -125,6 +125,7 @@
     _sig(L.cp_model_destroy, None, c_void_p)
     _sig(L.cp_model_workspace_bytes, c_size_t, c_void_p, c_int, c_int, c_int)
     _sig(L.cp_model_workspace_used, c_size_t, c_void_p)
+    _sig(L.cp_model_maxpool_launches, c_int, c_void_p)
     _sig(L.cp_model_forward, c_int, c_void_p, c_void_p, c_int, c_int, c_int, c_void_p, c_void_p, c_void_p, c_void_p,
          ctypes.POINTER(c_void_p), c_int, c_void_p, c_size_t)
     _sig(L.cp_model_forward_tap, c_int, c_void_p, c_void_p, c_int, c_int, c_int, c_void_p, c_void_p, c_void_p,
@@ -233,6 +234,7 @@
 def exported_symbols():
     return ["cp_version", "cp_last_error", "cp_dcnv2_workspace_bytes", "cp_dcnv2_forward", "cp_model_create",
             "cp_model_set_param", "cp_model_finalize", "cp_model_destroy", "cp_model_workspace_bytes", "cp_model_workspace_used",
+            "cp_model_maxpool_launches",
             "cp_model_forward", "cp_model_forward_tap", "cp_conv2d_workspace_bytes", "cp_conv2d_nhwc",
             "cp_decode_workspace_bytes", "cp_decode", "cp_pnp_workspace_bytes", "cp_pnp_solve", "cp_model_profile", "cp_model_profile_read",
             "cp_kernel_variant_name", "cp_set_default_precision", "cp_model_set_precision", "cp_model_detect_workspace_bytes", "cp_model_detect", "cp_set_debug", "cp_preprocess", "cp_preprocess_batch", "cp_postprocess_workspace_bytes", "cp_postprocess", "cp_render_gaussians",
@@ -1425,6 +1427,9 @@
 
     def workspace_used(self):
         return int(lib().cp_model_workspace_used(self._h))
+
+    def maxpool_launches(self):
+        return int(lib().cp_model_maxpool_launches(self._h))
 
     def _workspace(self, B, H, W, device):
         key = (B, H, W, str(device))
diff --git a/include/centerpose_hip.h b/include/centerpose_hip.h
--- a/include/centerpose_hip.h
+++ b/include/centerpose_hip.h
@@ -56,6 +56,7 @@
 
 size_t cp_model_workspace_bytes(cp_model* m, int B, int H, int W);
 size_t cp_model_workspace_used(const cp_model* m);
+int cp_model_maxpool_launches(const cp_model* m);
 
 int cp_model_forward(cp_model* m, cp_stream_t stream, int B, int H, int W, const float* images,
                      const float* pre_img, const float* pre_hm, const float* pre_hm_hp, float* const* head_out,
```

New measurement: 4624, median of 6. +1.0%, better.
